# fritzsedlazeck/Sniffles

Hardware: NVIDIA H100
Metric: aligned long-read Gbp/s through lead->cluster->consensus (higher is better)
Workload: dtype int32

## Files before the change

### include/snfb.h

```cpp
#ifndef SNFB_H
#define SNFB_H

#include <stddef.h>
#include <stdint.h>

#ifdef __cplusplus
extern "C" {
#endif

#define SNFB_ABI_VERSION 3

enum { SNFB_INS = 0, SNFB_DEL = 1, SNFB_DUP = 2, SNFB_INV = 3, SNFB_BND = 4,
       SNFB_SINGLE_LEFT = 5, SNFB_SINGLE_RIGHT = 6, SNFB_NTYPES = 7 };
enum { SNFB_SRC_INLINE = 0, SNFB_SRC_SPLIT_PRIM = 1, SNFB_SRC_SPLIT_SUP = 2, SNFB_SRC_BND_SA = 3 };

#define SNFB_MEM_HOST 0u
#define SNFB_MEM_DEVICE 1u
#define SNFB_MEM_HOST_SEQ_ON_DEMAND 2u

#define SNFB_CIGAR_BAM32 0u
#define SNFB_CIGAR_16 1u
#define SNFB_CIGAR16_EVT_MIN 11u

#define SNFB_AUX_NM 1u
// ... 154 lines not shown
    int32_t  fwd;
    int32_t  rev;
    int32_t  support_long;
    int32_t  support_sa;
    int32_t  cov_upstream, cov_start, cov_center, cov_end, cov_downstream;
    int32_t  hap_counts[6];
    int32_t  sa_count;
    int32_t  sa_total;
    int32_t  bnd_mate_contig;
    int32_t  bnd_mate_pos;
    int32_t  bnd_is_first;
    int32_t  bnd_is_reverse;
    int32_t  n_strands;
    int32_t  support_inline;
    int32_t  lead_off;
    int32_t  lead_n;
    int32_t  long_off;
    int32_t  long_n;
    int32_t  alt_off;
    int32_t  alt_len;
    int32_t  hp_top, hp_support, hp_other;
    int32_t  ps_top, ps_top_null, ps_support, ps_other;
    int32_t  cluster_seed;
    int32_t  resplit_bin;
    double   stdev_pos;
    double   stdev_len;
    double   nm_mean;
} snfb_cand;

typedef struct snfb_cand_view {
    uint64_t n_cand;
    const snfb_cand* cand;
    uint64_t n_cand_leads;
    const snfb_lead* cand_leads;
    const uint64_t*  rnames;
    const uint32_t*  rnames_off;
    const double*    task_coverage_mean;
    uint64_t unverified_breaks;
} snfb_cand_view;

typedef struct snfb_seq_view {
    uint64_t n_alt_bytes;
    const uint8_t* alt;
} snfb_seq_view;

typedef struct snfb_ctx snfb_ctx;

int         snfb_version(void);
size_t      snfb_sizeof(int which);
uint64_t    snfb_hash_name(const char* s, size_t n);
int         snfb_ctx_create(int device, snfb_ctx** out);
void        snfb_ctx_destroy(snfb_ctx* ctx);
const char* snfb_last_error(snfb_ctx* ctx);
int         snfb_set_config(snfb_ctx* ctx, const snfb_config* cfg);
int         snfb_load_records(snfb_ctx* ctx, const snfb_records* block);
int         snfb_extract_leads(snfb_ctx* ctx, snfb_lead_view* out);
int         snfb_cluster_call(snfb_ctx* ctx, snfb_cand_view* out);
int         snfb_consensus(snfb_ctx* ctx, snfb_seq_view* out);
int         snfb_run(snfb_ctx* ctx, snfb_lead_view* leads, snfb_cand_view* cands, snfb_seq_view* seqs);
typedef struct snfb_bam_span {
    uint64_t cbeg, cend;
    uint32_t ubeg, uend;
    uint32_t task;
    uint32_t region;
} snfb_bam_span;
typedef struct snfb_bam_input {
    const uint8_t* bgzf; uint64_t n_bytes;
    const snfb_bam_span* span; uint64_t n_span;
    uint32_t n_task, n_contig, n_tr, n_mask;
    const snfb_task* task; const snfb_contig* contig; const int32_t* tr; const int32_t* mask; const uint32_t* mask_task_off;
} snfb_bam_input;
int         snfb_load_bam(snfb_ctx* ctx, const snfb_bam_input* in);
typedef struct snfb_region { int32_t task, start, end, _pad; } snfb_region;
int         snfb_set_regions(snfb_ctx* ctx, const snfb_region* regions, uint32_t n);
int         snfb_ingest_sizes(snfb_ctx* ctx, uint64_t out[8]);
int         snfb_ingest_fetch(snfb_ctx* ctx, snfb_rec* rec, uint16_t* cigar16, uint8_t* var, uint8_t* seq);
int         snfb_inflate_bgzf(snfb_ctx* ctx, const uint8_t* bgzf, uint64_t n_bytes, uint8_t* out, uint64_t out_cap, uint64_t* out_len);
int         snfb_deflate_bgzf(snfb_ctx* ctx, const uint8_t* in, uint64_t n_in, uint8_t* out, uint64_t out_cap, uint64_t* out_len, uint64_t* coffset);
int         snfb_last_timings(snfb_ctx* ctx, const char** names, float* ms, uint64_t* bytes, int cap);
int         snfb_device_candidates(snfb_ctx* ctx, void** dptr, uint64_t* n_cand);
int         snfb_device_alt(snfb_ctx* ctx, void** dptr, uint64_t* n_bytes);
uint64_t    snfb_launch_count(snfb_ctx* ctx);
uint64_t    snfb_rerun_count(snfb_ctx* ctx);
int         snfb_coverage_bins(snfb_ctx* ctx, uint32_t task, int binsize, const double** out, uint64_t* n_bins);
typedef struct snfb_gt_in {
    uint64_t n;
    const int32_t* task; const int32_t* svtype; const int32_t* pos; const int32_t* svlen; const int32_t* bnd_is_first; const int32_t* mate_contig;
    int32_t combine_match, combine_match_max;
} snfb_gt_in;
typedef struct snfb_gt_out {
    int64_t* match;
    int32_t* cov_start; int32_t* cov_center; int32_t* cov_end; int32_t* bnd_no_prev;
} snfb_gt_out;
int         snfb_genotype_targets(snfb_ctx* ctx, const snfb_gt_in* in, snfb_gt_out* out);

#define SNFB_GATHER_LEADS 1u
#define SNFB_GATHER_DEVICE_ONLY 2u
typedef struct snfb_gather_view {
    uint64_t n_cand;        const snfb_cand* cand;
    uint64_t n_alt_bytes;   const uint8_t*  alt;
    uint64_t n_rnames;      const uint64_t* rnames;     const uint32_t* rnames_off;
    uint64_t n_cand_leads;  const snfb_lead* cand_leads;
    const uint64_t* rank_n_cand;
    const void* dev_buffer; uint64_t dev_bytes_per_rank;
} snfb_gather_view;
int         snfb_nccl_unique_id(void* out128);
int         snfb_comm_init(snfb_ctx* ctx, const void* unique_id128, int rank, int nranks);
int         snfb_allgather_candidates(snfb_ctx* ctx, uint32_t flags, snfb_gather_view* out);
typedef struct snfb_poa_job {
    uint64_t seq_off;
    uint32_t offs_off;
    uint32_t n_seq;
    int32_t  min_cov;
    int32_t  m, n, g, e, q, c;
    int32_t  band;
    uint32_t mode;
    uint32_t out_cap;
    uint64_t out_off;
} snfb_poa_job;
int         snfb_poa(snfb_ctx* ctx, const snfb_poa_job* jobs, uint32_t n_jobs, const uint8_t* seqs, uint64_t n_seq_bytes, const int32_t* offs, uint64_t n_offs,
                     uint8_t* out, uint64_t out_bytes, int32_t* out_len);
typedef struct snfb_combine_chain { uint32_t cand_off, n_cand, chunk_off, n_chunk, is_bnd, pad; } snfb_combine_chain;
typedef struct snfb_combine_chunk { int32_t cand_off, n_cand, curr_bin, size, cov_block, pad; } snfb_combine_chunk;
typedef struct snfb_combine_in {
    uint32_t n_chain, n_chunk, n_cand, n_samples;
    const snfb_combine_chain* chains; const snfb_combine_chunk* chunks;
    const int32_t* pos; const int32_t* svlen; const uint32_t* sample;
    const int32_t* mate_contig; const int32_t* mate_pos;
    uint32_t n_cov_block; int32_t bins_per_block, cov_binsize, pad;
    const int64_t* block_start;
    const int32_t* cov;
    int32_t combine_match, combine_match_max, cluster_merge_bnd, combine_separate_intra, combine_overlap_abs, pad2;
    double  combine_pctseq;
    const uint8_t* alt; const uint64_t* alt_off; const uint32_t* alt_len; uint64_t n_alt_bytes;
} snfb_combine_in;
typedef struct snfb_combine_out {
    uint32_t* cand_group;
    int32_t*  emit_chunk;
    uint32_t* emit_ord;
    int32_t*  cov_non;
} snfb_combine_out;
int         snfb_combine_groups(snfb_ctx* ctx, const snfb_combine_in* in, snfb_combine_out* out);
typedef struct snfb_combine_plan_in {
    uint32_t n_flat, n_task;
    const uint32_t* task; const uint32_t* row; const int32_t* svtype; const int32_t* support;
    int32_t support_threshold, bin_min_size, bin_max_candidates, exhaustive;
    snfb_combine_in group;
} snfb_combine_plan_in;
typedef struct snfb_combine_plan_out {
    uint32_t n_cand, n_chain, n_chunk, pad;
    uint32_t* perm; snfb_combine_chain* chains; snfb_combine_chunk* chunks;
    snfb_combine_out group;
} snfb_combine_plan_out;
int         snfb_combine_plan(snfb_ctx* ctx, const snfb_combine_plan_in* in, snfb_combine_plan_out* out);
typedef struct snfb_pop_table {
    uint32_t n, pad;
    const int32_t* contig; const int32_t* block; const int32_t* svtype; const int32_t* pos; const int32_t* svlen;
    const uint8_t* alt; const uint64_t* alt_off; const uint32_t* alt_len; uint64_t n_alt_bytes;
} snfb_pop_table;
typedef struct snfb_pop_query {
    uint32_t n, pad;
    const int32_t* contig; const int32_t* svtype; const int32_t* pos; const int32_t* svlen;
    const uint8_t* alt; const uint64_t* alt_off; const uint32_t* alt_len; uint64_t n_alt_bytes;
    int32_t combine_match, combine_match_max, block_size, pad2;
    double  combine_pctseq;
} snfb_pop_query;
// ... 41 lines not shown
```

### sniffles_b200/binding.py

```python
import ctypes as C
import os

import numpy as np

from . import abi

_HERE = os.path.dirname(os.path.abspath(__file__))
LIB_PATH = os.path.join(_HERE, "libsnfb200.so")
_LIB = None

EXPORTS = ["snfb_version", "snfb_sizeof", "snfb_hash_name", "snfb_ctx_create", "snfb_ctx_destroy", "snfb_last_error", "snfb_set_config",
           "snfb_load_records", "snfb_extract_leads", "snfb_cluster_call", "snfb_consensus", "snfb_run",
           "snfb_last_timings", "snfb_device_candidates", "snfb_device_alt", "snfb_launch_count",
           "snfb_pin_host", "snfb_unpin_host", "snfb_pack_cigar16", "snfb_rerun_count", "snfb_coverage_bins",
           "snfb_nccl_unique_id", "snfb_comm_init", "snfb_allgather_candidates", "snfb_selftest_sqrt_frac", "snfb_poa", "snfb_combine_groups", "snfb_combine_plan", "snfb_selftest_edit_distance",
           "snfb_load_bam", "snfb_set_regions", "snfb_ingest_sizes", "snfb_ingest_fetch", "snfb_inflate_bgzf", "snfb_deflate_bgzf",
           "snfb_genotype_targets", "snfb_load_reference", "snfb_reference_runs", "snfb_fetch_reference",
           "snfb_population_load", "snfb_population_match", "snfb_read_names"]


def lib():
    global _LIB
    if _LIB is None:
        if not os.path.exists(LIB_PATH):
            raise RuntimeError(f"{LIB_PATH} is missing: build it with `python -c 'import __graft_entry__ as g; g.build()'` "
                               "(the CUDA extension is required; there is no CPU fallback)")
        L = C.CDLL(LIB_PATH)
        L.snfb_version.restype = C.c_int
        L.snfb_sizeof.restype = C.c_size_t
        L.snfb_sizeof.argtypes = [C.c_int]
        L.snfb_hash_name.restype = C.c_uint64
        L.snfb_hash_name.argtypes = [C.c_char_p, C.c_size_t]
        L.snfb_ctx_create.argtypes = [C.c_int, C.POINTER(C.c_void_p)]
        L.snfb_ctx_destroy.argtypes = [C.c_void_p]
        L.snfb_last_error.restype = C.c_char_p
        L.snfb_last_error.argtypes = [C.c_void_p]
        L.snfb_set_config.argtypes = [C.c_void_p, C.POINTER(abi.Config)]
        L.snfb_load_records.argtypes = [C.c_void_p, C.POINTER(abi.Records)]
        L.snfb_load_bam.argtypes = [C.c_void_p, C.POINTER(abi.BamInput)]
        L.snfb_set_regions.argtypes = [C.c_void_p, C.c_void_p, C.c_uint32]
        L.snfb_ingest_sizes.argtypes = [C.c_void_p, C.c_void_p]
        L.snfb_ingest_fetch.argtypes = [C.c_void_p, C.c_void_p, C.c_void_p, C.c_void_p, C.c_void_p]
        L.snfb_inflate_bgzf.argtypes = [C.c_void_p, C.c_void_p, C.c_uint64, C.c_void_p, C.c_uint64, C.POINTER(C.c_uint64)]
        L.snfb_deflate_bgzf.argtypes = [C.c_void_p, C.c_void_p, C.c_uint64, C.c_void_p, C.c_uint64, C.POINTER(C.c_uint64), C.c_void_p]
        L.snfb_extract_leads.argtypes = [C.c_void_p, C.POINTER(abi.LeadView)]
        L.snfb_cluster_call.argtypes = [C.c_void_p, C.POINTER(abi.CandView)]
        L.snfb_consensus.argtypes = [C.c_void_p, C.POINTER(abi.SeqView)]
        L.snfb_run.argtypes = [C.c_void_p, C.POINTER(abi.LeadView), C.POINTER(abi.CandView), C.POINTER(abi.SeqView)]
        L.snfb_last_timings.argtypes = [C.c_void_p, C.POINTER(C.c_char_p), C.POINTER(C.c_float), C.POINTER(C.c_uint64), C.c_int]
        L.snfb_device_candidates.argtypes = [C.c_void_p, C.POINTER(C.c_void_p), C.POINTER(C.c_uint64)]
        L.snfb_device_alt.argtypes = [C.c_void_p, C.POINTER(C.c_void_p), C.POINTER(C.c_uint64)]
        L.snfb_launch_count.restype = C.c_uint64
        L.snfb_launch_count.argtypes = [C.c_void_p]
        L.snfb_pin_host.argtypes = [C.c_void_p, C.c_size_t]
        L.snfb_unpin_host.argtypes = [C.c_void_p]
        L.snfb_rerun_count.restype = C.c_uint64
        L.snfb_rerun_count.argtypes = [C.c_void_p]
        L.snfb_coverage_bins.argtypes = [C.c_void_p, C.c_uint32, C.c_int, C.POINTER(C.c_void_p), C.POINTER(C.c_uint64)]
        L.snfb_nccl_unique_id.argtypes = [C.c_void_p]
        L.snfb_comm_init.argtypes = [C.c_void_p, C.c_void_p, C.c_int, C.c_int]
        L.snfb_allgather_candidates.argtypes = [C.c_void_p, C.c_uint32, C.POINTER(abi.GatherView)]
        L.snfb_poa.argtypes = [C.c_void_p, C.c_void_p, C.c_uint32, C.c_void_p, C.c_uint64, C.c_void_p, C.c_uint64, C.c_void_p, C.c_uint64, C.c_void_p]
        L.snfb_genotype_targets.argtypes = [C.c_void_p, C.POINTER(abi.GtIn), C.POINTER(abi.GtOut)]
        L.snfb_read_names.argtypes = [C.c_void_p, C.POINTER(abi.RnamesView)]
        L.snfb_load_reference.argtypes = [C.c_void_p, C.POINTER(abi.RefInput)]
        L.snfb_reference_runs.argtypes = [C.c_void_p, C.POINTER(C.c_void_p), C.POINTER(C.c_void_p), C.POINTER(C.c_uint64)]
        L.snfb_fetch_reference.argtypes = [C.c_void_p, C.c_void_p, C.c_uint64, C.c_void_p, C.c_uint64]
        L.snfb_combine_groups.argtypes = [C.c_void_p, C.POINTER(abi.CombineIn), C.POINTER(abi.CombineOut)]
        L.snfb_combine_plan.argtypes = [C.c_void_p, C.POINTER(abi.CombinePlanIn), C.POINTER(abi.CombinePlanOut)]
        L.snfb_population_load.argtypes = [C.c_void_p, C.POINTER(abi.PopTable)]
        L.snfb_population_match.argtypes = [C.c_void_p, C.POINTER(abi.PopQuery), C.c_void_p]
        L.snfb_selftest_edit_distance.argtypes = [C.c_void_p, C.c_void_p, C.c_uint64, C.c_void_p, C.c_void_p, C.c_void_p, C.c_void_p, C.c_uint32, C.c_void_p]
        L.snfb_selftest_sqrt_frac.restype = C.c_double
        L.snfb_selftest_sqrt_frac.argtypes = [C.c_uint64, C.c_uint64, C.c_uint64, C.c_int]
        L.snfb_pack_cigar16.restype = C.c_uint64
        L.snfb_pack_cigar16.argtypes = [C.c_void_p, C.c_uint64, C.c_void_p, C.c_void_p, C.c_void_p, C.c_uint64, C.c_uint32]
        _LIB = L
    return _LIB


class SnfbError(RuntimeError):
    pass


def pack_cigar16(rec: np.ndarray, cigar32: np.ndarray, evt_min: int = 0):
    L = lib()
    rec = np.ascontiguousarray(rec)
    cigar32 = np.ascontiguousarray(cigar32, dtype="<u4")
    need = L.snfb_pack_cigar16(rec.ctypes.data, len(rec), cigar32.ctypes.data, None, None, 0, int(evt_min))
    if need == 0xFFFFFFFFFFFFFFFF:
        raise SnfbError("snfb_pack_cigar16: a CIGAR holds an operation the path does not know")
    rec16 = np.empty(len(rec), abi.REC_DTYPE)
    cigar16 = np.empty(int(need), "<u2")
    got = L.snfb_pack_cigar16(rec.ctypes.data, len(rec), cigar32.ctypes.data, rec16.ctypes.data, cigar16.ctypes.data, int(need), int(evt_min))
    if got != need:
        raise SnfbError("snfb_pack_cigar16 failed")
    return rec16, cigar16


class Result:

    def __init__(self):
        self.leads = None
        self.task_read_count = None
        self.task_mean_nm = None
        self.rec_nm = None
        self.n_pass = 0
        self.soft_errors = 0
        self.cand = np.zeros(0, abi.CAND_DTYPE)
        self.cand_leads = np.zeros(0, abi.LEAD_DTYPE)
        self.rnames = np.zeros(0, "<u8")
        self.rn_off = np.zeros(1, "<u4")
        self.task_cov_mean = None
        self.alt = np.zeros(0, "u1")

    def alt_of(self, i):
        c = self.cand[i]
        if c["alt_off"] < 0:
            return None
        return self.alt[int(c["alt_off"]):int(c["alt_off"]) + int(c["alt_len"])].tobytes().decode()


class GatheredResult(Result):
    n_cand = n_alt_bytes = n_rnames = n_cand_leads = dev_bytes_per_rank = 0

    def in_emission_order(self):
        return np.argsort(self.cand["task"], kind="stable")


def nccl_unique_id() -> bytes:
    buf = C.create_string_buffer(128)
    if lib().snfb_nccl_unique_id(buf) != 0:
        raise SnfbError("snfb_nccl_unique_id: NCCL is not available")
    return buf.raw


class Context:

    def __init__(self, device: int = 0):
        self._lib = lib()
# ... 56 lines not shown
        z = self.ingest_sizes()
        rec, cig = np.zeros(z["n_rec"], abi.REC_DTYPE), np.zeros(z["n_cigar"], "<u2")
        var, seq = np.zeros(z["n_var"], "u1"), np.zeros(z["n_seq"], "u1")
        self._check(self._lib.snfb_ingest_fetch(self._h, rec.ctypes.data, cig.ctypes.data, var.ctypes.data, seq.ctypes.data), "snfb_ingest_fetch")
        return rec, cig, var, seq

    def inflate_bgzf(self, bgzf: np.ndarray) -> bytes:
        bgzf = np.ascontiguousarray(bgzf, dtype="u1")
        n = C.c_uint64()
        self._check(self._lib.snfb_inflate_bgzf(self._h, bgzf.ctypes.data, len(bgzf), None, 0, C.byref(n)), "snfb_inflate_bgzf")
        out = np.zeros(max(int(n.value), 1), "u1")
        self._check(self._lib.snfb_inflate_bgzf(self._h, bgzf.ctypes.data, len(bgzf), out.ctypes.data, len(out), C.byref(n)), "snfb_inflate_bgzf")
        return out[:int(n.value)].tobytes()

    def deflate_bgzf(self, data) -> tuple:
        src = np.frombuffer(bytes(data), "u1")
        nb = (len(src) + 0xff00 - 1) // 0xff00
        out = np.empty(max(nb * 65536, 1), "u1")
        coff = np.zeros(max(nb, 1), "<u8")
        n = C.c_uint64()
        self._check(self._lib.snfb_deflate_bgzf(self._h, src.ctypes.data, len(src), out.ctypes.data, len(out), C.byref(n), coff.ctypes.data), "snfb_deflate_bgzf")
        return out[:int(n.value)].tobytes(), [int(x) for x in coff[:nb]]

    def run(self, want_leads=True, want_cands=True, want_seqs=True, copy=True) -> Result:
        lv, cv, sv = abi.LeadView(), abi.CandView(), abi.SeqView()
        rc = self._lib.snfb_run(self._h, C.byref(lv) if want_leads else None, C.byref(cv) if want_cands else None,
                                C.byref(sv) if want_seqs else None)
        self._check(rc, "snfb_run")
        return self._collect(lv if want_leads else None, cv if want_cands else None, sv if want_seqs else None, copy)

    def extract_leads(self, want=True):
        lv = abi.LeadView()
        self._check(self._lib.snfb_extract_leads(self._h, C.byref(lv) if want else None), "snfb_extract_leads")
        return self._collect(lv if want else None, None, None, True)

    def cluster_call(self, want=True):
        cv = abi.CandView()
        self._check(self._lib.snfb_cluster_call(self._h, C.byref(cv) if want else None), "snfb_cluster_call")
        return self._collect(None, cv if want else None, None, True)

    def consensus(self, want=True):
        sv = abi.SeqView()
        self._check(self._lib.snfb_consensus(self._h, C.byref(sv) if want else None), "snfb_consensus")
        return self._collect(None, None, sv if want else None, True)

    def _collect(self, lv, cv, sv, copy) -> Result:
        r = Result()
        cp = (lambda a: a.copy()) if copy else (lambda a: a)
        nt = None
        if lv is not None:
            r.leads = cp(abi.view(lv.leads, abi.LEAD_DTYPE, lv.n_leads))
            nt = self._n_task()
            r.task_read_count = cp(abi.view(lv.task_read_count, "<u4", nt))
            r.task_mean_nm = cp(abi.view(lv.task_mean_nm, "<f8", nt))
            r.n_pass, r.soft_errors = int(lv.n_pass), int(lv.soft_errors)
            r._rec_nm_ptr = lv.rec_nm
        if cv is not None:
            nt = self._n_task()
            r.cand = cp(abi.view(cv.cand, abi.CAND_DTYPE, cv.n_cand))
            r.cand_leads = cp(abi.view(cv.cand_leads, abi.LEAD_DTYPE, cv.n_cand_leads))
            r.rn_off = cp(abi.view(cv.rnames_off, "<u4", cv.n_cand + 1))
            r.rnames = cp(abi.view(cv.rnames, "<u8", int(r.rn_off[-1]) if cv.n_cand else 0))
            r.task_cov_mean = cp(abi.view(cv.task_coverage_mean, "<f8", nt))
        if sv is not None:
            r.alt = cp(abi.view(sv.alt, "u1", sv.n_alt_bytes))
        return r

    def _n_task(self):
        b = self._block
        return int(b.n_task) if isinstance(b, abi.Records) else len(b.task)

    def timings(self):
        names = (C.c_char_p * 64)()
        ms = (C.c_float * 64)()
        by = (C.c_uint64 * 64)()
        n = self._lib.snfb_last_timings(self._h, names, ms, by, 64)
        return [(names[i].decode(), float(ms[i]), int(by[i])) for i in range(n)]

    def launch_count(self):
        return int(self._lib.snfb_launch_count(self._h))

    def rerun_count(self):
        return int(self._lib.snfb_rerun_count(self._h))

    def coverage_bins(self, task: int, binsize: int) -> np.ndarray:
        p = C.c_void_p()
        n = C.c_uint64()
        self._check(self._lib.snfb_coverage_bins(self._h, int(task), int(binsize), C.byref(p), C.byref(n)), "snfb_coverage_bins")
        return abi.view(p.value, "<f8", n.value).copy()

    def genotype_targets(self, task, svtype, pos, svlen, bnd_is_first, mate_contig, combine_match, combine_match_max):
        cols = [np.ascontiguousarray(a, dtype="<i4") for a in (task, svtype, pos, svlen, bnd_is_first, mate_contig)]
        n = len(cols[0])
        if any(len(a) != n for a in cols):
            raise ValueError("genotype_targets: the target arrays differ in length")
        out = (np.full(n, -1, "<i8"),) + tuple(np.zeros(n, "<i4") for _ in range(4))
        I, O = abi.GtIn(), abi.GtOut()
        I.n = n
        I.task, I.svtype, I.pos, I.svlen, I.bnd_is_first, I.mate_contig = (a.ctypes.data for a in cols)
        I.combine_match, I.combine_match_max = int(combine_match), int(combine_match_max)
        O.match, O.cov_start, O.cov_center, O.cov_end, O.bnd_no_prev = (a.ctypes.data for a in out)
        self._check(self._lib.snfb_genotype_targets(self._h, C.byref(I), C.byref(O)), "snfb_genotype_targets")
        return out

    def read_names(self):
        v = abi.RnamesView()
        self._check(self._lib.snfb_read_names(self._h, C.byref(v)), "snfb_read_names")
        return ReadNames(abi.view(v.text, "u1", v.n_text).copy(), abi.view(v.off, "<u4", v.n_names + 1).copy() if v.n_names else np.zeros(1, "<u4"),
                         int(v.collisions))

    def load_reference(self, data, contigs, is_bgzf=False):
        data = np.frombuffer(data, "u1") if isinstance(data, (bytes, bytearray, memoryview)) else np.ascontiguousarray(data, dtype="u1")
        contigs = np.ascontiguousarray(contigs, dtype=abi.REF_CONTIG_DTYPE)
        I = abi.RefInput()
        I.bytes, I.n_bytes, I.is_bgzf, I.n_contig, I.contig = data.ctypes.data, len(data), int(bool(is_bgzf)), len(contigs), contigs.ctypes.data
        self._ref_n_contig = len(contigs)
        self._check(self._lib.snfb_load_reference(self._h, C.byref(I)), "snfb_load_reference")
        return self.reference_runs()

    def reference_runs(self):
        r, o, n = C.c_void_p(), C.c_void_p(), C.c_uint64()
        self._check(self._lib.snfb_reference_runs(self._h, C.byref(r), C.byref(o), C.byref(n)), "snfb_reference_runs")
        return abi.view(r.value, "<i4", 2 * n.value).reshape(-1, 2).copy(), abi.view(o.value, "<u8", 0 if not o.value else self._ref_n_contig + 1).copy()

    def fetch_reference(self, queries) -> np.ndarray:
        queries = np.ascontiguousarray(queries, dtype=abi.REF_QUERY_DTYPE)
        cap = int((queries["out_off"] + queries["length"]).max()) if len(queries) else 0
        out = np.zeros(max(cap, 1), "u1")
        self._check(self._lib.snfb_fetch_reference(self._h, queries.ctypes.data, len(queries), out.ctypes.data, cap), "snfb_fetch_reference")
        return out[:cap]

    def comm_init(self, unique_id: bytes, rank: int, nranks: int):
        buf = C.create_string_buffer(bytes(unique_id), 128)
        self._check(self._lib.snfb_comm_init(self._h, buf, int(rank), int(nranks)), "snfb_comm_init")

    def allgather_candidates(self, with_leads=False, device_only=False, copy=True):
        gv = abi.GatherView()
        flags = (abi.GATHER_LEADS if with_leads else 0) | (abi.GATHER_DEVICE_ONLY if device_only else 0)
        self._check(self._lib.snfb_allgather_candidates(self._h, flags, C.byref(gv)), "snfb_allgather_candidates")
        g = GatheredResult()
        g.n_cand, g.n_alt_bytes, g.n_rnames, g.n_cand_leads = int(gv.n_cand), int(gv.n_alt_bytes), int(gv.n_rnames), int(gv.n_cand_leads)
        g.dev_bytes_per_rank = int(gv.dev_bytes_per_rank)
        if not device_only:
            cp = (lambda a: a.copy()) if copy else (lambda a: a)
            g.cand = cp(abi.view(gv.cand, abi.CAND_DTYPE, gv.n_cand))
            g.alt = cp(abi.view(gv.alt, "u1", gv.n_alt_bytes))
            g.rnames = cp(abi.view(gv.rnames, "<u8", gv.n_rnames))
            g.rn_off = cp(abi.view(gv.rnames_off, "<u4", gv.n_cand + 1))
            g.cand_leads = cp(abi.view(gv.cand_leads, abi.LEAD_DTYPE, gv.n_cand_leads)) if with_leads else np.zeros(0, abi.LEAD_DTYPE)
        return g

    def poa(self, jobs):
        n = len(jobs)
        if n == 0:
            return []
        J = (abi.PoaJob * n)()
        flat, offs, out_off = [], [], 0
        seq_off = 0
        for k, jb in enumerate(jobs):
            seqs = [bytes(x) for x in jb["seqs"]]
            total = sum(len(x) for x in seqs)
            J[k].seq_off, J[k].offs_off, J[k].n_seq = seq_off, len(offs), len(seqs)
            o = 0
            for x in seqs:
                offs.append(o)
                o += len(x)
# ... 150 lines not shown
```

### sniffles_b200/csrc/api.cu

```cuda
#include <algorithm>
#include <climits>
#include <cstdio>
#include <cstdlib>
#include <cstring>
#include <string>
#include <vector>
#include <dlfcn.h>
#include <omp.h>

#include "common.cuh"
#include "prims.cuh"
#include "extract.cuh"
#include "cluster.cuh"
#include "consensus.cuh"
#include "poa.cuh"
#include "combine.cuh"
#include "population.cuh"
#include "ingest.cuh"
#include "bgzf_write.cuh"
#include "genotype.cuh"
#include "rnames.cuh"
#include "reference.cuh"

template <bool Pinned> struct Buf {
    void* p = nullptr; size_t cap = 0;
    Buf() = default;
    Buf(const Buf&) = delete; Buf& operator=(const Buf&) = delete;
    ~Buf() { release(); }
    int ensure(size_t bytes) {
        if (bytes <= cap) return 0;
        release();
        size_t want = bytes + bytes / 8 + 256;
        if ((Pinned ? cudaMallocHost(&p, want) : cudaMalloc(&p, want)) != cudaSuccess) { p = nullptr; cudaGetLastError(); return 1; }
        cap = want; return 0;
    }
    template <class T> T* as() { return reinterpret_cast<T*>(p); }
    void reset() { release(); }
private:
    void release() { if (p) { if (Pinned) cudaFreeHost(p); else cudaFree(p); } p = nullptr; cap = 0; }
};
using DevBuf = Buf<false>;
using HostBuf = Buf<true>;
struct Carver {
    uint8_t* base = nullptr; size_t off = 0;
    template <class T> T* take(size_t n) { const size_t o = off; off += (n * sizeof(T) + 255) & ~(size_t)255; return base ? reinterpret_cast<T*>(base + o) : nullptr; }
};
template <bool Pinned, class Lay> static int carve(Buf<Pinned>& buf, Lay&& lay) {
    Carver m; lay(m);
    if (buf.ensure(m.off + 256)) return 1;
    Carver a; a.base = buf.template as<uint8_t>(); lay(a);
    return 0;
}

constexpr int MAX_TIMINGS = 64;

struct Id128 { char b[128]; };
struct NcclApi {
    void* h = nullptr; bool tried = false;
    int (*GetUniqueId)(void*) = nullptr; int (*CommInitRank)(void**, int, Id128, int) = nullptr;
    int (*CommDestroy)(void*) = nullptr; int (*AllGather)(const void*, void*, size_t, int, void*, cudaStream_t) = nullptr; const char* (*GetErrorString)(int) = nullptr;
};
static NcclApi g_nccl;
static bool nccl_load(std::string* err) {
    if (g_nccl.tried) { if (!g_nccl.AllGather && err) *err = "NCCL is not available in this process"; return g_nccl.AllGather != nullptr; }
    g_nccl.tried = true;
    void* h = dlopen(nullptr, RTLD_NOW | RTLD_GLOBAL);
    if (!h || !dlsym(h, "ncclAllGather")) { h = nullptr; const char* names[] = { "libnccl.so.2", "libnccl.so" }; for (const char* n : names) { h = dlopen(n, RTLD_NOW | RTLD_GLOBAL); if (h) break; } }
    if (!h) { if (err) *err = "libnccl.so.2 not found"; return false; }
    g_nccl.h = h;
    g_nccl.GetUniqueId = (int (*)(void*))dlsym(h, "ncclGetUniqueId");
    g_nccl.CommInitRank = (int (*)(void**, int, Id128, int))dlsym(h, "ncclCommInitRank");
    g_nccl.CommDestroy = (int (*)(void*))dlsym(h, "ncclCommDestroy");
    g_nccl.AllGather = (int (*)(const void*, void*, size_t, int, void*, cudaStream_t))dlsym(h, "ncclAllGather");
    g_nccl.GetErrorString = (const char* (*)(int))dlsym(h, "ncclGetErrorString");
    if (!g_nccl.GetUniqueId || !g_nccl.CommInitRank || !g_nccl.CommDestroy || !g_nccl.AllGather) { g_nccl.AllGather = nullptr; if (err) *err = "NCCL symbols missing"; return false; }
    return true;
}

struct Caps { unsigned long long lead = 0, cand = 0, cand_lead = 0, rn = 0, alt = 0, scr16 = 0, item = 0, tile = 0, req = 0, req16 = 0; };

struct snfb_ctx {
    int device = 0; cudaStream_t st = nullptr, st_copy = nullptr, st_side = nullptr; cudaEvent_t ev_b = nullptr, ev_mid = nullptr, ev_fork = nullptr, ev_join = nullptr; std::string err;
    snfb_config cfg{}; bool have_cfg = false;
    bool loaded = false, on_device = false, seq_on_demand = false; const uint8_t* h_seq = nullptr; uint32_t evt_min = 0;
    uint64_t n_rec = 0, n_cigar = 0, n_var = 0, n_seq = 0; uint32_t n_task = 0, n_contig = 0, n_tr = 0, n_mask = 0;
    const snfb_rec* d_rec = nullptr; const uint16_t* d_cigar = nullptr; const uint8_t* d_var = nullptr; const uint8_t* d_seq = nullptr;
    DevBuf b_rec, b_cigar, b_var, b_seq, b_task, b_contig, b_tr, b_trp, b_mask, b_mask_off, b_mask_task;
    HostBuf h_c16, h_rec16;
    DevBuf b_comp, b_raw, b_ing, b_ing_work; HostBuf h_ing; uint64_t ing_sizes[8] = {0, 0, 0, 0, 0, 0, 0, 0}; bool from_bam = false;
    DevBuf b_zin, b_zslot, b_zout, b_zwork;
    DevBuf b_gt;
    DevBuf b_rn, b_rn_text; HostBuf h_rn_meta, h_rn_text;
    DevBuf b_pop, b_popq; population::P pop{}; bool have_pop = false;
    DevBuf b_ref, b_ref_work; std::vector<refseq::Contig> ref_ctg; bool have_ref = false;
    HostBuf h_ref_runs, h_ref_coff, h_ref_out; uint64_t ref_n_runs = 0;
    std::vector<snfb_task> tasks;
    std::vector<snfb_region> regions, next_regions; DevBuf b_region; uint32_t n_region = 0; bool cov_view = false;
    Caps cap; bool force_no_cuts = false;
    DevBuf b_ctr, arena_r, arena_l, arena_c;
    int32_t* rec_pos; int32_t* rec_end; uint8_t* rec_flags; double* rec_nm; uint32_t* rec_nlead; uint32_t* rec_lead_off; uint32_t* sa_list; extract::RecScan* scanrec; extract::RecClip* clip; int32_t* rec_big;
    uint32_t* task_first; uint32_t* task_last; uint32_t* task_reads; unsigned long long* task_cov; int32_t* task_span; double* task_nm; double* nm_part; unsigned* nm_cnt; extract::Seg* sa_seg; uint32_t* scan_tmp_r;
    int32_t* v_pos; int32_t* v_end; uint8_t* v_flags; uint64_t* v_k0; uint64_t* v_k1; uint32_t* v_v0; uint32_t* v_v1; uint32_t* v_hist; uint32_t* v_scan; unsigned long long* v_n;
    snfb_lead* leads; extract::Event* ev_buf; snfb_lead* sorted_leads; uint32_t* radix_hist;
    cluster::B B{};
    consensus::C Cc{}; consensus::SeqReq* seq_req; uint32_t* arena_off; uint8_t* seq_arena;
    HostBuf h_seq_req, h_seq_arena; uint64_t seq_h2d_bytes = 0;
    bool stage_a_done = false, stage_b_done = false, stage_c_done = false;
    HostBuf h_ctr_buf; DevCounters* h_mid = nullptr; DevCounters* h_fin = nullptr; uint32_t* h_work = nullptr;
    HostBuf h_leads, h_task_reads, h_task_nm, h_rec_nm, h_cand, h_cand_leads, h_rnames, h_rn_off, h_task_cov, h_task_cov_raw, h_alt, h_cov_bins;
    void* comm = nullptr; int rank = 0, nranks = 1; DevBuf b_gsend, b_grecv; HostBuf h_gather, h_gather_out; unsigned long long gather_cap = 0;
    cudaEvent_t ev[MAX_TIMINGS + 1]; const char* ev_name[MAX_TIMINGS + 1]; uint64_t ev_bytes[MAX_TIMINGS + 1]; int n_ev = 0; int n_ev_load = 0; uint64_t launches = 0; uint64_t reruns = 0;
};

static uint32_t evt_need(const snfb_ctx* ctx) {
    if (!ctx->have_cfg) return SNFB_CIGAR16_EVT_MIN;
    int t = ctx->cfg.minsvlen_screen < 1 ? 1 : ctx->cfg.minsvlen_screen;
    if ((ctx->cfg.qc_nm_measure || ctx->cfg.phase) && t > 11) t = 11;
    return (uint32_t)(t < (int)SNFB_CIGAR16_EVT_MIN ? t : (int)SNFB_CIGAR16_EVT_MIN);
}
static void ctx_fail(snfb_ctx* ctx, const char* what, const char* msg) { ctx->err = std::string(what) + ": " + msg; }
static int fail(snfb_ctx* ctx, const std::string& m) { ctx->err = m; return 1; }

static void mark(snfb_ctx* ctx, const char* name, uint64_t bytes = 0) {
    if (ctx->n_ev >= MAX_TIMINGS) return;
    cudaEventRecord(ctx->ev[ctx->n_ev], ctx->st);
    ctx->ev_name[ctx->n_ev] = name; ctx->ev_bytes[ctx->n_ev] = bytes; ++ctx->n_ev;
}
static int grid_for(unsigned long long n, int threads) { unsigned long long g = (n + threads - 1) / threads; if (g < 1) g = 1; if (g > (uint64_t)NUM_SMS * 32) g = (uint64_t)NUM_SMS * 32; return (int)g; }
static int bits_for(uint32_t n) { int b = 0; while ((1ull << b) < n) ++b; return b; }

__global__ void k_gather_leads(const snfb_lead* __restrict__ leads, const uint32_t* __restrict__ sval, snfb_lead* __restrict__ out, const unsigned long long* n_ptr, unsigned long long cap) {
    const unsigned long long n = *n_ptr < cap ? *n_ptr : cap;
    for (unsigned long long i = blockIdx.x * (unsigned long long)blockDim.x + threadIdx.x; i < n; i += (unsigned long long)gridDim.x * blockDim.x) out[i] = leads[sval[i]];
}
__global__ void k_view_keys(const snfb_rec* __restrict__ rec, const int32_t* __restrict__ rec_pos, unsigned long long n, uint64_t* __restrict__ key, uint32_t* __restrict__ val, unsigned long long* n_out) {
    for (unsigned long long i = blockIdx.x * (unsigned long long)blockDim.x + threadIdx.x; i < n; i += (unsigned long long)gridDim.x * blockDim.x) {
        key[i] = ((uint64_t)(uint32_t)__ldg(&rec[i].task) << 32) | (uint64_t)((uint32_t)rec_pos[i] ^ 0x80000000u); val[i] = (uint32_t)i;
    }
    if (blockIdx.x == 0 && threadIdx.x == 0) *n_out = n;
}
__global__ void k_view_gather(const uint32_t* __restrict__ ord, unsigned long long n, const int32_t* __restrict__ pos, const int32_t* __restrict__ end, const uint8_t* __restrict__ flags,
                              int32_t* __restrict__ v_pos, int32_t* __restrict__ v_end, uint8_t* __restrict__ v_flags) {
    for (unsigned long long i = blockIdx.x * (unsigned long long)blockDim.x + threadIdx.x; i < n; i += (unsigned long long)gridDim.x * blockDim.x) {
        const uint32_t j = ord[i]; v_pos[i] = pos[j]; v_end[i] = end[j]; v_flags[i] = flags[j];
    }
}
__global__ void k_cov_bins(const int32_t* __restrict__ rec_pos, const int32_t* __restrict__ rec_end, const uint8_t* __restrict__ rec_flags, uint32_t lo, uint32_t hi,
                           int binsize, long long contig_len, long long nbins, unsigned long long* __restrict__ acc) {
    for (unsigned long long i = lo + blockIdx.x * (unsigned long long)blockDim.x + threadIdx.x; i < hi; i += (unsigned long long)gridDim.x * blockDim.x) {
        if (!(rec_flags[i] & extract::RF_PASS)) continue;
        long long a = rec_pos[i], e = rec_end[i]; if (a < 0) a = 0; if (e > contig_len) e = contig_len;
        if (e <= a) continue;
        for (long long bb = a / binsize; bb <= (e - 1) / binsize && bb < nbins; ++bb) {
            const long long s0 = bb * binsize, s1 = s0 + binsize;
            const long long o0 = a > s0 ? a : s0, o1 = e < s1 ? e : s1;
            if (o1 > o0) atomicAdd(&acc[bb], (unsigned long long)(o1 - o0));
        }
    }
}


struct GatherHdr { unsigned long long n_cand, n_alt, n_rn, n_leads, need_bytes, overflow, pad0, pad1; };
__host__ __device__ inline void gather_offsets(const GatherHdr& h, unsigned long long off[6]) {
    auto al = [](unsigned long long x) { return (x + 15ull) & ~15ull; };
    off[0] = sizeof(GatherHdr); off[1] = al(off[0] + h.n_cand * sizeof(snfb_cand)); off[2] = al(off[1] + h.n_alt); off[3] = al(off[2] + 8 * h.n_rn);
    off[4] = al(off[3] + 4 * h.n_cand); off[5] = al(off[4] + h.n_leads * sizeof(snfb_lead));
}
__device__ inline void copy16(uint8_t* dst, const uint8_t* src, unsigned long long nbytes) {
    const unsigned long long n16 = (nbytes + 15) >> 4;
    for (unsigned long long i = blockIdx.x * (unsigned long long)blockDim.x + threadIdx.x; i < n16; i += (unsigned long long)gridDim.x * blockDim.x)
        reinterpret_cast<uint4*>(dst)[i] = reinterpret_cast<const uint4*>(src)[i];
}
__global__ void k_gather_pack(const DevCounters* ctr, const snfb_cand* cand, const uint8_t* alt, const uint64_t* rnames, const uint32_t* rn_off, const snfb_lead* leads, int with_leads,
                              uint8_t* slot, unsigned long long cap) {
    GatherHdr h; h.n_cand = ctr->n_cand; h.n_alt = ctr->n_alt_bytes; h.n_rn = ctr->n_rnames; h.n_leads = with_leads ? ctr->n_cand_leads : 0ull; h.pad0 = h.pad1 = 0;
    unsigned long long off[6]; gather_offsets(h, off);
    h.need_bytes = off[5]; h.overflow = off[5] > cap ? 1ull : 0ull;
    if (blockIdx.x == 0 && threadIdx.x == 0) *reinterpret_cast<GatherHdr*>(slot) = h;
    if (h.overflow) return;
    copy16(slot + off[0], reinterpret_cast<const uint8_t*>(cand), h.n_cand * sizeof(snfb_cand));
    copy16(slot + off[1], alt, h.n_alt);
    copy16(slot + off[2], reinterpret_cast<const uint8_t*>(rnames), 8 * h.n_rn);
    copy16(slot + off[3], reinterpret_cast<const uint8_t*>(rn_off), 4 * h.n_cand);
    if (with_leads) copy16(slot + off[4], reinterpret_cast<const uint8_t*>(leads), h.n_leads * sizeof(snfb_lead));
}
__global__ void k_gather_merge(const uint8_t* recv, unsigned long long cap, int nranks, int with_leads, uint8_t* out, unsigned long long out_cap, unsigned long long* out_layout ) {
    GatherHdr tot{}; bool ovf = false;
    for (int r = 0; r < nranks; ++r) { const GatherHdr* h = reinterpret_cast<const GatherHdr*>(recv + (size_t)r * cap); tot.n_cand += h->n_cand; tot.n_alt += h->n_alt; tot.n_rn += h->n_rn; tot.n_leads += h->n_leads; ovf = ovf || h->overflow; }
    auto al = [](unsigned long long x) { return (x + 255ull) & ~255ull; };
    const unsigned long long o_hdr = 0, o_cand = al((unsigned long long)nranks * sizeof(GatherHdr)), o_alt = al(o_cand + tot.n_cand * sizeof(snfb_cand)), o_rn = al(o_alt + tot.n_alt), o_ro = al(o_rn + 8 * tot.n_rn),
                             o_leads = al(o_ro + 4 * (tot.n_cand + 1)), o_end = al(o_leads + tot.n_leads * sizeof(snfb_lead));
    const bool fits = !ovf && o_end <= out_cap;
    if (blockIdx.x == 0 && threadIdx.x == 0) { out_layout[0] = o_cand; out_layout[1] = o_alt; out_layout[2] = o_rn; out_layout[3] = o_ro; out_layout[4] = o_leads; out_layout[5] = o_end; out_layout[6] = fits ? 0 : 1; out_layout[7] = tot.n_cand; }
    if (!fits) return;
    const unsigned long long tid = blockIdx.x * (unsigned long long)blockDim.x + threadIdx.x, nthr = (unsigned long long)gridDim.x * blockDim.x;
    unsigned long long b_cand = 0, b_alt = 0, b_rn = 0, b_leads = 0;
    for (int r = 0; r < nranks; ++r) {
        const uint8_t* slot = recv + (size_t)r * cap; const GatherHdr h = *reinterpret_cast<const GatherHdr*>(slot);
        unsigned long long off[6]; gather_offsets(h, off);
        if (tid == 0) reinterpret_cast<GatherHdr*>(out + o_hdr)[r] = h;
        const snfb_cand* sc = reinterpret_cast<const snfb_cand*>(slot + off[0]); snfb_cand* dc = reinterpret_cast<snfb_cand*>(out + o_cand) + b_cand;
        for (unsigned long long i = tid; i < h.n_cand; i += nthr) { snfb_cand c = sc[i]; if (c.alt_off >= 0) c.alt_off += (int)b_alt; if (with_leads) { c.lead_off += (int)b_leads; c.long_off += (int)b_leads; } dc[i] = c; }
        for (unsigned long long i = tid; i < h.n_alt; i += nthr) (out + o_alt + b_alt)[i] = (slot + off[1])[i];
        const uint64_t* sr = reinterpret_cast<const uint64_t*>(slot + off[2]); uint64_t* dr = reinterpret_cast<uint64_t*>(out + o_rn) + b_rn;
        for (unsigned long long i = tid; i < h.n_rn; i += nthr) dr[i] = sr[i];
        const uint32_t* so = reinterpret_cast<const uint32_t*>(slot + off[3]); uint32_t* dof = reinterpret_cast<uint32_t*>(out + o_ro) + b_cand;
        for (unsigned long long i = tid; i < h.n_cand; i += nthr) dof[i] = so[i] + (uint32_t)b_rn;
        if (with_leads) { const uint4* sl = reinterpret_cast<const uint4*>(slot + off[4]); uint4* dl = reinterpret_cast<uint4*>(out + o_leads) + 4 * b_leads; for (unsigned long long i = tid; i < 4 * h.n_leads; i += nthr) dl[i] = sl[i]; }
        b_cand += h.n_cand; b_alt += h.n_alt; b_rn += h.n_rn; b_leads += h.n_leads;
    }
    if (tid == 0) reinterpret_cast<uint32_t*>(out + o_ro)[tot.n_cand] = (uint32_t)tot.n_rn;
}

static void launch_inflate(snfb_ctx* ctx, const ingest::BgzfBlock* d_blk, unsigned nb, ingest::IngestCounters* d_ctr) {
    const size_t smem = ingest::INF_SMEM_BYTES;
    const unsigned per_block = ingest::INF_WARPS * (32 / ingest::INF_LANES);
    const unsigned resident = (unsigned)std::max<size_t>(1, std::min<size_t>(8, (220 * 1024) / (smem + 1024)));
    const unsigned grid = std::min<unsigned>((nb + per_block - 1) / per_block, (unsigned)NUM_SMS * resident);
    launch(ctx->launches, ingest::k_inflate, grid, ingest::INF_WARPS * 32, smem, ctx->st, ctx->b_comp.as<uint8_t>(), d_blk, nb, ctx->b_raw.as<uint8_t>(), d_ctr);
}

extern "C" {

int snfb_version(void) { return SNFB_ABI_VERSION; }
size_t snfb_sizeof(int which) {
    switch (which) { case 0: return sizeof(snfb_rec); case 1: return sizeof(snfb_task); case 2: return sizeof(snfb_contig); case 3: return sizeof(snfb_records);
                     case 4: return sizeof(snfb_config); case 5: return sizeof(snfb_lead); case 6: return sizeof(snfb_cand); case 7: return sizeof(snfb_gather_view);
                     case 8: return sizeof(snfb_gt_in); case 9: return sizeof(snfb_gt_out);
                     case 10: return sizeof(snfb_ref_contig); case 11: return sizeof(snfb_ref_input); case 12: return sizeof(snfb_ref_query); case 13: return sizeof(snfb_region);
                     case 14: return sizeof(snfb_combine_plan_in); case 15: return sizeof(snfb_combine_plan_out);
                     case 16: return sizeof(snfb_pop_table); case 17: return sizeof(snfb_pop_query); case 18: return sizeof(snfb_rnames_view); default: return 0; }
}

uint64_t snfb_hash_name(const char* s, size_t n) {
    uint64_t h = 0xcbf29ce484222325ull; for (size_t i = 0; i < n; ++i) { h ^= (uint8_t)s[i]; h *= 0x100000001b3ull; } return h;
}

int snfb_ctx_create(int device, snfb_ctx** out) {
    if (!out) return 1;
    *out = nullptr;
    int ndev = 0;
    if (cudaGetDeviceCount(&ndev) != cudaSuccess || ndev <= 0 || device < 0 || device >= ndev) return 2;
    if (cudaSetDevice(device) != cudaSuccess) return 3;
    snfb_ctx* ctx = new snfb_ctx();
    ctx->device = device;
    if (cudaStreamCreateWithFlags(&ctx->st, cudaStreamNonBlocking) != cudaSuccess || cudaStreamCreateWithFlags(&ctx->st_copy, cudaStreamNonBlocking) != cudaSuccess
        || cudaStreamCreateWithFlags(&ctx->st_side, cudaStreamNonBlocking) != cudaSuccess) { delete ctx; return 4; }
    cudaEventCreateWithFlags(&ctx->ev_b, cudaEventDisableTiming); cudaEventCreateWithFlags(&ctx->ev_mid, cudaEventDisableTiming);
    cudaEventCreateWithFlags(&ctx->ev_fork, cudaEventDisableTiming); cudaEventCreateWithFlags(&ctx->ev_join, cudaEventDisableTiming);
    for (int i = 0; i <= MAX_TIMINGS; ++i) cudaEventCreate(&ctx->ev[i]);
    if (ctx->h_ctr_buf.ensure(2 * sizeof(DevCounters) + 256) || ctx->b_ctr.ensure(sizeof(DevCounters) + 64)) { delete ctx; return 5; }
    ctx->h_mid = ctx->h_ctr_buf.as<DevCounters>(); ctx->h_fin = ctx->h_mid + 1; ctx->h_work = reinterpret_cast<uint32_t*>(ctx->h_fin + 1);
    memset(ctx->h_ctr_buf.p, 0, 2 * sizeof(DevCounters) + 256);
    cudaFuncSetAttribute(cluster::k_cluster_warp<cluster::SMALL_CAP, cluster::CWS_WARPS, false>, cudaFuncAttributeMaxDynamicSharedMemorySize, (int)cluster::CwCfg<cluster::SMALL_CAP, cluster::CWS_WARPS>::smem);
    cudaFuncSetAttribute(cluster::k_cluster_warp<cluster::WARP_CAP, cluster::CWM_WARPS, true>, cudaFuncAttributeMaxDynamicSharedMemorySize, (int)cluster::CwCfg<cluster::WARP_CAP, cluster::CWM_WARPS>::smem);
    cudaFuncSetAttribute(cluster::k_cluster_block, cudaFuncAttributeMaxDynamicSharedMemorySize, (int)cluster::CB_SMEM);
    cudaFuncSetAttribute(bgzfw::k_deflate, cudaFuncAttributeMaxDynamicSharedMemorySize, (int)bgzfw::DEF_SMEM_BYTES);
    *out = ctx; return 0;
}

void snfb_ctx_destroy(snfb_ctx* ctx) {
    if (!ctx) return;
    cudaSetDevice(ctx->device);
    cudaStreamSynchronize(ctx->st); cudaStreamSynchronize(ctx->st_copy); cudaStreamSynchronize(ctx->st_side);
    if (ctx->comm && g_nccl.CommDestroy) g_nccl.CommDestroy(ctx->comm);
    for (int i = 0; i <= MAX_TIMINGS; ++i) cudaEventDestroy(ctx->ev[i]);
    cudaEventDestroy(ctx->ev_b); cudaEventDestroy(ctx->ev_mid); cudaEventDestroy(ctx->ev_fork); cudaEventDestroy(ctx->ev_join);
    cudaStreamDestroy(ctx->st_side); cudaStreamDestroy(ctx->st_copy); cudaStreamDestroy(ctx->st);
    delete ctx;
}

const char* snfb_last_error(snfb_ctx* ctx) { return ctx ? ctx->err.c_str() : "null context"; }

int snfb_set_config(snfb_ctx* ctx, const snfb_config* cfg) {
    if (!ctx || !cfg) return 1;
    ctx->force_no_cuts = false;
    if (cfg->consensus_kmer_len != 6) return fail(ctx, "consensus_kmer_len must be 6 (the reference fixes it, config.py:550)");
    if (cfg->cluster_binsize <= 0 || cfg->cluster_resplit_binsize <= 0 || cfg->coverage_binsize <= 0) return fail(ctx, "bin sizes must be positive");
    ctx->cfg = *cfg; ctx->have_cfg = true; ctx->stage_a_done = ctx->stage_b_done = ctx->stage_c_done = false; return 0;
}

static bool c16_offsets(const snfb_rec* rec_in, uint64_t n_rec, const uint32_t* cigar32, std::vector<uint64_t>& off) {
    off.assign(n_rec + 1, 0);
    const uint8_t* raw = reinterpret_cast<const uint8_t*>(cigar32);
    bool bad = false;
    #pragma omp parallel for schedule(static) reduction(|| : bad)
    for (long long i = 0; i < (long long)n_rec; ++i) {
        long long ref; int b = 0;
        const uint32_t w = ingest::c16_convert<1>(raw, 4ull * rec_in[i].cigar_off, rec_in[i].n_cigar, nullptr, 0, 0, &ref, &b);
        bad = bad || b; off[i + 1] = (w + 7) & ~7ull;
    }
    if (bad) return false;
    for (uint64_t i = 0; i < n_rec; ++i) off[i + 1] += off[i];
    return true;
}
static void c16_fill(const snfb_rec* rec_in, uint64_t n_rec, const uint32_t* cigar32, const std::vector<uint64_t>& off, snfb_rec* rec_out, uint16_t* out16, uint32_t evt_min) {
    const uint8_t* raw = reinterpret_cast<const uint8_t*>(cigar32);
    #pragma omp parallel for schedule(static)
    for (long long i = 0; i < (long long)n_rec; ++i) {
        uint16_t* dst = out16 + off[i]; const uint64_t span = off[i + 1] - off[i];
        long long ref; int bad = 0;
        const uint64_t k = ingest::c16_convert<1>(raw, 4ull * rec_in[i].cigar_off, rec_in[i].n_cigar, dst, evt_min, 0, &ref, &bad);
        if (k < span) memset(dst + k, 0, 2 * (span - k));
        snfb_rec r = rec_in[i]; r.n_cigar = (uint32_t)k; r.cigar_off = off[i];
        rec_out[i] = r;
    }
    memset(out16 + off[n_rec], 0, 16);
}
uint64_t snfb_pack_cigar16(const snfb_rec* rec_in, uint64_t n_rec, const uint32_t* cigar32, snfb_rec* rec_out, uint16_t* out16, uint64_t out_cap, uint32_t evt_min) {
    if (n_rec && (!rec_in || !cigar32)) return UINT64_MAX;
    if (evt_min == 0) evt_min = SNFB_CIGAR16_EVT_MIN;
    std::vector<uint64_t> off;
    if (!c16_offsets(rec_in, n_rec, cigar32, off)) return UINT64_MAX;
    const uint64_t total = off[n_rec] + 8;
    if (!out16) return total;
    if (!rec_out || out_cap < total) return UINT64_MAX;
    c16_fill(rec_in, n_rec, cigar32, off, rec_out, out16, evt_min);
    return total;
}

static int check_tables(snfb_ctx* ctx, const snfb_records* R) {
    for (uint32_t t = 0; t < R->n_task; ++t) {
        const snfb_task& k = R->task[t];
        if (k.tr_n < 0 || k.tr_off < 0 || (uint64_t)k.tr_off + (uint64_t)k.tr_n > R->n_tr) return fail(ctx, "task table: tandem-repeat range outside tr[]");
        if (R->n_contig && (k.contig < 0 || (uint32_t)k.contig >= R->n_contig)) return fail(ctx, "task table: contig index out of range");
        if (k.contig_len < 0 || k.start > k.end) return fail(ctx, "task table: bad region");
        if ((long long)k.contig_len >= ((long long)1 << 26) * (long long)(ctx->have_cfg ? ctx->cfg.cluster_binsize : 100)) return fail(ctx, "contig too long for the bin field of the sort key (contig_len / cluster_binsize must stay below 2^26)");
    }
    if (ctx->n_region) {
        for (uint32_t g = 0; g < ctx->n_region; ++g) {
            const snfb_region& r = ctx->regions[g];
            const std::string who = "region " + std::to_string(g) + " (task " + std::to_string(r.task) + ")";
            if (r.task < 0 || (uint32_t)r.task >= R->n_task) return fail(ctx, "region table: " + who + ": task index out of range");
            if (g && r.task < ctx->regions[g - 1].task) return fail(ctx, "region table: " + who + ": regions must be grouped by task in task order");
            if (r.start < 0 || r.start > r.end) return fail(ctx, "region table: " + who + ": start < 0 or start > end");
        }
    }
    if (R->n_mask && R->mask && R->mask_task_off) {
        for (uint32_t t = 0; t < R->n_task; ++t) if (R->mask_task_off[t] > R->mask_task_off[t + 1] || R->mask_task_off[t + 1] > R->n_mask) return fail(ctx, "mask_task_off must be non-decreasing and end at n_mask");
        for (uint32_t t = 0; t < R->n_task; ++t)
            for (uint32_t m = R->mask_task_off[t]; m < R->mask_task_off[t + 1]; ++m) {
                const uint32_t k = m - R->mask_task_off[t];
                if (R->mask[2 * m] > R->mask[2 * m + 1]) return fail(ctx, "N mask of task " + std::to_string(t) + ": run " + std::to_string(k) + " has start > end");
                if (k && R->mask[2 * m] < R->mask[2 * m - 1]) return fail(ctx, "N mask of task " + std::to_string(t) + ": run " + std::to_string(k) + " starts before run " + std::to_string(k - 1) + " ends (runs must be sorted and disjoint)");
            }
    }
    return 0;
}
static int upload_tables(snfb_ctx* ctx, const snfb_records* R) {
    ctx->tasks.assign(R->task, R->task + R->n_task);
// ... 267 lines not shown
        mark(ctx, "record_sizes", 0);
        launch(ctx->launches, ingest::k_rec_sizes, warp_grid, 256, 0, st, raw, recs, raw_region, (unsigned)n_raw, ctx->b_task.as<snfb_task>(), dev_regions(ctx), evt, keep, groups, var16, seq16, d_ctr);
        prims::exclusive_scan(ctx->launches, keep, idx, scan_tmp, nullptr, n_raw, &d_ctr->n_keep, st);
        prims::exclusive_scan(ctx->launches, groups, grp_off, scan_tmp, nullptr, n_raw, &d_ctr->n_groups, st);
        prims::exclusive_scan(ctx->launches, var16, var_off, scan_tmp, nullptr, n_raw, &d_ctr->n_var, st);
        prims::exclusive_scan(ctx->launches, seq16, seq_off, scan_tmp, nullptr, n_raw, &d_ctr->n_seq16, st);
        CUDA_TRY(cudaMemcpyAsync(hc, d_ctr, sizeof(*hc), cudaMemcpyDeviceToHost, st));
        CUDA_TRY(cudaStreamSynchronize(st));
        if (hc->malformed || hc->bad_cigar) return fail(ctx, std::to_string(hc->malformed) + " malformed BAM record(s), " + std::to_string(hc->bad_cigar) + " with a CIGAR operation the path does not know");
        n_rec = hc->n_keep; n_groups = hc->n_groups; n_var16 = hc->n_var; n_seq16 = hc->n_seq16;
    }
    const uint64_t n_words = 8 * n_groups + 8;
    if (ctx->b_rec.ensure(sizeof(snfb_rec) * (n_rec + 1)) || ctx->b_cigar.ensure(2 * (n_words + 16)) || ctx->b_var.ensure(16 * n_var16 + 16) || ctx->b_seq.ensure(16 * n_seq16 + 16))
        return fail(ctx, "out of device memory for the record block");
    mark(ctx, "pack_records", sizeof(snfb_rec) * n_rec + 2 * n_words + 16 * n_var16 + 16 * n_seq16);
    CUDA_TRY(cudaMemsetAsync(ctx->b_cigar.as<uint16_t>() + 8 * n_groups, 0, 2 * 24, st));
    if (n_raw) {
        const unsigned warp_grid = (unsigned)std::min<uint64_t>((n_raw + 7) / 8, (uint64_t)NUM_SMS * 16);
        launch(ctx->launches, ingest::k_pack, warp_grid, 256, 0, st, raw, recs, raw_region, (unsigned)n_raw, evt, keep, idx, grp_off, groups, var_off, seq_off, ctx->b_rec.as<snfb_rec>(), ctx->b_cigar.as<uint16_t>(), ctx->b_var.as<uint8_t>(), ctx->b_seq.as<uint8_t>());
    }
    mark(ctx, nullptr);
    ctx->n_ev_load = ctx->n_ev;
    ctx->n_rec = n_rec; ctx->n_cigar = n_words; ctx->n_var = 16 * n_var16; ctx->n_seq = 16 * n_seq16; ctx->n_task = in->n_task; ctx->n_contig = in->n_contig; ctx->n_tr = in->n_tr;
    ctx->on_device = false; ctx->seq_on_demand = false; ctx->h_seq = nullptr; ctx->evt_min = evt;
    ctx->d_rec = ctx->b_rec.as<snfb_rec>(); ctx->d_cigar = ctx->b_cigar.as<uint16_t>(); ctx->d_var = ctx->b_var.as<uint8_t>(); ctx->d_seq = ctx->b_seq.as<uint8_t>();
    ctx->ing_sizes[0] = n_rec; ctx->ing_sizes[1] = n_words; ctx->ing_sizes[2] = 16 * n_var16; ctx->ing_sizes[3] = 16 * n_seq16; ctx->ing_sizes[4] = n_raw; ctx->ing_sizes[5] = nb; ctx->ing_sizes[6] = raw_len; ctx->ing_sizes[7] = in->n_bytes;
    CUDA_TRY(cudaStreamSynchronize(st));
    ctx->loaded = true; ctx->from_bam = true; return 0;
}

int snfb_ingest_sizes(snfb_ctx* ctx, uint64_t out[8]) {
    if (!ctx || !out || !ctx->from_bam) return 1;
    for (int i = 0; i < 8; ++i) out[i] = ctx->ing_sizes[i];
    return 0;
}
int snfb_ingest_fetch(snfb_ctx* ctx, snfb_rec* rec, uint16_t* cigar16, uint8_t* var, uint8_t* seq) {
    if (!ctx || !ctx->from_bam || !ctx->loaded) return ctx ? fail(ctx, "snfb_ingest_fetch: no block built by snfb_load_bam") : 1;
    cudaSetDevice(ctx->device);
    if (rec && ctx->n_rec) CUDA_TRY(cudaMemcpy(rec, ctx->d_rec, sizeof(snfb_rec) * ctx->n_rec, cudaMemcpyDeviceToHost));
    if (cigar16 && ctx->n_cigar) CUDA_TRY(cudaMemcpy(cigar16, ctx->d_cigar, 2 * ctx->n_cigar, cudaMemcpyDeviceToHost));
    if (var && ctx->n_var) CUDA_TRY(cudaMemcpy(var, ctx->d_var, ctx->n_var, cudaMemcpyDeviceToHost));
    if (seq && ctx->n_seq) CUDA_TRY(cudaMemcpy(seq, ctx->d_seq, ctx->n_seq, cudaMemcpyDeviceToHost));
    return 0;
}

}

static void carve_r(snfb_ctx* ctx, Carver& c) {
    const size_t n = ctx->n_rec + 1, nt = ctx->n_task;
    ctx->rec_pos = c.take<int32_t>(n); ctx->rec_end = c.take<int32_t>(n); ctx->rec_flags = c.take<uint8_t>(n); ctx->rec_nm = c.take<double>(n); ctx->rec_nlead = c.take<uint32_t>(n); ctx->rec_lead_off = c.take<uint32_t>(n);
    ctx->sa_list = c.take<uint32_t>(n); ctx->scanrec = c.take<extract::RecScan>(n); ctx->clip = c.take<extract::RecClip>(n); ctx->rec_big = c.take<int32_t>(n);
    ctx->task_first = c.take<uint32_t>(nt); ctx->task_last = c.take<uint32_t>(nt); ctx->task_reads = c.take<uint32_t>(nt); ctx->task_cov = c.take<unsigned long long>(nt); ctx->task_span = c.take<int32_t>(nt); ctx->task_nm = c.take<double>(nt);
    const size_t cpt = (ctx->n_rec + extract::NM_CHUNK - 1) / extract::NM_CHUNK + 1;
    ctx->nm_part = c.take<double>(cpt * nt + 1); ctx->nm_cnt = c.take<unsigned>(cpt * nt + 1);
    ctx->sa_seg = c.take<extract::Seg>((size_t)extract::MAXSEG * extract::SA_THREADS * extract::SA_BLOCKS);
    ctx->scan_tmp_r = c.take<uint32_t>(prims::scan_tmp_elems(n) + 16);
    const size_t nv = ctx->cov_view ? n : 1;
    ctx->v_pos = c.take<int32_t>(nv); ctx->v_end = c.take<int32_t>(nv); ctx->v_flags = c.take<uint8_t>(nv);
    ctx->v_k0 = c.take<uint64_t>(nv); ctx->v_k1 = c.take<uint64_t>(nv); ctx->v_v0 = c.take<uint32_t>(nv); ctx->v_v1 = c.take<uint32_t>(nv);
    ctx->v_hist = c.take<uint32_t>(prims::radix_hist_elems(nv) + 16); ctx->v_scan = c.take<uint32_t>(prims::scan_tmp_elems(std::max<size_t>(nv, prims::radix_hist_elems(nv))) + 16);
    ctx->v_n = c.take<unsigned long long>(1);
}
static void carve_l(snfb_ctx* ctx, Carver& c) {
    const size_t n = (size_t)ctx->cap.lead + 8; cluster::B& b = ctx->B;
    ctx->leads = c.take<snfb_lead>(n); ctx->ev_buf = c.take<extract::Event>(n); ctx->sorted_leads = c.take<snfb_lead>(n);
    b.key0 = c.take<uint64_t>(n); b.val0 = c.take<uint32_t>(n); b.key1 = c.take<uint64_t>(n); b.val1 = c.take<uint32_t>(n); b.flag = c.take<uint32_t>(n); b.scan = c.take<uint32_t>(n);
    b.scan_tmp = c.take<uint32_t>(prims::scan_tmp_elems(std::max<unsigned long long>(n, prims::radix_hist_elems(n))) + 16);
    ctx->radix_hist = c.take<uint32_t>(prims::radix_hist_elems(n) + 16);
    b.bin_start = c.take<uint32_t>(n); b.bin_nl = c.take<uint32_t>(n); b.bin_nlong = c.take<uint32_t>(n); b.bin_kept = c.take<uint32_t>(n); b.bin_hap = c.take<uint32_t>(3 * n);
    b.kl_off = c.take<uint32_t>(n); b.kll_off = c.take<uint32_t>(n); b.kb_idx = c.take<uint32_t>(n); b.kl = c.take<uint32_t>(n); b.kll = c.take<uint32_t>(n); b.kleads = c.take<snfb_lead>(n); b.klleads = c.take<snfb_lead>(n);
    b.kb_bin = c.take<uint32_t>(n); b.kb_lead_off = c.take<uint32_t>(n); b.kb_lead_n = c.take<uint32_t>(n); b.kb_long_off = c.take<uint32_t>(n); b.kb_long_n = c.take<uint32_t>(n); b.kb_seed = c.take<int32_t>(n); b.kb_chain = c.take<uint32_t>(n); b.kb_repeat = c.take<uint8_t>(n);
    b.seg_start = c.take<uint32_t>(n); b.c_next = c.take<uint32_t>(n); b.c_last = c.take<uint32_t>(n); b.c_sd = c.take<double>(n); b.c_mean = c.take<double>(n); b.c_rep = c.take<uint8_t>(n);
    b.seg_sd_last = c.take<double>(n); b.seg_maxsd_first = c.take<double>(n); b.cl_first = c.take<uint32_t>(n); b.cl_last = c.take<uint32_t>(n); b.cl_rep = c.take<uint8_t>(n); b.big_list = c.take<uint32_t>(n); b.mid_list = c.take<uint32_t>(n);
    b.g_khi = c.take<uint64_t>(n); b.g_klo = c.take<uint64_t>(n); b.g_u32 = c.take<uint32_t>((size_t)cluster::coop::NU32 * n);
    b.ord = c.take<uint32_t>(n); b.st_leads = c.take<snfb_lead>(n); b.st_plo = c.take<uint32_t>(n); b.st_pn = c.take<uint32_t>(n); b.st_rn = c.take<uint64_t>(n); b.cand_tmp = c.take<snfb_cand>(n); b.sub_valid = c.take<uint8_t>(n);
    b.cl_nsub = c.take<uint32_t>(n); b.cl_nvalid = c.take<uint32_t>(n); b.cl_nlead = c.take<uint32_t>(n); b.cl_nrn = c.take<uint32_t>(n); b.cl_cand_base = c.take<uint32_t>(n); b.cl_lead_base = c.take<uint32_t>(n); b.cl_rn_base = c.take<uint32_t>(n);
    ctx->arena_off = c.take<uint32_t>(n);
}
static void carve_c(snfb_ctx* ctx, Carver& c) {
    const Caps& k = ctx->cap; cluster::B& b = ctx->B; consensus::C& cc = ctx->Cc;
    b.cand = c.take<snfb_cand>(k.cand + 1); b.cand_leads = c.take<snfb_lead>(k.cand_lead + 1); b.out_plo = c.take<uint32_t>(k.cand_lead + 1); b.out_pn = c.take<uint32_t>(k.cand_lead + 1);
    b.rnames = c.take<uint64_t>(k.rn + 1); b.rn_off_out = c.take<uint32_t>(k.cand + 2);
    cc.plan_best = c.take<uint32_t>(k.cand + 1); cc.plan_nother = c.take<uint32_t>(k.cand + 1); cc.plan_otot = c.take<uint32_t>(k.cand + 1); cc.alt_len = c.take<uint32_t>(k.cand + 1); cc.scr_len = c.take<uint32_t>(k.cand + 1);
    cc.alt_off = c.take<uint32_t>(k.cand + 1); cc.scr_off = c.take<uint32_t>(k.cand + 1); cc.work_big = c.take<uint32_t>(k.cand + 1); cc.work_small = c.take<uint32_t>(k.cand + 1); cc.work_ctr = c.take<uint32_t>(64);
    cc.items_big = c.take<consensus::C::Item>(k.item + 1); cc.items_small = c.take<consensus::C::Item>(k.item + 1); cc.tiles = c.take<uint2>(k.tile + 1);
    cc.alt = c.take<uint8_t>(k.alt + 64); cc.scr = c.take<uint8_t>(k.scr16 * 16 + 64);
    ctx->seq_req = c.take<consensus::SeqReq>(k.req + 1); ctx->seq_arena = c.take<uint8_t>(k.req16 * 16 + 64);
}
static int ensure_arenas(snfb_ctx* ctx) {
    if (carve(ctx->arena_r, [&](Carver& c) { carve_r(ctx, c); })) return fail(ctx, "out of device memory (per-record arrays)");
    if (carve(ctx->arena_l, [&](Carver& c) { carve_l(ctx, c); })) return fail(ctx, "out of device memory (per-lead arrays)");
    if (carve(ctx->arena_c, [&](Carver& c) { carve_c(ctx, c); })) return fail(ctx, "out of device memory (candidate / consensus arrays)");
    return 0;
}

static void bind_inputs(snfb_ctx* ctx) {
    cluster::B& b = ctx->B;
    b.leads = ctx->leads; b.rec = ctx->d_rec; b.task = ctx->b_task.as<snfb_task>(); b.contig = ctx->b_contig.as<snfb_contig>();
    b.tr = ctx->n_tr ? ctx->b_tr.as<int32_t>() : nullptr; b.tr_pmax = ctx->b_trp.as<int32_t>();
    b.rec_pos = ctx->cov_view ? ctx->v_pos : ctx->rec_pos; b.rec_end = ctx->cov_view ? ctx->v_end : ctx->rec_end; b.rec_flags = ctx->cov_view ? ctx->v_flags : ctx->rec_flags; b.rec_nm = ctx->rec_nm; b.rec_nlead = ctx->rec_nlead; b.rec_lead_off = ctx->rec_lead_off;
    b.task_first = ctx->task_first; b.task_last = ctx->task_last; b.task_maxspan = ctx->task_span;
    b.mask = ctx->n_mask ? ctx->b_mask.as<int32_t>() : nullptr; b.mask_task_off = ctx->n_mask ? ctx->b_mask_off.as<uint32_t>() : nullptr;
    b.n_task = ctx->n_task; b.n_bound = ctx->cap.lead; b.ctr = ctx->b_ctr.as<DevCounters>(); b.cfg = ctx->cfg;
    b.cut_gap = ctx->force_no_cuts ? INT_MAX : cluster::break_gap(ctx->cfg);
    b.cand_cap = ctx->cap.cand; b.cand_lead_cap = ctx->cap.cand_lead; b.rn_cap = ctx->cap.rn;
    consensus::C& c = ctx->Cc;
    c.cand = b.cand; c.cand_rw = b.cand; c.cand_leads = b.cand_leads; c.out_plo = b.out_plo; c.out_pn = b.out_pn; c.ord = b.ord; c.kleads = b.kleads; c.rec = ctx->d_rec; c.seq = ctx->d_seq; c.arena_off = nullptr;
    c.cand_cap = ctx->cap.cand; c.ctr = b.ctr; c.cfg = ctx->cfg; c.item_cap = ctx->cap.item; c.tile_cap = ctx->cap.tile; c.alt_cap = ctx->cap.alt; c.scr_cap16 = ctx->cap.scr16;
}

static int enqueue_stage_a(snfb_ctx* ctx) {
    const uint64_t nrec = ctx->n_rec; const uint32_t nt = ctx->n_task; const snfb_config& cf = ctx->cfg; cluster::B& b = ctx->B;
    DevCounters* ctr = b.ctr; cudaStream_t st = ctx->st;
    CUDA_TRY(cudaMemsetAsync(ctr, 0, sizeof(DevCounters), st));
    CUDA_TRY(cudaMemsetAsync(ctx->task_first, 0, 4 * nt, st)); CUDA_TRY(cudaMemsetAsync(ctx->task_last, 0, 4 * nt, st));
    CUDA_TRY(cudaMemsetAsync(ctx->task_reads, 0, 4 * nt, st)); CUDA_TRY(cudaMemsetAsync(ctx->task_cov, 0, 8 * nt, st)); CUDA_TRY(cudaMemsetAsync(ctx->task_span, 0, 4 * nt, st));
    CUDA_TRY(cudaMemsetAsync(ctx->task_nm, 0, 8 * nt, st));
    extract::WalkParams S{};
    S.scan = ctx->scanrec; S.n_rec = (uint32_t)nrec; S.cigar = ctx->d_cigar; S.task = b.task;
    S.rec_end = ctx->rec_end; S.rec_nlead = ctx->rec_nlead; S.rec_big = ctx->rec_big; S.rec = ctx->d_rec; S.region = dev_regions(ctx);
    S.ev = ctx->ev_buf; S.ev_cap = ctx->cap.lead; S.n_ev = &ctr->n_ev; S.ctr = ctr; S.minsv = cf.minsvlen_screen;
    if (evt_need(ctx) < ctx->evt_min) {
        if (ctx->on_device) return fail(ctx, "the device-resident CIGAR16 arena was packed with a larger event length than the configuration needs: repack with snfb_pack_cigar16(evt_min)");
        launch(ctx->launches, extract::k_reflag, NUM_SMS * 8, 256, 0, st, const_cast<uint16_t*>(ctx->d_cigar), ctx->n_cigar, evt_need(ctx));
        ctx->evt_min = evt_need(ctx);
    }
    mark(ctx, "k_rec_index");
    if (nrec) {
        extract::IndexParams I{};
        I.rec = ctx->d_rec; I.cigar = ctx->d_cigar; I.task = b.task; I.n_rec = (uint32_t)nrec; I.n_task = nt; I.rec_pos = ctx->rec_pos; I.task_first = ctx->task_first; I.task_last = ctx->task_last;
        I.scan = ctx->scanrec; I.clip = ctx->clip; I.rec_end = ctx->rec_end; I.rec_flags = ctx->rec_flags; I.rec_nm = ctx->rec_nm; I.rec_nlead = ctx->rec_nlead; I.ctr = ctr;
        I.mapq_min = cf.mapq; I.alen_min = cf.min_alignment_length; I.excl = cf.exclude_flags; I.want_nm = (cf.qc_nm_measure || cf.phase) ? 1 : 0;
        I.n_cigar = ctx->n_cigar; I.n_var = ctx->n_var; I.n_seq = ctx->n_seq; I.check_seq = ctx->seq_on_demand ? 0 : 1;
        I.sa_list = ctx->sa_list; I.n_sa = &ctr->n_sa; I.region = dev_regions(ctx); I.last_region = dev_last_region(ctx); I.n_region = ctx->n_region;
        launch(ctx->launches, extract::k_rec_index, (unsigned)((nrec + 255) / 256), 256, 0, st, I);
        mark(ctx, "k_scan", 2 * ctx->n_cigar);
        if (nrec >= extract::WALK_WIDE_MIN) launch(ctx->launches, extract::k_cigar_walk<32>, extract::WALK_BLOCKS, extract::WALK_THREADS, 0, st, S);
        else launch(ctx->launches, extract::k_cigar_walk<1>, extract::WALK_BLOCKS, extract::WALK_THREADS, 0, st, S);
        mark(ctx, "k_rec_post");
        extract::PostParams Q{};
        Q.scan = I.scan; Q.clip = I.clip; Q.task = b.task; Q.n_rec = (uint32_t)nrec; Q.rec_end = ctx->rec_end; Q.rec_big = ctx->rec_big; Q.rec_nm = ctx->rec_nm;
        Q.task_reads = ctx->task_reads; Q.task_cov_bp = ctx->task_cov; Q.task_maxspan = ctx->task_span;
        launch(ctx->launches, extract::k_rec_post, (unsigned)((nrec + 255) / 256), 256, 0, st, Q);
        mark(ctx, "k_emit");
        extract::EmitParams E{};
        E.rec = ctx->d_rec; E.clip = ctx->clip; E.var = ctx->d_var; E.ev = S.ev; E.n_ev = S.n_ev; E.ev_cap = ctx->cap.lead;
        E.leads = ctx->leads; E.ctr = ctr; E.maxlen = cf.dev_seq_cache_maxlen; E.detect_large_ins = cf.detect_large_ins; E.longinslen = (double)cf.long_ins_length / 2.0;
        launch(ctx->launches, extract::k_emit, NUM_SMS * 16, 128, 0, st, E);
        mark(ctx, "k_sa");
        extract::SaParams A{};
        A.rec = ctx->d_rec; A.clip = ctx->clip; A.var = ctx->d_var; A.task = b.task; A.contig = b.contig; A.n_contig = ctx->n_contig;
        A.sa_list = ctx->sa_list; A.n_sa = &ctr->n_sa; A.rec_end = ctx->rec_end; A.rec_nlead = ctx->rec_nlead; A.leads = E.leads; A.lead_cap = ctx->cap.lead; A.ctr = ctr; A.cfg = cf; A.seg_scratch = ctx->sa_seg; A.region = dev_regions(ctx);
        launch(ctx->launches, extract::k_sa, extract::SA_BLOCKS, extract::SA_THREADS, 0, st, A);
        mark(ctx, "k_task_nm");
        const int cpt = (int)((nrec + extract::NM_CHUNK - 1) / extract::NM_CHUNK);
        launch(ctx->launches, extract::k_nm_partial, dim3(cpt, nt), 256, 0, st, ctx->rec_flags, ctx->rec_nm, ctx->task_first, ctx->task_last, ctx->nm_part, ctx->nm_cnt);
        launch(ctx->launches, extract::k_task_nm, nt, 256, 0, st, ctx->task_first, ctx->task_last, ctx->nm_part, ctx->nm_cnt, cpt, ctx->task_nm);
        if (ctx->cov_view) {
            mark(ctx, "cov_order");
            launch(ctx->launches, k_view_keys, grid_for(nrec, 256), 256, 0, st, ctx->d_rec, ctx->rec_pos, (unsigned long long)nrec, ctx->v_k0, ctx->v_v0, ctx->v_n);
            prims::RadixTemp vt{ ctx->v_hist, ctx->v_scan };
            bool vfirst = true;
            prims::radix_sort(ctx->launches, ctx->v_k0, ctx->v_v0, ctx->v_k1, ctx->v_v1, vt, ctx->v_n, nrec, 32 + bits_for(nt), &vfirst, st);
            launch(ctx->launches, k_view_gather, grid_for(nrec, 256), 256, 0, st, vfirst ? ctx->v_v0 : ctx->v_v1, (unsigned long long)nrec, ctx->rec_pos, ctx->rec_end, ctx->rec_flags, ctx->v_pos, ctx->v_end, ctx->v_flags);
        }
    }
    mark(ctx, "scan_rec_leads");
    prims::exclusive_scan(ctx->launches, ctx->rec_nlead, ctx->rec_lead_off, ctx->scan_tmp_r, nullptr, nrec, &ctr->n_leads, st);
    const unsigned long long nb = b.n_bound; const int g = grid_for(nb, 256);
    mark(ctx, "sort_leads");
    launch(ctx->launches, cluster::k_scatter_keys, g, 256, 0, st, b);
    prims::RadixTemp rt{ ctx->radix_hist, b.scan_tmp };
    bool first = true;
    prims::radix_sort(ctx->launches, b.key0, b.val0, b.key1, b.val1, rt, &ctr->n_leads, nb, cluster::TASK_SHIFT + bits_for(ctx->n_task), &first, st);
    b.skey = first ? b.key0 : b.key1; b.sval = first ? b.val0 : b.val1;
    mark(ctx, "bins");
    launch(ctx->launches, cluster::k_bin_heads, g, 256, 0, st, b);
    prims::exclusive_scan(ctx->launches, b.flag, b.scan, b.scan_tmp, &ctr->n_leads, nb, &ctr->n_bins, st);
    launch(ctx->launches, cluster::k_bin_build, g, 256, 0, st, b);
    launch(ctx->launches, cluster::k_bin_stats, g, 256, 0, st, b);
    mark(ctx, nullptr);
    CUDA_TRY(cudaGetLastError());
    return 0;
}

static int enqueue_stage_b(snfb_ctx* ctx) {
    cluster::B& b = ctx->B; DevCounters* ctr = b.ctr; cudaStream_t st = ctx->st;
    const unsigned long long nb = b.n_bound; const int g = grid_for(nb, 128);
    mark(ctx, "kept_bins");
    prims::exclusive_scan(ctx->launches, b.bin_nl, b.kl_off, b.scan_tmp, &ctr->n_bins, nb, &ctr->n_kl, st);
    prims::exclusive_scan(ctx->launches, b.bin_nlong, b.kll_off, b.scan_tmp, &ctr->n_bins, nb, &ctr->n_kll, st);
    prims::exclusive_scan(ctx->launches, b.bin_kept, b.kb_idx, b.scan_tmp, &ctr->n_bins, nb, &ctr->n_kbins, st);
    launch(ctx->launches, cluster::k_kbin_build, g, 128, 0, st, b);
    launch(ctx->launches, cluster::k_gather_kept, grid_for(nb, 256), 256, 0, st, b);
    mark(ctx, "merge_chains");
    launch(ctx->launches, cluster::k_seg_heads, g, 128, 0, st, b);
    prims::exclusive_scan(ctx->launches, b.flag, b.scan, b.scan_tmp, &ctr->n_kbins, nb, &ctr->n_segs, st);
    launch(ctx->launches, cluster::k_seg_build, g, 128, 0, st, b);
    launch(ctx->launches, cluster::k_merge, g, 128, 0, st, b);
    launch(ctx->launches, cluster::k_verify_cuts, g, 128, 0, st, b);
    prims::exclusive_scan(ctx->launches, b.flag, b.scan, b.scan_tmp, &ctr->n_kbins, nb, &ctr->n_clusters, st);
    launch(ctx->launches, cluster::k_cluster_build, g, 128, 0, st, b);
    mark(ctx, "cluster_call");
    CUDA_TRY(cudaEventRecord(ctx->ev_fork, st)); CUDA_TRY(cudaStreamWaitEvent(ctx->st_side, ctx->ev_fork, 0));
    launch(ctx->launches, cluster::k_cluster_block, NUM_SMS, cluster::CB_THREADS, cluster::CB_SMEM, ctx->st_side, b);
    launch(ctx->launches, cluster::k_cluster_warp<cluster::WARP_CAP, cluster::CWM_WARPS, true>, NUM_SMS * 2, cluster::CWM_WARPS * 32, cluster::CwCfg<cluster::WARP_CAP, cluster::CWM_WARPS>::smem, ctx->st_side, b);
    CUDA_TRY(cudaEventRecord(ctx->ev_join, ctx->st_side));
    launch(ctx->launches, cluster::k_cluster_warp<cluster::SMALL_CAP, cluster::CWS_WARPS, false>, NUM_SMS * 4, cluster::CWS_WARPS * 32, cluster::CwCfg<cluster::SMALL_CAP, cluster::CWS_WARPS>::smem, st, b);
    CUDA_TRY(cudaStreamWaitEvent(st, ctx->ev_join, 0));
    mark(ctx, "emit_cands");
    prims::exclusive_scan(ctx->launches, b.cl_nvalid, b.cl_cand_base, b.scan_tmp, &ctr->n_clusters, nb, &ctr->n_cand, st);
    prims::exclusive_scan(ctx->launches, b.cl_nlead, b.cl_lead_base, b.scan_tmp, &ctr->n_clusters, nb, &ctr->n_cand_leads, st);
    prims::exclusive_scan(ctx->launches, b.cl_nrn, b.cl_rn_base, b.scan_tmp, &ctr->n_clusters, nb, &ctr->n_rnames, st);
    launch(ctx->launches, cluster::k_emit_cands, NUM_SMS * 8, 128, 0, st, b);
    mark(ctx, "coverage");
    if (ctx->n_mask) launch(ctx->launches, cluster::k_mask_bp, grid_for((unsigned long long)ctx->n_mask * 32, 128), 128, 0, st, b, ctx->b_mask_task.as<uint32_t>(), ctx->n_mask, ctx->task_cov);
    launch(ctx->launches, cluster::k_coverage, NUM_SMS * 32, 128, 0, st, b);
    consensus::C& c = ctx->Cc;
    CUDA_TRY(cudaMemsetAsync(c.work_ctr, 0, 64, st));
    mark(ctx, "consensus_plan");
    launch(ctx->launches, consensus::k_plan, grid_for(ctx->cap.cand, 128), 128, 0, st, c);
    prims::exclusive_scan(ctx->launches, c.alt_len, c.alt_off, b.scan_tmp, &ctr->n_cand, ctx->cap.cand, &ctr->n_alt_bytes, st);
    prims::exclusive_scan(ctx->launches, c.scr_len, c.scr_off, b.scan_tmp, &ctr->n_cand, ctx->cap.cand, &ctr->n_seq_bytes, st);
    launch(ctx->launches, consensus::k_plan_finish, grid_for(ctx->cap.cand, 128), 128, 0, st, c);
    mark(ctx, nullptr);
    CUDA_TRY(cudaGetLastError());
    return 0;
}

static int enqueue_stage_c(snfb_ctx* ctx) {
    cluster::B& b = ctx->B; consensus::C& c = ctx->Cc; DevCounters* ctr = b.ctr; cudaStream_t st = ctx->st;
    c.seq = ctx->d_seq; c.arena_off = nullptr; ctx->seq_h2d_bytes = 0;
    if (ctx->seq_on_demand) {
        mark(ctx, "seq_requests");
        launch(ctx->launches, consensus::k_seq_requests, grid_for(ctx->cap.cand, 128), 128, 0, st, c, ctx->seq_req, ctx->cap.req, ctx->arena_off, &ctr->n_req, &ctr->n_req_units);
        mark(ctx, nullptr);
        CUDA_TRY(cudaMemcpyAsync(ctx->h_fin, ctr, sizeof(DevCounters), cudaMemcpyDeviceToHost, st));
        CUDA_TRY(cudaStreamSynchronize(st));
        const unsigned long long nreq = ctx->h_fin->n_req, nunits = ctx->h_fin->n_req_units;
        if (nreq <= ctx->cap.req && nunits <= ctx->cap.req16 && nreq) {
            if (ctx->h_seq_req.ensure(sizeof(consensus::SeqReq) * (nreq + 1)) || ctx->h_seq_arena.ensure(nunits * 16 + 64)) return fail(ctx, "out of pinned memory (seq arena)");
            CUDA_TRY(cudaMemcpyAsync(ctx->h_seq_req.p, ctx->seq_req, sizeof(consensus::SeqReq) * nreq, cudaMemcpyDeviceToHost, st));
            CUDA_TRY(cudaStreamSynchronize(st));
            const consensus::SeqReq* rq = ctx->h_seq_req.as<consensus::SeqReq>(); uint8_t* dst = ctx->h_seq_arena.as<uint8_t>(); const uint8_t* src = ctx->h_seq; const uint64_t nseq = ctx->n_seq;
            #pragma omp parallel for schedule(static, 256)
            for (long long i = 0; i < (long long)nreq; ++i) {
                unsigned long long s0 = rq[i].src; unsigned long long nbytes = rq[i].nbytes; if (s0 > nseq) s0 = nseq; if (s0 + nbytes > nseq) nbytes = nseq - s0;
                memcpy(dst + (size_t)rq[i].dst16 * 16, src + s0, (size_t)nbytes);
            }
            mark(ctx, "h2d_seq_slices", nunits * 16);
            CUDA_TRY(cudaMemcpyAsync(ctx->seq_arena, ctx->h_seq_arena.p, nunits * 16, cudaMemcpyHostToDevice, st));
            mark(ctx, nullptr);
            ctx->seq_h2d_bytes = nunits * 16;
        }
        c.seq = ctx->seq_arena; c.arena_off = ctx->arena_off;
    }
    mark(ctx, "consensus");
    launch(ctx->launches, consensus::k_prep, NUM_SMS * 8, 128, 0, st, c);
    mark(ctx, "consensus_align");
    launch(ctx->launches, consensus::k_align, NUM_SMS * 7, consensus::ALIGN_WARPS * 32, 0, st, c);
    mark(ctx, "consensus_vote");
    launch(ctx->launches, consensus::k_vote, NUM_SMS * 16, consensus::VOTE_THREADS, 0, st, c);
    mark(ctx, nullptr);
    CUDA_TRY(cudaGetLastError());
    return 0;
}

static void initial_caps(snfb_ctx* ctx) {
    Caps& k = ctx->cap;
    const unsigned long long nrec = ctx->n_rec;
    const unsigned long long lead = std::max<unsigned long long>(1ull << 16, nrec) + (unsigned long long)extract::WALK_BLOCKS * (extract::WALK_THREADS / 32) * extract::WALK_SLOTS
                                    + (unsigned long long)extract::SA_BLOCKS * extract::SA_THREADS * extract::SLOT_CHUNK / 4;
    if (k.lead < lead) k.lead = lead;
    if (k.cand < k.lead / 8 + 1024) k.cand = k.lead / 8 + 1024;
    if (k.cand_lead < k.lead / 2 + 1024) k.cand_lead = k.lead / 2 + 1024;
    if (k.rn < k.lead / 2 + 1024) k.rn = k.lead / 2 + 1024;
    if (k.alt < (4ull << 20)) k.alt = 4ull << 20;
    if (k.scr16 < (2ull << 20)) k.scr16 = 2ull << 20;
    if (k.item < k.cand_lead / 2 + 1024) k.item = k.cand_lead / 2 + 1024;
    if (k.tile < k.cand + 4096) k.tile = k.cand + 4096;
    if (ctx->seq_on_demand) { if (k.req < k.cand_lead / 2 + 1024) k.req = k.cand_lead / 2 + 1024; if (k.req16 < (1ull << 20)) k.req16 = 1ull << 20; }
    else { if (k.req < 16) k.req = 16; if (k.req16 < 16) k.req16 = 16; }
}
static unsigned long long grown(unsigned long long need) { return need + need / 4 + 1024; }
static bool caps_fit(snfb_ctx* ctx, const DevCounters& c, const uint32_t* work, int upto) {
    Caps& k = ctx->cap; bool ok = true;
    const unsigned long long need_lead = std::max(c.n_slots, c.n_leads);
    if (need_lead > k.lead || c.lead_overflow) { k.lead = std::max(grown(need_lead), k.lead + k.lead / 2); ok = false; }
    if (upto >= 2) {
        if (c.n_cand > k.cand) { k.cand = grown(c.n_cand); ok = false; }
        if (c.n_cand_leads > k.cand_lead) { k.cand_lead = grown(c.n_cand_leads); ok = false; }
        if (c.n_rnames > k.rn) { k.rn = grown(c.n_rnames); ok = false; }
        if (c.n_alt_bytes > k.alt) { k.alt = grown(c.n_alt_bytes); ok = false; }
        if (c.n_seq_bytes > k.scr16) { k.scr16 = grown(c.n_seq_bytes); ok = false; }
        const unsigned long long items = std::max(work[4], work[5]);
        if (items > k.item) { k.item = grown(items); ok = false; }
        if (work[8] > k.tile) { k.tile = grown(work[8]); ok = false; }
    }
    if (upto >= 3) {
        if (c.n_req > k.req) { k.req = grown(c.n_req); ok = false; }
        if (c.n_req_units > k.req16) { k.req16 = grown(c.n_req_units); ok = false; }
        if (ok && c.scratch_overflow) { ok = false; k.alt = grown(k.alt); k.scr16 = grown(k.scr16); }
    } else if (ok && c.scratch_overflow) { ok = false; k.cand_lead = grown(k.cand_lead); k.rn = grown(k.rn); }
    return ok;
}

static int fill_lead_view(snfb_ctx* ctx, snfb_lead_view* out) {
    const DevCounters& c = *ctx->h_fin; const unsigned long long nl = c.n_leads; const uint32_t nt = ctx->n_task;
    if (ctx->h_leads.ensure(sizeof(snfb_lead) * (nl + 1)) || ctx->h_task_reads.ensure(4 * nt) || ctx->h_task_nm.ensure(8 * nt) || ctx->h_rec_nm.ensure(8 * (ctx->n_rec + 1)))
        return fail(ctx, "out of memory for the lead view");
    if (nl) {
        launch(ctx->launches, k_gather_leads, grid_for(nl, 256), 256, 0, ctx->st, ctx->leads, ctx->B.sval, ctx->sorted_leads, &ctx->B.ctr->n_leads, ctx->cap.lead);
        CUDA_TRY(cudaMemcpyAsync(ctx->h_leads.p, ctx->sorted_leads, sizeof(snfb_lead) * nl, cudaMemcpyDeviceToHost, ctx->st));
    }
    CUDA_TRY(cudaMemcpyAsync(ctx->h_task_reads.p, ctx->task_reads, 4 * nt, cudaMemcpyDeviceToHost, ctx->st));
    CUDA_TRY(cudaMemcpyAsync(ctx->h_task_nm.p, ctx->task_nm, 8 * nt, cudaMemcpyDeviceToHost, ctx->st));
    if (ctx->n_rec) CUDA_TRY(cudaMemcpyAsync(ctx->h_rec_nm.p, ctx->rec_nm, 8 * ctx->n_rec, cudaMemcpyDeviceToHost, ctx->st));
    CUDA_TRY(cudaStreamSynchronize(ctx->st));
    out->n_leads = nl; out->leads = ctx->h_leads.as<snfb_lead>();
    out->task_read_count = ctx->h_task_reads.as<uint32_t>(); out->task_mean_nm = ctx->h_task_nm.as<double>(); out->rec_nm = ctx->h_rec_nm.as<double>();
    uint64_t np = 0; for (uint32_t t = 0; t < nt; ++t) np += out->task_read_count[t];
    out->n_pass = np; out->soft_errors = c.soft_errors;
    return 0;
}
static int enqueue_cand_copies(snfb_ctx* ctx, const DevCounters& c, cudaStream_t stream) {
    cluster::B& b = ctx->B; const uint32_t nt = ctx->n_task;
    if (ctx->h_cand.ensure(sizeof(snfb_cand) * (c.n_cand + 1)) || ctx->h_cand_leads.ensure(sizeof(snfb_lead) * (c.n_cand_leads + 1)) || ctx->h_rnames.ensure(8 * (c.n_rnames + 1)) || ctx->h_rn_off.ensure(4 * (c.n_cand + 2))
        || ctx->h_task_cov.ensure(8 * nt) || ctx->h_task_cov_raw.ensure(8 * nt)) return fail(ctx, "out of pinned memory for the candidate view");
    if (c.n_cand) { CUDA_TRY(cudaMemcpyAsync(ctx->h_cand.p, b.cand, sizeof(snfb_cand) * c.n_cand, cudaMemcpyDeviceToHost, stream)); CUDA_TRY(cudaMemcpyAsync(ctx->h_rn_off.p, b.rn_off_out, 4 * c.n_cand, cudaMemcpyDeviceToHost, stream)); }
    if (c.n_cand_leads) CUDA_TRY(cudaMemcpyAsync(ctx->h_cand_leads.p, b.cand_leads, sizeof(snfb_lead) * c.n_cand_leads, cudaMemcpyDeviceToHost, stream));
    if (c.n_rnames) CUDA_TRY(cudaMemcpyAsync(ctx->h_rnames.p, b.rnames, 8 * c.n_rnames, cudaMemcpyDeviceToHost, stream));
    CUDA_TRY(cudaMemcpyAsync(ctx->h_task_cov_raw.p, ctx->task_cov, 8 * nt, cudaMemcpyDeviceToHost, stream));
    return 0;
}
static void finish_cand_view(snfb_ctx* ctx, const DevCounters& c, snfb_cand_view* out) {
    const uint32_t nt = ctx->n_task;
    ctx->h_rn_off.as<uint32_t>()[c.n_cand] = (uint32_t)c.n_rnames;
    double* cm = ctx->h_task_cov.as<double>(); const unsigned long long* cov = ctx->h_task_cov_raw.as<unsigned long long>();
    for (uint32_t t = 0; t < nt; ++t) cm[t] = ctx->tasks[t].contig_len > 0 ? (double)cov[t] / (double)ctx->tasks[t].contig_len : 0.0;
    out->n_cand = c.n_cand; out->cand = ctx->h_cand.as<snfb_cand>(); out->n_cand_leads = c.n_cand_leads; out->cand_leads = ctx->h_cand_leads.as<snfb_lead>();
    out->rnames = ctx->h_rnames.as<uint64_t>(); out->rnames_off = ctx->h_rn_off.as<uint32_t>(); out->task_coverage_mean = cm; out->unverified_breaks = c.unverified_breaks;
}

static const char* fatal_counter(const DevCounters& c) {
    if (c.bad_records) return "the record block is malformed: a record points outside its task table or arenas";
    if (c.unsorted) return "records are not coordinate sorted inside a task";
    if (c.ordinal_overflow) return "a read carries more than 65535 SV signatures (16-bit lead ordinal)";
    return nullptr;
}
static int run_pipeline(snfb_ctx* ctx, int upto, snfb_lead_view* leads, snfb_cand_view* cands, snfb_seq_view* seqs) {
    if (!ctx->loaded) return fail(ctx, "no records loaded");
    if (!ctx->have_cfg) return fail(ctx, "snfb_set_config was not called");
    cudaSetDevice(ctx->device);
    for (uint32_t t = 0; t < ctx->n_task; ++t) if ((long long)ctx->tasks[t].contig_len / ctx->cfg.cluster_binsize >= (1ll << 26)) return fail(ctx, "contig_len / cluster_binsize must stay below 2^26 (bin field of the sort key)");
    initial_caps(ctx);
    ctx->stage_a_done = ctx->stage_b_done = ctx->stage_c_done = false;
    for (int attempt = 0; ; ++attempt) {
        if (attempt == 6) return fail(ctx, "buffer capacities did not converge");
        if (ensure_arenas(ctx)) return 1;
        bind_inputs(ctx);
        ctx->n_ev = ctx->n_ev_load;
        cudaStream_t st = ctx->st; DevCounters* ctr = ctx->B.ctr;
        if (enqueue_stage_a(ctx)) return 1;
        bool mid = false, copies = false;
        if (upto >= 2) {
            if (enqueue_stage_b(ctx)) return 1;
            CUDA_TRY(cudaEventRecord(ctx->ev_b, st)); CUDA_TRY(cudaStreamWaitEvent(ctx->st_copy, ctx->ev_b, 0));
            CUDA_TRY(cudaMemcpyAsync(ctx->h_mid, ctr, sizeof(DevCounters), cudaMemcpyDeviceToHost, ctx->st_copy));
            CUDA_TRY(cudaMemcpyAsync(ctx->h_work, ctx->Cc.work_ctr, 64, cudaMemcpyDeviceToHost, ctx->st_copy));
            CUDA_TRY(cudaEventRecord(ctx->ev_mid, ctx->st_copy));
            mid = true;
        }
        if (upto >= 3 && !ctx->seq_on_demand) { if (enqueue_stage_c(ctx)) return 1; }
        if (mid) {
            CUDA_TRY(cudaEventSynchronize(ctx->ev_mid));
            if (const char* m = fatal_counter(*ctx->h_mid)) { cudaStreamSynchronize(st); return fail(ctx, m); }
            if (!caps_fit(ctx, *ctx->h_mid, ctx->h_work, 2)) { CUDA_TRY(cudaStreamSynchronize(st)); ++ctx->reruns; continue; }
            if (ctx->h_mid->unverified_breaks && !ctx->force_no_cuts) { CUDA_TRY(cudaStreamSynchronize(st)); ctx->force_no_cuts = true; ++ctx->reruns; continue; }
            if (cands) { if (enqueue_cand_copies(ctx, *ctx->h_mid, ctx->st_copy)) return 1; copies = true; }
            if (upto >= 3 && ctx->seq_on_demand) { if (enqueue_stage_c(ctx)) return 1; }
        }
        if (upto >= 3 && seqs) {
            const unsigned long long na = ctx->h_mid->n_alt_bytes;
            if (ctx->h_alt.ensure(na + 16)) return fail(ctx, "out of pinned memory for the ALT arena");
            if (na) CUDA_TRY(cudaMemcpyAsync(ctx->h_alt.p, ctx->Cc.alt, na, cudaMemcpyDeviceToHost, st));
        }
        CUDA_TRY(cudaMemcpyAsync(ctx->h_fin, ctr, sizeof(DevCounters), cudaMemcpyDeviceToHost, st));
        CUDA_TRY(cudaMemcpyAsync(ctx->h_work + 16, ctx->Cc.work_ctr, 64, cudaMemcpyDeviceToHost, st));
        CUDA_TRY(cudaStreamSynchronize(st));
        if (copies) CUDA_TRY(cudaStreamSynchronize(ctx->st_copy));
        CUDA_TRY(cudaGetLastError());
        if (const char* m = fatal_counter(*ctx->h_fin)) return fail(ctx, m);
        if (!caps_fit(ctx, *ctx->h_fin, upto >= 2 ? ctx->h_work + 16 : ctx->h_work, upto)) { ++ctx->reruns; continue; }
        break;
    }
    ctx->stage_a_done = true; ctx->stage_b_done = upto >= 2; ctx->stage_c_done = upto >= 3;
    if (leads) { memset(leads, 0, sizeof *leads); if (fill_lead_view(ctx, leads)) return 1; }
    if (cands) { memset(cands, 0, sizeof *cands); finish_cand_view(ctx, *ctx->h_fin, cands); }
    if (seqs) { memset(seqs, 0, sizeof *seqs); seqs->n_alt_bytes = ctx->h_fin->n_alt_bytes; seqs->alt = ctx->h_alt.as<uint8_t>(); }
    return 0;
}

extern "C" {

int snfb_extract_leads(snfb_ctx* ctx, snfb_lead_view* out) {
    if (!ctx) return 1;
    return run_pipeline(ctx, 1, out, nullptr, nullptr);
}
int snfb_cluster_call(snfb_ctx* ctx, snfb_cand_view* out) {
    if (!ctx) return 1;
    if (!ctx->stage_a_done) return fail(ctx, "snfb_extract_leads must run first");
    return run_pipeline(ctx, 2, nullptr, out, nullptr);
}
int snfb_consensus(snfb_ctx* ctx, snfb_seq_view* out) {
    if (!ctx) return 1;
    if (!ctx->stage_b_done) return fail(ctx, "snfb_cluster_call must run first");
    snfb_seq_view tmp; return run_pipeline(ctx, 3, nullptr, nullptr, out ? out : &tmp);
}
int snfb_run(snfb_ctx* ctx, snfb_lead_view* leads, snfb_cand_view* cands, snfb_seq_view* seqs) {
    if (!ctx) return 1;
    snfb_seq_view tmp; return run_pipeline(ctx, 3, leads, cands, seqs ? seqs : &tmp);
}

int snfb_last_timings(snfb_ctx* ctx, const char** names, float* ms, uint64_t* bytes, int cap) {
    if (!ctx) return 0;
    cudaSetDevice(ctx->device);
    cudaStreamSynchronize(ctx->st);
    int n = 0;
    for (int i = 0; i + 1 < ctx->n_ev && n < cap; ++i) {
        if (!ctx->ev_name[i]) continue;
        float t = 0; if (cudaEventElapsedTime(&t, ctx->ev[i], ctx->ev[i + 1]) != cudaSuccess) t = -1.f;
        names[n] = ctx->ev_name[i]; ms[n] = t; if (bytes) bytes[n] = ctx->ev_bytes[i]; ++n;
    }
    if (ctx->n_ev - ctx->n_ev_load >= 2 && n < cap) {
        float t = 0; if (cudaEventElapsedTime(&t, ctx->ev[ctx->n_ev_load], ctx->ev[ctx->n_ev - 1]) != cudaSuccess) t = -1.f;
        names[n] = "total"; ms[n] = t; if (bytes) bytes[n] = 0; ++n;
    }
    return n;
}

int snfb_device_candidates(snfb_ctx* ctx, void** dptr, uint64_t* n_cand) {
    if (!ctx || !ctx->stage_b_done) return 1;
    if (dptr) *dptr = ctx->B.cand; if (n_cand) *n_cand = ctx->h_fin->n_cand; return 0;
}
int snfb_device_alt(snfb_ctx* ctx, void** dptr, uint64_t* n_bytes) {
    if (!ctx || !ctx->stage_c_done) return 1;
    if (dptr) *dptr = ctx->Cc.alt; if (n_bytes) *n_bytes = ctx->h_fin->n_alt_bytes; return 0;
}
uint64_t snfb_launch_count(snfb_ctx* ctx) { return ctx ? ctx->launches : 0; }
double snfb_selftest_sqrt_frac(uint64_t p_hi, uint64_t p_lo, uint64_t q, int slow) { const u128 P = ((u128)p_hi << 64) | p_lo; return slow ? sqrt_frac_rn_slow(P, q) : sqrt_frac_rn(P, q); }
uint64_t snfb_rerun_count(snfb_ctx* ctx) { return ctx ? ctx->reruns : 0; }
int snfb_pin_host(void* p, size_t bytes) { return cudaHostRegister(p, bytes, cudaHostRegisterDefault) == cudaSuccess ? 0 : 1; }
int snfb_unpin_host(void* p) { return cudaHostUnregister(p) == cudaSuccess ? 0 : 1; }

int snfb_nccl_unique_id(void* out128) {
    std::string e; if (!out128 || !nccl_load(&e)) return 1;
    Id128 id; memset(&id, 0, sizeof id);
    if (g_nccl.GetUniqueId(&id) != 0) return 2;
    memcpy(out128, &id, 128); return 0;
}
int snfb_comm_init(snfb_ctx* ctx, const void* unique_id128, int rank, int nranks) {
    if (!ctx || !unique_id128 || nranks < 1 || rank < 0 || rank >= nranks) return 1;
    std::string e; if (!nccl_load(&e)) return fail(ctx, "NCCL: " + e);
    cudaSetDevice(ctx->device);
    if (ctx->comm) { g_nccl.CommDestroy(ctx->comm); ctx->comm = nullptr; }
    Id128 id; memcpy(&id, unique_id128, 128);
    const int rc = g_nccl.CommInitRank(&ctx->comm, nranks, id, rank);
    if (rc != 0) { ctx->comm = nullptr; return fail(ctx, std::string("ncclCommInitRank: ") + (g_nccl.GetErrorString ? g_nccl.GetErrorString(rc) : "error")); }
    ctx->rank = rank; ctx->nranks = nranks; ctx->gather_cap = 0; return 0;
}
int snfb_allgather_candidates(snfb_ctx* ctx, uint32_t flags, snfb_gather_view* out) {
    if (!ctx || !out) return 1;
    if (!ctx->stage_c_done) return fail(ctx, "snfb_run must run first");
    if (ctx->nranks > 1 && !ctx->comm) return fail(ctx, "snfb_comm_init was not called");
    cudaSetDevice(ctx->device);
    const int nr = ctx->nranks, with_leads = (flags & SNFB_GATHER_LEADS) ? 1 : 0; cudaStream_t st = ctx->st; cluster::B& b = ctx->B;
    memset(out, 0, sizeof *out);
    unsigned long long* h_layout = nullptr; GatherHdr* h_hdr = nullptr; uint64_t* rank_n = nullptr;
    if (carve(ctx->h_gather, [&](Carver& c) { h_layout = c.take<unsigned long long>(8); h_hdr = c.take<GatherHdr>(nr); rank_n = c.take<uint64_t>(nr); })) return fail(ctx, "out of pinned memory (gather)");
    for (int attempt = 0; attempt < 4; ++attempt) {
        if (ctx->gather_cap == 0) {
            const DevCounters& c = *ctx->h_fin; GatherHdr h{}; h.n_cand = c.n_cand; h.n_alt = c.n_alt_bytes; h.n_rn = c.n_rnames; h.n_leads = with_leads ? c.n_cand_leads : 0;
            unsigned long long off[6]; gather_offsets(h, off);
            unsigned long long mx = off[5];
            if (nr > 1) {
                if (ctx->b_gsend.ensure(256) || ctx->b_grecv.ensure(8 * (size_t)nr + 256)) return fail(ctx, "out of device memory (gather)");
                CUDA_TRY(cudaMemcpyAsync(ctx->b_gsend.p, &off[5], 8, cudaMemcpyHostToDevice, st));
                if (g_nccl.AllGather(ctx->b_gsend.p, ctx->b_grecv.p, 8, 0 , ctx->comm, st) != 0) return fail(ctx, "ncclAllGather (sizes) failed");
                std::vector<unsigned long long> all(nr);
                CUDA_TRY(cudaMemcpyAsync(all.data(), ctx->b_grecv.p, 8 * (size_t)nr, cudaMemcpyDeviceToHost, st)); CUDA_TRY(cudaStreamSynchronize(st));
                for (int r = 0; r < nr; ++r) mx = std::max(mx, all[r]);
            }
            ctx->gather_cap = (grown(mx) + 255ull) & ~255ull;
        }
        const unsigned long long cap = ctx->gather_cap, out_cap = (unsigned long long)nr * cap + 4096ull * 8;
        uint8_t* recv = nullptr; uint8_t* merged = nullptr; unsigned long long* d_layout = nullptr;
        if (ctx->b_gsend.ensure(cap + 256) || carve(ctx->b_grecv, [&](Carver& c) { recv = c.take<uint8_t>((size_t)nr * cap); merged = c.take<uint8_t>(out_cap); d_layout = c.take<unsigned long long>(8); }))
            return fail(ctx, "out of device memory (gather)");
        mark(ctx, "allgather");
        launch(ctx->launches, k_gather_pack, NUM_SMS * 4, 256, 0, st, b.ctr, b.cand, ctx->Cc.alt, b.rnames, b.rn_off_out, b.cand_leads, with_leads, nr > 1 ? ctx->b_gsend.as<uint8_t>() : recv, cap);
        if (nr > 1 && g_nccl.AllGather(ctx->b_gsend.p, recv, cap, 0 , ctx->comm, st) != 0) return fail(ctx, "ncclAllGather failed");
        launch(ctx->launches, k_gather_merge, NUM_SMS * 4, 256, 0, st, recv, cap, nr, with_leads, merged, out_cap, d_layout);
        mark(ctx, nullptr);
        CUDA_TRY(cudaMemcpyAsync(h_layout, d_layout, 64, cudaMemcpyDeviceToHost, st));
        CUDA_TRY(cudaMemcpyAsync(h_hdr, recv, sizeof(GatherHdr), cudaMemcpyDeviceToHost, st));
        for (int r = 1; r < nr; ++r) CUDA_TRY(cudaMemcpyAsync(h_hdr + r, recv + (size_t)r * cap, sizeof(GatherHdr), cudaMemcpyDeviceToHost, st));
        CUDA_TRY(cudaStreamSynchronize(st));
        unsigned long long mx = 0; for (int r = 0; r < nr; ++r) mx = std::max(mx, h_hdr[r].need_bytes);
        if (h_layout[6]) { ctx->gather_cap = (grown(mx) + 255ull) & ~255ull; ++ctx->reruns; continue; }
        if (grown(mx) > cap) ctx->gather_cap = (grown(mx) + 255ull) & ~255ull;
        GatherHdr tot{}; for (int r = 0; r < nr; ++r) { tot.n_cand += h_hdr[r].n_cand; tot.n_alt += h_hdr[r].n_alt; tot.n_rn += h_hdr[r].n_rn; tot.n_leads += h_hdr[r].n_leads; }
        for (int r = 0; r < nr; ++r) rank_n[r] = h_hdr[r].n_cand;
        out->n_cand = tot.n_cand; out->n_alt_bytes = tot.n_alt; out->n_rnames = tot.n_rn; out->n_cand_leads = tot.n_leads; out->rank_n_cand = rank_n;
        out->dev_buffer = merged; out->dev_bytes_per_rank = cap;
        if (!(flags & SNFB_GATHER_DEVICE_ONLY)) {
            const unsigned long long total = h_layout[5];
            if (ctx->h_gather_out.ensure(total)) return fail(ctx, "out of pinned memory (gather result)");
            uint8_t* hm = ctx->h_gather_out.as<uint8_t>();
            CUDA_TRY(cudaMemcpyAsync(hm, merged, total, cudaMemcpyDeviceToHost, st)); CUDA_TRY(cudaStreamSynchronize(st));
            out->cand = reinterpret_cast<const snfb_cand*>(hm + h_layout[0]); out->alt = hm + h_layout[1]; out->rnames = reinterpret_cast<const uint64_t*>(hm + h_layout[2]);
            out->rnames_off = reinterpret_cast<const uint32_t*>(hm + h_layout[3]); out->cand_leads = with_leads ? reinterpret_cast<const snfb_lead*>(hm + h_layout[4]) : nullptr;
        }
        return 0;
    }
    return fail(ctx, "gather buffer sizes did not converge");
}

int snfb_poa(snfb_ctx* ctx, const snfb_poa_job* jobs, uint32_t n_jobs, const uint8_t* seqs, uint64_t n_seq_bytes, const int32_t* offs, uint64_t n_offs, uint8_t* out, uint64_t out_bytes, int32_t* out_len) {
    if (!ctx || (n_jobs && (!jobs || !seqs || !offs || !out || !out_len))) return ctx ? fail(ctx, "snfb_poa: null argument") : 1;
    if (n_jobs == 0) return 0;
    cudaSetDevice(ctx->device);
    size_t smax = 0;
    for (uint32_t k = 0; k < n_jobs; ++k) {
        const snfb_poa_job& j = jobs[k];
// ... 558 lines not shown
```

### sniffles_b200/csrc/consensus.cuh

```cuda
#pragma once
#include "common.cuh"

namespace consensus {

constexpr int THREADS = 128;
constexpr int TAB = 2048;
constexpr uint8_t DASH = 0xff;
constexpr int MAXHIT = 512, MAXHIT_LIGHT = 384; constexpr uint32_t HEAVY_L = 3000;

struct C {
    const snfb_cand* cand; snfb_cand* cand_rw; const snfb_lead* cand_leads;
    const uint32_t* out_plo; const uint32_t* out_pn;
    const uint32_t* ord; const snfb_lead* kleads;
    const snfb_rec* rec; const uint8_t* seq;
    const uint32_t* arena_off;
    uint32_t* plan_best; uint32_t* plan_nother; uint32_t* plan_otot; uint32_t* alt_len; uint32_t* scr_len; uint32_t* alt_off; uint32_t* scr_off;
    uint8_t* alt; uint8_t* scr; unsigned long long alt_cap, scr_cap16, cand_cap;
    uint32_t* work_big; uint32_t* work_small; uint32_t* work_ctr;
    struct Item { uint32_t cand; uint32_t k; uint32_t row; uint32_t rd_off; };
    Item* items_big; Item* items_small; uint2* tiles; unsigned long long item_cap, tile_cap;
    DevCounters* ctr; snfb_config cfg;
};

__device__ __forceinline__ uint8_t seq_code(const uint8_t* sq, long long q) { const uint8_t v = sq[q >> 1]; return (q & 1) ? (v & 15) : (v >> 4); }

__global__ void k_plan(C c) {
    const unsigned long long nc = c.ctr->n_cand < c.cand_cap ? c.ctr->n_cand : c.cand_cap;
    for (unsigned long long i = blockIdx.x * (unsigned long long)blockDim.x + threadIdx.x; i < nc; i += (unsigned long long)gridDim.x * blockDim.x) {
        uint32_t al = 0, sl = 0;
        if (c.cand[i].svtype == SNFB_INS && !c.cfg.symbolic) {
            const snfb_cand* cd = &c.cand[i]; long nm = 0, bi = -1; long long bd = 0; long long tot = 0;
            for (int k = 0; k < cd->lead_n; ++k) { const snfb_lead* l = &c.cand_leads[cd->lead_off + k]; if (!(l->flags & SNFB_LF_HAS_SEQ)) continue;
                long long a = (long long)l->seq_len - cd->svlen; if (a < 0) a = -a; long long p = (long long)l->ref_start - cd->pos; if (p < 0) p = -p;
                const long long d = 2 * a + 3 * p; if (nm == 0 || d < bd) { bd = d; bi = k; } ++nm; tot += ((long long)l->seq_len + 7) & ~7ll; }
            if (nm > 0) {
                const uint32_t L = (uint32_t)c.cand_leads[cd->lead_off + bi].seq_len; al = L;
                const bool cons = (nm - 1 >= c.cfg.consensus_min_reads) && !c.cfg.no_consensus;
                c.plan_best[i] = (uint32_t)bi; c.plan_nother[i] = cons ? (uint32_t)(nm - 1) : 0u; c.plan_otot[i] = (uint32_t)(tot - ((L + 7u) & ~7u));
                const unsigned long long bytes = cons ? (unsigned long long)tot + 8 + (unsigned long long)(nm - 1) * ((L + 3u) & ~3u) + (unsigned long long)(nm - 1) * 16 + 64 + 16 + TAB * 8 : (unsigned long long)L + 24;
                sl = (uint32_t)((bytes + 15) / 16);
                c.cand_rw[i].alt_len = (int)L;
                const unsigned long long work = (unsigned long long)L * (unsigned long long)nm;
                if (work > 60000ull) c.work_big[atomicAdd(&c.work_ctr[0], 1u)] = (uint32_t)i; else c.work_small[atomicAdd(&c.work_ctr[1], 1u)] = (uint32_t)i;
                if (cons) {
                    const bool heavy = L > HEAVY_L; C::Item* dst = heavy ? c.items_big : c.items_small;
                    const uint32_t base = atomicAdd(&c.work_ctr[heavy ? 4 : 5], (uint32_t)(nm - 1));
                    uint32_t row = 0, ro = 0;
                    for (int k = 0; k < cd->lead_n; ++k) { const snfb_lead* l = &c.cand_leads[cd->lead_off + k]; if (!(l->flags & SNFB_LF_HAS_SEQ) || k == bi) continue;
                        if ((unsigned long long)base + row < c.item_cap) { C::Item it; it.cand = (uint32_t)i; it.k = (uint32_t)k; it.row = row; it.rd_off = ro; dst[base + row] = it; }
                        ++row; ro += ((uint32_t)l->seq_len + 7u) & ~7u; }
                    const uint32_t nt = (L + 4095u) / 4096u; const uint32_t tb = atomicAdd(&c.work_ctr[8], nt);
                    for (uint32_t t = 0; t < nt; ++t) if ((unsigned long long)tb + t < c.tile_cap) c.tiles[tb + t] = make_uint2((uint32_t)i, t);
                }
            }
        }
        c.alt_len[i] = al; c.scr_len[i] = sl;
    }
}

__global__ void k_plan_finish(C c) {
    const unsigned long long nc = c.ctr->n_cand < c.cand_cap ? c.ctr->n_cand : c.cand_cap;
    for (unsigned long long i = blockIdx.x * (unsigned long long)blockDim.x + threadIdx.x; i < nc; i += (unsigned long long)gridDim.x * blockDim.x)
        if (c.scr_len[i]) c.cand_rw[i].alt_off = (int)c.alt_off[i];
}

__device__ __forceinline__ uint32_t nib_swap(uint32_t w) { return ((w & 0x0f0f0f0fu) << 4) | ((w >> 4) & 0x0f0f0f0fu); }
__device__ __forceinline__ uint32_t spread4(uint32_t x) { const uint32_t t = (x | (x << 8)) & 0x00ff00ffu; return (t | (t << 4)) & 0x0f0f0f0fu; }
__device__ __forceinline__ uint2 unpack8(const uint8_t* __restrict__ sq, long long q, int n) {
    const uintptr_t A = (uintptr_t)(sq + (q >> 1));
    const uint32_t* w = reinterpret_cast<const uint32_t*>(A & ~(uintptr_t)3);
    const int qn = (int)((A & 3) << 1) | (int)(q & 1);
    const uint32_t lo = nib_swap(__ldg(w)), hi = qn + n > 8 ? nib_swap(__ldg(w + 1)) : 0u;
    const uint32_t x = __funnelshift_r(lo, hi, 4 * qn);
    return make_uint2(spread4(x & 0xffffu), spread4(x >> 16));
}
__device__ __forceinline__ void unpack_span(const uint8_t* __restrict__ sq, long long off, int len, uint8_t* __restrict__ dst, int tid, int nthr) {
    const int full = ((uintptr_t)dst & 7) == 0 ? (len & ~7) : 0;
    int jb = tid * 8;
    for (; jb + 7 * nthr * 8 < full; jb += 8 * nthr * 8) {
        uint2 v[8];
        #pragma unroll
        for (int u = 0; u < 8; ++u) v[u] = unpack8(sq, off + jb + u * nthr * 8, 8);
        #pragma unroll
        for (int u = 0; u < 8; ++u) *reinterpret_cast<uint2*>(dst + jb + u * nthr * 8) = v[u];
    }
    for (; jb < full; jb += nthr * 8) *reinterpret_cast<uint2*>(dst + jb) = unpack8(sq, off + jb, 8);
    for (; jb < len; jb += nthr * 8) {
        const int n = min(8, len - jb); const uint2 v = unpack8(sq, off + jb, n);
        for (int t = 0; t < n; ++t) dst[jb + t] = (uint8_t)(((t < 4 ? v.x : v.y) >> (8 * (t & 3))) & 15u);
    }
}
__device__ inline void unpack_lead(const C& c, uint32_t cl_index, uint8_t* dst, int tid, int nthr) {
    const uint32_t plo = c.out_plo[cl_index], pn = c.out_pn[cl_index];
    long long o = 0;
    for (uint32_t p = 0; p < pn; ++p) {
        const uint32_t slot = c.ord[plo + p]; const snfb_lead* l = &c.kleads[slot];
        const uint8_t* sq = c.arena_off ? c.seq + (size_t)c.arena_off[slot] * 16 : c.seq + c.rec[l->rec].seq_off;
        unpack_span(sq, c.arena_off ? (l->seq_off & 1) : l->seq_off, l->seq_len, dst + o, tid, nthr);
        o += l->seq_len;
    }
}

__device__ __forceinline__ uint32_t kmer6(const uint8_t* s) { return (uint32_t)s[0] | ((uint32_t)s[1] << 4) | ((uint32_t)s[2] << 8) | ((uint32_t)s[3] << 12) | ((uint32_t)s[4] << 16) | ((uint32_t)s[5] << 20); }
__device__ __forceinline__ uint32_t kmer6_u(const uint8_t* s) {
    const uintptr_t A = (uintptr_t)s; const uint32_t* w = reinterpret_cast<const uint32_t*>(A & ~(uintptr_t)3); const uint32_t sh = (uint32_t)(A & 3) * 8;
    const uint32_t l0 = w[0], l1 = w[1], l2 = sh > 16 ? w[2] : 0u;
    const uint32_t x0 = __funnelshift_r(l0, l1, sh), x1 = __funnelshift_r(l1, l2, sh);
    uint32_t t = x0 & 0x0f0f0f0fu; t = (t | (t >> 4)) & 0x00ff00ffu; t = (t | (t >> 8)) & 0xffffu;
    return t | ((x1 & 15u) << 16) | (((x1 >> 8) & 15u) << 20);
}
__device__ __forceinline__ uint32_t kslot(uint32_t key) { return (key * 2654435761u) >> 21; }

struct SeqReq { unsigned long long src; uint32_t nbytes; uint32_t dst16; };
__global__ void k_seq_requests(C c, SeqReq* req, unsigned long long req_cap, uint32_t* arena_off_rw, unsigned long long* n_req, unsigned long long* n_units) {
    const unsigned long long nc = c.ctr->n_cand < c.cand_cap ? c.ctr->n_cand : c.cand_cap;
    for (unsigned long long i = blockIdx.x * (unsigned long long)blockDim.x + threadIdx.x; i < nc; i += (unsigned long long)gridDim.x * blockDim.x) {
        if (c.scr_len[i] == 0) continue;
        const snfb_cand* cd = &c.cand[i]; const bool cons = c.plan_nother[i] > 0;
        for (int k = 0; k < cd->lead_n; ++k) {
            const snfb_lead* cl = &c.cand_leads[cd->lead_off + k];
            if (!(cl->flags & SNFB_LF_HAS_SEQ) || (!cons && (uint32_t)k != c.plan_best[i])) continue;
            const uint32_t plo = c.out_plo[cd->lead_off + k], pn = c.out_pn[cd->lead_off + k];
            for (uint32_t p = 0; p < pn; ++p) {
                const uint32_t slot = c.ord[plo + p]; const snfb_lead* l = &c.kleads[slot];
                const unsigned long long b0 = (unsigned long long)l->seq_off >> 1, b1 = ((unsigned long long)l->seq_off + l->seq_len + 1) >> 1;
                const uint32_t nb = (uint32_t)(b1 - b0) + 1;
                const unsigned long long u = atomicAdd(n_units, (unsigned long long)((nb + 15) / 16));
                const unsigned long long r = atomicAdd(n_req, 1ULL);
                arena_off_rw[slot] = (uint32_t)u;
                if (r < req_cap) { req[r].src = c.rec[l->rec].seq_off + b0; req[r].nbytes = nb; req[r].dst16 = (uint32_t)u; }
            }
        }
    }
}



__device__ __forceinline__ int match_count(const uint8_t* a, const uint8_t* b, long n) {
    const uint32_t sa = ((uintptr_t)a & 3) * 8, sb = ((uintptr_t)b & 3) * 8;
    const uint32_t* wa = reinterpret_cast<const uint32_t*>((uintptr_t)a & ~(uintptr_t)3); const uint32_t* wb = reinterpret_cast<const uint32_t*>((uintptr_t)b & ~(uintptr_t)3);
    uint32_t alo = wa[0], blo = wb[0]; int mt = 0;
    long q = 0;
    #pragma unroll 2
    for (; q + 4 <= n; q += 4) {
        const uint32_t ahi = *++wa, bhi = *++wb;
        const uint32_t x = __funnelshift_r(alo, ahi, sa) ^ __funnelshift_r(blo, bhi, sb);
// ... 58 lines not shown
    }
    __device__ __forceinline__ int exclmax(int v, int& tot) const {
        int inc = v;
        #pragma unroll
        for (int o = 1; o < 32; o <<= 1) { const int t = __shfl_up_sync(FULL, inc, o); if (tid >= o) inc = max(inc, t); }
        tot = __shfl_sync(FULL, inc, 31); int e = __shfl_up_sync(FULL, inc, 1); if (tid == 0) e = -1; return e;
    }
    __device__ __forceinline__ long sum(long v) const { return (long)__reduce_add_sync(FULL, (unsigned)v); }
};
template <int WARPS>
struct BlockGrp {
    static constexpr int NTHR = WARPS * 32; int tid; int* red;
    __device__ __forceinline__ void sync() const { __syncthreads(); }
    __device__ __forceinline__ int excl(int v, int& tot) const {
        const int lane = tid & 31, w = tid >> 5; int inc = v;
        #pragma unroll
        for (int o = 1; o < 32; o <<= 1) { const int t = __shfl_up_sync(FULL, inc, o); if (lane >= o) inc += t; }
        if (lane == 31) red[w] = inc;
        __syncthreads();
        int base = 0, all = 0;
        #pragma unroll
        for (int k = 0; k < WARPS; ++k) { const int t = red[k]; if (k < w) base += t; all += t; }
        __syncthreads();
        tot = all; return base + inc - v;
    }
    __device__ __forceinline__ int exclmax(int v, int& tot) const {
        const int lane = tid & 31, w = tid >> 5; int inc = v;
        #pragma unroll
        for (int o = 1; o < 32; o <<= 1) { const int t = __shfl_up_sync(FULL, inc, o); if (lane >= o) inc = max(inc, t); }
        int e = __shfl_up_sync(FULL, inc, 1); if (lane == 0) e = -1;
        if (lane == 31) red[w] = inc;
        __syncthreads();
        int all = -1;
        #pragma unroll
        for (int k = 0; k < WARPS; ++k) { const int t = red[k]; if (k < w) e = max(e, t); all = max(all, t); }
        __syncthreads();
        tot = all; return e;
    }
    __device__ __forceinline__ long sum(long v) const {
        const int lane = tid & 31, w = tid >> 5; const int sv = (int)__reduce_add_sync(FULL, (unsigned)v);
        if (lane == 0) red[w] = sv;
        __syncthreads();
        int all = 0;
        #pragma unroll
        for (int k = 0; k < WARPS; ++k) all += red[k];
        __syncthreads();
        return (long)all;
    }
};

template <int G>
__device__ __forceinline__ long segments_pass(const int* hi, const int* hj, int* hcl, int na, long c0, long j0, long L, const uint8_t* rd, const uint8_t* best, int tid, int nthr) {
    const int PER = nthr / G; const int grp = tid / G, sub = tid % G; long span = 0;
    for (int mb = 1; mb < na; mb += PER) {
        const int m = mb + grp; const bool v = m < na;
        long li = 0, lj = 0, i = 0, j = 0; if (v) { li = hi[m - 1]; lj = hj[m - 1]; i = hi[m]; j = hj[m]; }
        long cs = c0 + lj - j0; if (cs > L) cs = L;
        const long d = j - lj; long fwd_j = d; if (cs + fwd_j > L) fwd_j = L - cs;
        const bool el = v && i - li == fwd_j && fwd_j > 0;
        long nc = 0; if (el) { nc = L - 1 - li; if (nc > d) nc = d; if (nc < 0) nc = 0; }
        const int mt = group_sum<G>(group_match<G>(rd + lj + 1, best + li + 1, nc, sub));
        int st = -1; bool second = false;
        if (el) { if (sub == 0) span += d; if (__ddiv_rn((double)mt, (double)d) >= 0.5) { if (cs == li && fwd_j == d && nc == d) st = mt; else second = true; } }
        const int m2 = group_sum<G>(group_match<G>(rd + lj, best + cs, second ? fwd_j : 0, sub));
        if (second) st = m2;
        if (v && sub == 0) hcl[m] = st;
    }
    return span;
}

struct Layout { uint8_t* best; uint8_t* oth; uint8_t* rows; uint8_t* acc; uint32_t Ls; };
__device__ __forceinline__ Layout cand_layout(const C& c, uint32_t ci, uint32_t L, uint32_t no) {
    Layout y; y.best = c.scr + (size_t)c.scr_off[ci] * 16; y.oth = y.best + ((L + 7u) & ~7u);
    y.rows = reinterpret_cast<uint8_t*>(((uintptr_t)(y.oth + c.plan_otot[ci]) + 3) & ~(uintptr_t)3); y.Ls = (L + 3u) & ~3u; y.acc = y.rows + (size_t)no * y.Ls;
    return y;
}
__device__ __forceinline__ uint8_t* cand_table(const C& c, uint32_t ci, uint32_t** keys, int** pos) {
    uint8_t* scr = c.scr + (size_t)c.scr_off[ci] * 16;
    uint8_t* end = scr + (size_t)c.scr_len[ci] * 16;
    *keys = reinterpret_cast<uint32_t*>(end - TAB * 8); *pos = reinterpret_cast<int*>(end - TAB * 4);
    return scr;
}

__global__ void __launch_bounds__(128) k_prep(C c) {
    __shared__ uint32_t s_cand;
    static const char CODE[17] = "=ACMGRSVTWYHKDBN";
    for (;;) {
        __syncthreads();
        if (threadIdx.x == 0) { const uint32_t q = atomicAdd(&c.work_ctr[2], 1u); const uint32_t nb = c.work_ctr[0], ns = c.work_ctr[1];
            s_cand = q < nb ? c.work_big[q] : (q < nb + ns ? c.work_small[q - nb] : 0xffffffffu); }
        __syncthreads();
        const uint32_t ci = s_cand; if (ci == 0xffffffffu) break;
        const uint32_t L = c.alt_len[ci];
        if ((unsigned long long)c.alt_off[ci] + L > c.alt_cap || (unsigned long long)c.scr_off[ci] + c.scr_len[ci] > c.scr_cap16) { if (threadIdx.x == 0) atomicAdd(&c.ctr->scratch_overflow, 1ULL); continue; }
        const snfb_cand cd = c.cand[ci];
        uint32_t* tk; int* tp; uint8_t* best = cand_table(c, ci, &tk, &tp);
        unpack_lead(c, cd.lead_off + c.plan_best[ci], best, threadIdx.x, blockDim.x);
        const uint32_t no = c.plan_nother[ci];
        if (no == 0 || L == 0) { __syncthreads(); uint8_t* out = c.alt + c.alt_off[ci]; for (uint32_t h = threadIdx.x; h < L; h += blockDim.x) out[h] = (uint8_t)CODE[best[h]]; continue; }
        for (int i = threadIdx.x; i < TAB; i += blockDim.x) { tk[i] = 0xffffffffu; tp[i] = -1; }
        __syncthreads();
        const long skip = c.cfg.consensus_kmer_skip_base + (long)__dmul_rn((double)L, c.cfg.consensus_kmer_skip_seqlen_mult);
        for (long i = (long)threadIdx.x * skip; i < (long)L - 6; i += (long)blockDim.x * skip) {
            const uint32_t key = kmer6_u(best + i); uint32_t s = kslot(key);
            for (;;) { const uint32_t old = atomicCAS(&tk[s], 0xffffffffu, key); if (old == 0xffffffffu || old == key) break; s = (s + 1) & (TAB - 1); }
            if (atomicCAS(&tp[s], -1, (int)i) != -1) tp[s] = -2;
        }
    }
}

template <typename G>
__device__ __forceinline__ void align_item(const C& c, const C::Item it, const G g, int* hi, int* hj, int* hcl, int* run_st, int* run_len, int cap) {
    const int tid = g.tid; constexpr int NT = G::NTHR; const int klen = 6;
    const uint32_t ci = it.cand; const uint32_t L = c.alt_len[ci];
    if ((unsigned long long)c.scr_off[ci] + c.scr_len[ci] > c.scr_cap16) return;
    const snfb_cand* cd = &c.cand[ci];
    uint32_t* t_key; int* t_pos; cand_table(c, ci, &t_key, &t_pos);
    const uint32_t no = c.plan_nother[ci];
    const Layout y = cand_layout(c, ci, L, no);
    uint8_t* best = y.best; uint8_t* acc = y.acc;
    const snfb_lead* l = &c.cand_leads[cd->lead_off + it.k];
    const long Lo = l->seq_len; uint8_t* rd = y.oth + it.rd_off; uint8_t* row = y.rows + (size_t)it.row * y.Ls;
    const long skip = c.cfg.consensus_kmer_skip_base + (long)__dmul_rn((double)L, c.cfg.consensus_kmer_skip_seqlen_mult);
    unpack_lead(c, cd->lead_off + it.k, rd, tid, NT);
    g.sync();
    int nh = 0;
    const long nk = Lo - klen > 0 ? (Lo - klen + skip - 1) / skip : 0;
    for (long kb = 0; kb < nk; kb += 4 * NT) {
        uint32_t key[4], sl[4], tk[4]; int ai[4];
        #pragma unroll
        for (int u = 0; u < 4; ++u) { const long kk = kb + u * NT + tid; key[u] = kk < nk ? kmer6_u(rd + kk * skip) : 0u; sl[u] = kslot(key[u]); }
        #pragma unroll
        for (int u = 0; u < 4; ++u) tk[u] = kb + u * NT + tid < nk ? t_key[sl[u]] : 0xffffffffu;
        #pragma unroll
        for (int u = 0; u < 4; ++u) while (tk[u] != 0xffffffffu && tk[u] != key[u]) { sl[u] = (sl[u] + 1) & (TAB - 1); tk[u] = t_key[sl[u]]; }
        #pragma unroll
        for (int u = 0; u < 4; ++u) ai[u] = tk[u] != 0xffffffffu ? t_pos[sl[u]] : -1;
        #pragma unroll
        for (int u = 0; u < 4; ++u) {
            if (kb + (long)u * NT >= nk) break;
            const long j = (kb + u * NT + tid) * skip;
            if (ai[u] >= 0) { long d = ai[u] - j; if (d < 0) d = -d; if (d > klen) ai[u] = -1; }
            int tot; const int off = g.excl(ai[u] >= 0 ? 1 : 0, tot);
            if (ai[u] >= 0) { const int p = nh + off; if (p < cap) { hi[p] = ai[u]; hj[p] = (int)j; } }
            nh += tot;
        }
    }
    if (nh > cap) nh = cap;
    g.sync();
    int na = 0, pm = -1;
    for (int hb = 0; hb < nh; hb += NT) {
        const int h = hb + tid; const int vi = h < nh ? hi[h] : -1, vj = h < nh ? hj[h] : 0;
        int tmax; const int exc = max(g.exclmax(vi, tmax), pm);
        const bool accp = h < nh && vi > exc;
        int tot; const int off = g.excl(accp ? 1 : 0, tot);
        g.sync();
        if (accp) { hi[na + off] = vi; hj[na + off] = vj; }
        na += tot; pm = max(pm, tmax);
        g.sync();
    }
    const long j0 = na ? hj[0] : 0, c0 = (na && j0 > 0) ? hi[0] : 0;
    long span = skip > 12 ? segments_pass<8>(hi, hj, hcl, na, c0, j0, (long)L, rd, best, tid, NT) : segments_pass<1>(hi, hj, hcl, na, c0, j0, (long)L, rd, best, tid, NT);
    span = g.sum(span);
    g.sync();
    {
        int* hr = hi;
        for (int m = tid; m < na; m += NT) { run_st[m] = 0; run_len[m] = 0; }
        g.sync();
        int run_base = 0;
        for (int mb = 1; mb < na; mb += NT) {
            const int m = mb + tid; int st = -1; long len = 0;
            if (m < na) { const long lj = hj[m - 1]; long cs = c0 + lj - j0; if (cs > (long)L) cs = (long)L; len = hj[m] - lj; if (cs + len > (long)L) len = (long)L - cs; st = hcl[m]; }
            int tot; const int rid = run_base + g.excl((m < na && st < 0 && len > 0) ? 1 : 0, tot);
            g.sync();
            if (m < na) { hr[m] = rid; if (st >= 0) { atomicAdd(&run_st[rid], st); atomicAdd(&run_len[rid], (int)len); } }
            run_base += tot;
        }
        g.sync();
        for (int m = 1 + tid; m < na; m += NT) {
            if (hcl[m] < 0) continue;
            const int r = hr[m], ident = run_st[r];
            if (!(__ddiv_rn((double)ident, (double)run_len[r]) > 0.5 && ident > 5)) hcl[m] = -1;
        }
        g.sync();
    }
    {
        long cl = 0; if (na) { cl = c0 + hj[na - 1] - j0; if (cl > (long)L) cl = (long)L; }
        const uint8_t* src0 = rd + (j0 - c0);
        #pragma unroll 4
        for (long X = 4L * tid; X < (long)L; X += 4L * NT) {
            uint32_t v = 0xffffffffu;
            if (X + 4 > c0 && X < cl) {
                v = load_u32_unaligned(src0 + X);
                if (X < c0) v |= (1u << (8 * (c0 - X))) - 1u;
                if (X + 4 > cl) v |= ~((1u << (8 * (cl - X))) - 1u);
            }
            *reinterpret_cast<uint32_t*>(row + X) = v;
        }
        g.sync();
        for (int m = 1 + tid; m < na; m += NT) {
            if (hcl[m] >= 0) continue;
            const long lj = hj[m - 1]; long cs = c0 + lj - j0; if (cs > (long)L) cs = (long)L;
            long len = hj[m] - lj; if (cs + len > (long)L) len = (long)L - cs;
            if (len > 0) fill_dash(row + cs, len);
        }
    }
    if (tid == 0) acc[it.row] = __ddiv_rn((double)span, (double)L) > 0.2;
    g.sync();
}

constexpr int ALIGN_WARPS = 4;
__global__ void __launch_bounds__(ALIGN_WARPS * 32, 7) k_align(C c) {
    __shared__ int sm[5][ALIGN_WARPS * MAXHIT_LIGHT]; __shared__ int s_red[2 * ALIGN_WARPS]; __shared__ uint32_t s_q;
    static_assert(ALIGN_WARPS * MAXHIT_LIGHT >= MAXHIT, "a block item needs MAXHIT entries");
    const int lane = lane_id(), warp = threadIdx.x >> 5;
    const uint32_t nb = (uint32_t)min((unsigned long long)c.work_ctr[4], c.item_cap), ns = (uint32_t)min((unsigned long long)c.work_ctr[5], c.item_cap);
    for (;;) {
        __syncthreads();
        if (threadIdx.x == 0) s_q = atomicAdd(&c.work_ctr[6], 1u);
        __syncthreads();
        const uint32_t q = s_q; if (q >= nb) break;
        BlockGrp<ALIGN_WARPS> g; g.tid = threadIdx.x; g.red = s_red;
        align_item(c, c.items_big[q], g, sm[0], sm[1], sm[2], sm[3], sm[4], ALIGN_WARPS * MAXHIT_LIGHT);
    }
    __syncthreads();
    for (;;) {
        uint32_t q = 0; if (lane == 0) q = atomicAdd(&c.work_ctr[7], 1u);
        q = __shfl_sync(FULL, q, 0);
        if (q >= ns) break;
        WarpGrp g; g.tid = lane; const int o = warp * MAXHIT_LIGHT;
        align_item(c, c.items_small[q], g, sm[0] + o, sm[1] + o, sm[2] + o, sm[3] + o, sm[4] + o, MAXHIT_LIGHT);
    }
}

constexpr int VOTE_LIST = 256;
__device__ __forceinline__ void vote_add(unsigned long long (&cnt)[4], uint32_t code) {
    const unsigned long long inc = 1ull << (16 * (code & 3u)); const uint32_t sel = (code >> 2) & 3u;
    #pragma unroll
    for (int k = 0; k < 4; ++k) cnt[k] += sel == (uint32_t)k ? inc : 0ull;
}
constexpr int VOTE_THREADS = 64;
__global__ void __launch_bounds__(VOTE_THREADS) k_vote(C c) {
    __shared__ uint2 s_tile; __shared__ int s_nacc, s_nlist; __shared__ uint16_t s_rows[VOTE_LIST];
    static const char CODE[17] = "=ACMGRSVTWYHKDBN";
    for (;;) {
        __syncthreads();
        if (threadIdx.x == 0) { const uint32_t q = atomicAdd(&c.work_ctr[9], 1u); s_tile = q < c.work_ctr[8] && q < c.tile_cap ? c.tiles[q] : make_uint2(0xffffffffu, 0); }
        __syncthreads();
        const uint32_t ci = s_tile.x; if (ci == 0xffffffffu) break;
        const uint32_t L = c.alt_len[ci], no = c.plan_nother[ci];
        if ((unsigned long long)c.alt_off[ci] + L > c.alt_cap || (unsigned long long)c.scr_off[ci] + c.scr_len[ci] > c.scr_cap16) continue;
        const Layout y = cand_layout(c, ci, L, no);
        const uint8_t* best = y.best; const uint8_t* rows = y.rows; const uint8_t* acc = y.acc; const uint32_t Ls = y.Ls;
        if (threadIdx.x < 32) {
            int cnt = 0, extra = 0; const uint32_t lim = no < (uint32_t)VOTE_LIST ? no : (uint32_t)VOTE_LIST;
            for (uint32_t r0 = 0; r0 < lim; r0 += 32) { const uint32_t r = r0 + threadIdx.x; const bool a = r < lim && acc[r]; const unsigned bm = __ballot_sync(FULL, a);
                if (a) s_rows[cnt + __popc(bm & lanemask_lt())] = (uint16_t)r; cnt += __popc(bm); }
            for (uint32_t r = lim + threadIdx.x; r < no; r += 32) extra += acc[r] ? 1 : 0;
            extra = (int)__reduce_add_sync(FULL, (unsigned)extra);
            if (threadIdx.x == 0) { s_nlist = cnt; s_nacc = cnt + extra; }
        }
        __syncthreads();
        const double maxal = (double)(1 + s_nacc); const int nlist = s_nlist;
        uint8_t* out = c.alt + c.alt_off[ci];
        const uint32_t h_end = min(L, (s_tile.y + 1u) * 4096u);
        for (uint32_t h = s_tile.y * 4096u + threadIdx.x * 4u; h < h_end; h += blockDim.x * 4u) {
            const uint32_t bw = *reinterpret_cast<const uint32_t*>(best + h);
            if (nlist == s_nacc && nlist < 255) {
                uint32_t cA = 0, cC = 0, cG = 0, cT = 0, cD = 0, multi = 0;
                for (int r0 = 0; r0 < nlist; r0 += 8) {
                    uint32_t cv[8];
                    #pragma unroll
                    for (int u = 0; u < 8; ++u) cv[u] = r0 + u < nlist ? *reinterpret_cast<const uint32_t*>(rows + (size_t)s_rows[r0 + u] * Ls + h) : 0xffffffffu;
                    #pragma unroll
                    for (int u = 0; u < 8; ++u) {
                        const uint32_t hb = cv[u] & 0x80808080u, d1 = hb >> 7, t = cv[u] & ~(hb | (hb - d1));
                        cD += d1; multi |= ((t | 0x10101010u) - 0x01010101u) & t;
                        cA += t & 0x01010101u; cC += (t >> 1) & 0x01010101u; cG += (t >> 2) & 0x01010101u; cT += (t >> 3) & 0x01010101u;
                    }
                }
                const uint32_t padded = (uint32_t)((nlist + 7) & ~7);
                const uint32_t tot = cA + cC + cG + cT + cD;
                const bool best_ok = (((bw | 0x10101010u) - 0x01010101u) & bw) == 0 && ((bw - 0x01010101u) & ~bw & 0x80808080u) == 0;
                if (multi == 0 && best_ok && padded <= 248 && tot == padded * 0x01010101u) {
                    #pragma unroll
                    for (int b2 = 0; b2 < 4; ++b2) {
                        if (h + b2 >= h_end) break;
                        const uint32_t bc = (bw >> (8 * b2)) & 255u; uint32_t res = bc;
                        const int nal = (int)padded - (int)((cD >> (8 * b2)) & 255u);
                        if (!(nal < 2 || __ddiv_rn((double)nal, maxal) < 0.25)) {
                            int v4[4] = { (int)((cA >> (8 * b2)) & 255u), (int)((cC >> (8 * b2)) & 255u), (int)((cG >> (8 * b2)) & 255u), (int)((cT >> (8 * b2)) & 255u) };
                            int t0 = -1, t1 = -1, c0 = 0, nd = 0;
                            #pragma unroll
                            for (int k = 0; k < 4; ++k) { const int v = v4[k] + ((bc >> k) & 1u); if (!v) continue; ++nd; if (v > t0) { t1 = t0; t0 = v; c0 = 1 << k; } else if (v > t1) t1 = v; }
                            if (nd > 1 && t0 - t1 >= 3) res = (uint32_t)c0;
                        }
                        out[h + b2] = (uint8_t)CODE[res];
                    }
                    continue;
                }
            }
            unsigned long long cnt[4][4]; int nal[4];
            #pragma unroll
            for (int b2 = 0; b2 < 4; ++b2) { nal[b2] = 0; cnt[b2][0] = cnt[b2][1] = cnt[b2][2] = cnt[b2][3] = 0; }
            for (int r0 = 0; r0 < nlist; r0 += 8) {
                uint32_t cv[8];
                #pragma unroll
                for (int u = 0; u < 8; ++u) cv[u] = r0 + u < nlist ? *reinterpret_cast<const uint32_t*>(rows + (size_t)s_rows[r0 + u] * Ls + h) : 0xffffffffu;
                #pragma unroll
                for (int u = 0; u < 8; ++u) {
                    #pragma unroll
                    for (int b2 = 0; b2 < 4; ++b2) { const uint32_t cc = (cv[u] >> (8 * b2)) & 255u; if (cc != DASH) { vote_add(cnt[b2], cc); ++nal[b2]; } }
                }
            }
            for (uint32_t r = VOTE_LIST; r < no; ++r) if (acc[r]) {
                const uint32_t v = *reinterpret_cast<const uint32_t*>(rows + (size_t)r * Ls + h);
                #pragma unroll
                for (int b2 = 0; b2 < 4; ++b2) { const uint32_t cc = (v >> (8 * b2)) & 255u; if (cc != DASH) { vote_add(cnt[b2], cc); ++nal[b2]; } }
            }
            #pragma unroll
            for (int b2 = 0; b2 < 4; ++b2) {
                if (h + b2 >= h_end) break;
                const uint32_t bc = (bw >> (8 * b2)) & 255u; uint32_t res = bc;
                if (!(nal[b2] < 2 || __ddiv_rn((double)nal[b2], maxal) < 0.25)) {
                    vote_add(cnt[b2], bc);
                    int t0 = -1, t1 = -1, c0 = 0, nd = 0;
                    #pragma unroll
                    for (int code = 0; code < 16; ++code) { const int v = (int)((cnt[b2][code >> 2] >> (16 * (code & 3))) & 0xffff); if (!v) continue; ++nd; if (v > t0) { t1 = t0; t0 = v; c0 = code; } else if (v > t1) t1 = v; }
                    if (nd > 1 && t0 - t1 >= 3) res = (uint32_t)c0;
                }
// ... 8 lines not shown
```

### sniffles_b200/csrc/prims.cuh

```cuda
#pragma once
#include "common.cuh"

namespace prims {

constexpr int SCAN_THREADS = 256;
constexpr int SCAN_ITEMS = 16;
constexpr int SCAN_TILE = SCAN_THREADS * SCAN_ITEMS;

__device__ __forceinline__ uint32_t warp_incl_scan(uint32_t v) {
    #pragma unroll
    for (int o = 1; o < 32; o <<= 1) { uint32_t t = __shfl_up_sync(FULL, v, o); if (lane_id() >= o) v += t; }
    return v;
}

__device__ inline uint32_t block_excl_scan(uint32_t v, uint32_t* total) {
    __shared__ uint32_t wsum[8];
    __shared__ uint32_t tot;
    uint32_t inc = warp_incl_scan(v);
    int w = threadIdx.x >> 5;
    if (lane_id() == 31) wsum[w] = inc;
    __syncthreads();
    if (threadIdx.x < 32) {
        uint32_t x = threadIdx.x < 8 ? wsum[threadIdx.x] : 0;
        uint32_t xi = warp_incl_scan(x);
        if (threadIdx.x < 8) wsum[threadIdx.x] = xi - x;
        if (threadIdx.x == 7) tot = xi;
    }
    __syncthreads();
    uint32_t r = inc - v + wsum[w];
    *total = tot;
    __syncthreads();
    return r;
}

__global__ void __launch_bounds__(SCAN_THREADS) k_scan_reduce(const uint32_t* __restrict__ in, uint32_t* __restrict__ tile_sum,
                                                              const unsigned long long* __restrict__ n_ptr, unsigned long long n_bound) {
    unsigned long long n = n_ptr ? *n_ptr : n_bound; if (n > n_bound) n = n_bound;
    unsigned long long base = (unsigned long long)blockIdx.x * SCAN_TILE;
    uint32_t s = 0;
    #pragma unroll
    for (int i = 0; i < SCAN_ITEMS; ++i) { unsigned long long j = base + (unsigned long long)i * SCAN_THREADS + threadIdx.x; if (j < n) s += in[j]; }
    uint32_t tot; block_excl_scan(s, &tot);
    if (threadIdx.x == 0) tile_sum[blockIdx.x] = tot;
}
__global__ void __launch_bounds__(SCAN_THREADS) k_scan_tiles(uint32_t* __restrict__ tile_sum, int ntiles, unsigned long long* total_out) {
    uint32_t carry = 0;
    for (int b = 0; b < ntiles; b += SCAN_THREADS) {
        int j = b + threadIdx.x; uint32_t v = j < ntiles ? tile_sum[j] : 0; uint32_t tot;
        uint32_t e = block_excl_scan(v, &tot);
        if (j < ntiles) tile_sum[j] = e + carry;
        carry += tot;
    }
    if (threadIdx.x == 0 && total_out) *total_out = carry;
}
__global__ void __launch_bounds__(SCAN_THREADS) k_scan_down(const uint32_t* __restrict__ in, uint32_t* __restrict__ out, const uint32_t* __restrict__ tile_sum,
                                                            const unsigned long long* __restrict__ n_ptr, unsigned long long n_bound) {
    unsigned long long n = n_ptr ? *n_ptr : n_bound; if (n > n_bound) n = n_bound;
    unsigned long long base = (unsigned long long)blockIdx.x * SCAN_TILE + (unsigned long long)threadIdx.x * SCAN_ITEMS;
    uint32_t v[SCAN_ITEMS]; uint32_t s = 0;
    #pragma unroll
    for (int i = 0; i < SCAN_ITEMS; ++i) { v[i] = base + i < n ? in[base + i] : 0; s += v[i]; }
    uint32_t tot; uint32_t e = block_excl_scan(s, &tot) + tile_sum[blockIdx.x];
    #pragma unroll
    for (int i = 0; i < SCAN_ITEMS; ++i) { if (base + i < n) out[base + i] = e; e += v[i]; }
}

inline void exclusive_scan(uint64_t& launches, const uint32_t* in, uint32_t* out, uint32_t* tmp, const unsigned long long* n_ptr, unsigned long long n_bound,
                           unsigned long long* total_out, cudaStream_t st) {
    if (n_bound == 0) { if (total_out) cudaMemsetAsync(total_out, 0, 8, st); return; }
    int ntiles = (int)((n_bound + SCAN_TILE - 1) / SCAN_TILE);
    launch(launches, k_scan_reduce, ntiles, SCAN_THREADS, 0, st, in, tmp, n_ptr, n_bound);
    launch(launches, k_scan_tiles, 1, SCAN_THREADS, 0, st, tmp, ntiles, total_out);
    launch(launches, k_scan_down, ntiles, SCAN_THREADS, 0, st, in, out, tmp, n_ptr, n_bound);
}
inline size_t scan_tmp_elems(unsigned long long n_bound) { return (size_t)((n_bound + SCAN_TILE - 1) / SCAN_TILE) + 1; }

constexpr int RS_THREADS = 256;
constexpr int RS_ITEMS = 8;
constexpr int RS_TILE = RS_THREADS * RS_ITEMS;

__global__ void __launch_bounds__(RS_THREADS) k_radix_hist(const uint64_t* __restrict__ keys, uint32_t* __restrict__ hist, const unsigned long long* __restrict__ n_ptr,
                                                           unsigned long long n_bound, int shift, int nblk) {
    __shared__ uint32_t h[256];
    unsigned long long n = *n_ptr; if (n > n_bound) n = n_bound;
    unsigned long long base = (unsigned long long)blockIdx.x * RS_TILE;
    h[threadIdx.x] = 0;
    __syncthreads();
    if (base < n) {
        #pragma unroll
        for (int i = 0; i < RS_ITEMS; ++i) { unsigned long long j = base + (unsigned long long)i * RS_THREADS + threadIdx.x; if (j < n) atomicAdd(&h[(keys[j] >> shift) & 255], 1u); }
    }
    __syncthreads();
    hist[(size_t)threadIdx.x * nblk + blockIdx.x] = h[threadIdx.x];
}

__global__ void __launch_bounds__(RS_THREADS) k_radix_scatter(const uint64_t* __restrict__ kin, const uint32_t* __restrict__ vin, uint64_t* __restrict__ kout, uint32_t* __restrict__ vout,
                                                              const uint32_t* __restrict__ offs, const unsigned long long* __restrict__ n_ptr, unsigned long long n_bound, int shift, int nblk) {
    __shared__ uint32_t cnt[8][256];
    unsigned long long n = *n_ptr; if (n > n_bound) n = n_bound;
    unsigned long long tile0 = (unsigned long long)blockIdx.x * RS_TILE;
    if (tile0 >= n) return;
    int w = threadIdx.x >> 5, l = lane_id();
    for (int i = threadIdx.x; i < 8 * 256; i += RS_THREADS) (&cnt[0][0])[i] = 0;
    __syncthreads();
    uint64_t k[RS_ITEMS]; uint32_t v[RS_ITEMS]; uint32_t lr[RS_ITEMS];
    unsigned long long wbase = tile0 + (unsigned long long)w * 32 * RS_ITEMS;
    #pragma unroll
    for (int r = 0; r < RS_ITEMS; ++r) {
        unsigned long long j = wbase + (unsigned long long)r * 32 + l;
        bool valid = j < n;
        k[r] = valid ? kin[j] : 0; v[r] = valid ? vin[j] : 0;
        uint32_t d = (uint32_t)(k[r] >> shift) & 255u;
        uint32_t m = __match_any_sync(FULL, valid ? d : (256u + (uint32_t)l));
        uint32_t rank = __popc(m & lanemask_lt());
        uint32_t base = valid ? cnt[w][d] : 0;
        __syncwarp();
        if (valid && rank == 0) cnt[w][d] = base + __popc(m);
        __syncwarp();
        lr[r] = base + rank;
    }
    __syncthreads();
    {
        uint32_t s = offs[(size_t)threadIdx.x * nblk + blockIdx.x];
        #pragma unroll
        for (int ww = 0; ww < 8; ++ww) { uint32_t t = cnt[ww][threadIdx.x]; cnt[ww][threadIdx.x] = s; s += t; }
    }
    __syncthreads();
    #pragma unroll
    for (int r = 0; r < RS_ITEMS; ++r) {
        unsigned long long j = wbase + (unsigned long long)r * 32 + l;
        if (j < n) { uint32_t d = (uint32_t)(k[r] >> shift) & 255u; uint32_t pos = cnt[w][d] + lr[r]; kout[pos] = k[r]; vout[pos] = v[r]; }
    }
}

struct RadixTemp { uint32_t* hist; uint32_t* scan_tmp; };
inline size_t radix_hist_elems(unsigned long long n_bound) { return (size_t)256 * (size_t)((n_bound + RS_TILE - 1) / RS_TILE) + 256; }

inline void radix_sort(uint64_t& launches, uint64_t* k0, uint32_t* v0, uint64_t* k1, uint32_t* v1, RadixTemp tmp, const unsigned long long* n_ptr, unsigned long long n_bound,
                       int bits, bool* in_first, cudaStream_t st) {
    *in_first = true;
    if (n_bound == 0) return;
    int nblk = (int)((n_bound + RS_TILE - 1) / RS_TILE);
    for (int shift = 0; shift < bits; shift += 8) {
        const uint64_t* ki = *in_first ? k0 : k1; const uint32_t* vi = *in_first ? v0 : v1;
        uint64_t* ko = *in_first ? k1 : k0; uint32_t* vo = *in_first ? v1 : v0;
        launch(launches, k_radix_hist, nblk, RS_THREADS, 0, st, ki, tmp.hist, n_ptr, n_bound, shift, nblk);
        exclusive_scan(launches, tmp.hist, tmp.hist, tmp.scan_tmp, nullptr, (unsigned long long)256 * nblk, nullptr, st);
        launch(launches, k_radix_scatter, nblk, RS_THREADS, 0, st, ki, vi, ko, vo, tmp.hist, n_ptr, n_bound, shift, nblk);
        *in_first = !*in_first;
    }
}

}
```

Baseline: 9550.

## Slice consensus into candidate ranges pipelined across two streams with per-slice ALT copies

Splits the consensus prep/align/vote work into k slices of candidates, cut so each slice holds about the same number of sequence bytes. Slices alternate between the main and side streams, with event chaining so each slice's prep/align can overlap the previous slice's vote. Each slice's ALT bytes are copied device-to-host as soon as that slice finishes, overlapping the transfer with the remaining compute. This requires per-queue column scans, a slice-planning kernel, and more events and launches, which could outweigh the overlap if slices are small.

```diff
diff --git a/include/snfb.h b/include/snfb.h
--- a/include/snfb.h
+++ b/include/snfb.h
@@ -260,6 +260,7 @@
 int         snfb_device_alt(snfb_ctx* ctx, void** dptr, uint64_t* n_bytes);
 uint64_t    snfb_launch_count(snfb_ctx* ctx);
 uint64_t    snfb_rerun_count(snfb_ctx* ctx);
+int         snfb_set_consensus_slices(snfb_ctx* ctx, int k);
 int         snfb_coverage_bins(snfb_ctx* ctx, uint32_t task, int binsize, const double** out, uint64_t* n_bins);
 typedef struct snfb_gt_in {
     uint64_t n;
diff --git a/sniffles_b200/binding.py b/sniffles_b200/binding.py
--- a/sniffles_b200/binding.py
+++ b/sniffles_b200/binding.py
@@ -16,7 +16,7 @@
            "snfb_nccl_unique_id", "snfb_comm_init", "snfb_allgather_candidates", "snfb_selftest_sqrt_frac", "snfb_poa", "snfb_combine_groups", "snfb_combine_plan", "snfb_selftest_edit_distance",
            "snfb_load_bam", "snfb_set_regions", "snfb_ingest_sizes", "snfb_ingest_fetch", "snfb_inflate_bgzf", "snfb_deflate_bgzf",
            "snfb_genotype_targets", "snfb_load_reference", "snfb_reference_runs", "snfb_fetch_reference",
-           "snfb_population_load", "snfb_population_match", "snfb_read_names"]
+           "snfb_population_load", "snfb_population_match", "snfb_read_names", "snfb_set_consensus_slices"]
 
 
 def lib():
@@ -56,6 +56,7 @@
         L.snfb_unpin_host.argtypes = [C.c_void_p]
         L.snfb_rerun_count.restype = C.c_uint64
         L.snfb_rerun_count.argtypes = [C.c_void_p]
+        L.snfb_set_consensus_slices.argtypes = [C.c_void_p, C.c_int]
         L.snfb_coverage_bins.argtypes = [C.c_void_p, C.c_uint32, C.c_int, C.POINTER(C.c_void_p), C.POINTER(C.c_uint64)]
         L.snfb_nccl_unique_id.argtypes = [C.c_void_p]
         L.snfb_comm_init.argtypes = [C.c_void_p, C.c_void_p, C.c_int, C.c_int]
@@ -278,6 +279,9 @@
 
     def rerun_count(self):
         return int(self._lib.snfb_rerun_count(self._h))
+
+    def set_consensus_slices(self, k: int):
+        self._check(self._lib.snfb_set_consensus_slices(self._h, int(k)), "snfb_set_consensus_slices")
 
     def coverage_bins(self, task: int, binsize: int) -> np.ndarray:
         p = C.c_void_p()
diff --git a/sniffles_b200/csrc/api.cu b/sniffles_b200/csrc/api.cu
--- a/sniffles_b200/csrc/api.cu
+++ b/sniffles_b200/csrc/api.cu
@@ -81,6 +81,7 @@
 
 struct snfb_ctx {
     int device = 0; cudaStream_t st = nullptr, st_copy = nullptr, st_side = nullptr; cudaEvent_t ev_b = nullptr, ev_mid = nullptr, ev_fork = nullptr, ev_join = nullptr; std::string err;
+    cudaEvent_t ev_aligned[consensus::MAX_SLICES] = {}, ev_slice[consensus::MAX_SLICES] = {}; int n_slices = consensus::DEFAULT_SLICES;
     snfb_config cfg{}; bool have_cfg = false;
     bool loaded = false, on_device = false, seq_on_demand = false; const uint8_t* h_seq = nullptr; uint32_t evt_min = 0;
     uint64_t n_rec = 0, n_cigar = 0, n_var = 0, n_seq = 0; uint32_t n_task = 0, n_contig = 0, n_tr = 0, n_mask = 0;
@@ -103,10 +104,10 @@
     int32_t* v_pos; int32_t* v_end; uint8_t* v_flags; uint64_t* v_k0; uint64_t* v_k1; uint32_t* v_v0; uint32_t* v_v1; uint32_t* v_hist; uint32_t* v_scan; unsigned long long* v_n;
     snfb_lead* leads; extract::Event* ev_buf; snfb_lead* sorted_leads; uint32_t* radix_hist;
     cluster::B B{};
-    consensus::C Cc{}; consensus::SeqReq* seq_req; uint32_t* arena_off; uint8_t* seq_arena;
+    consensus::C Cc{}; consensus::SeqReq* seq_req; uint32_t* arena_off; uint8_t* seq_arena; uint32_t* q_scan_tmp;
     HostBuf h_seq_req, h_seq_arena; uint64_t seq_h2d_bytes = 0;
     bool stage_a_done = false, stage_b_done = false, stage_c_done = false;
-    HostBuf h_ctr_buf; DevCounters* h_mid = nullptr; DevCounters* h_fin = nullptr; uint32_t* h_work = nullptr;
+    HostBuf h_ctr_buf; DevCounters* h_mid = nullptr; DevCounters* h_fin = nullptr; consensus::Work* h_work = nullptr;
     HostBuf h_leads, h_task_reads, h_task_nm, h_rec_nm, h_cand, h_cand_leads, h_rnames, h_rn_off, h_task_cov, h_task_cov_raw, h_alt, h_cov_bins;
     void* comm = nullptr; int rank = 0, nranks = 1; DevBuf b_gsend, b_grecv; HostBuf h_gather, h_gather_out; unsigned long long gather_cap = 0;
     cudaEvent_t ev[MAX_TIMINGS + 1]; const char* ev_name[MAX_TIMINGS + 1]; uint64_t ev_bytes[MAX_TIMINGS + 1]; int n_ev = 0; int n_ev_load = 0; uint64_t launches = 0; uint64_t reruns = 0;
@@ -248,10 +249,12 @@
         || cudaStreamCreateWithFlags(&ctx->st_side, cudaStreamNonBlocking) != cudaSuccess) { delete ctx; return 4; }
     cudaEventCreateWithFlags(&ctx->ev_b, cudaEventDisableTiming); cudaEventCreateWithFlags(&ctx->ev_mid, cudaEventDisableTiming);
     cudaEventCreateWithFlags(&ctx->ev_fork, cudaEventDisableTiming); cudaEventCreateWithFlags(&ctx->ev_join, cudaEventDisableTiming);
+    for (int i = 0; i < consensus::MAX_SLICES; ++i) { cudaEventCreateWithFlags(&ctx->ev_aligned[i], cudaEventDisableTiming); cudaEventCreateWithFlags(&ctx->ev_slice[i], cudaEventDisableTiming); }
     for (int i = 0; i <= MAX_TIMINGS; ++i) cudaEventCreate(&ctx->ev[i]);
-    if (ctx->h_ctr_buf.ensure(2 * sizeof(DevCounters) + 256) || ctx->b_ctr.ensure(sizeof(DevCounters) + 64)) { delete ctx; return 5; }
-    ctx->h_mid = ctx->h_ctr_buf.as<DevCounters>(); ctx->h_fin = ctx->h_mid + 1; ctx->h_work = reinterpret_cast<uint32_t*>(ctx->h_fin + 1);
-    memset(ctx->h_ctr_buf.p, 0, 2 * sizeof(DevCounters) + 256);
+    const size_t ctr_bytes = 2 * sizeof(DevCounters) + 2 * sizeof(consensus::Work);
+    if (ctx->h_ctr_buf.ensure(ctr_bytes) || ctx->b_ctr.ensure(sizeof(DevCounters) + 64)) { delete ctx; return 5; }
+    ctx->h_mid = ctx->h_ctr_buf.as<DevCounters>(); ctx->h_fin = ctx->h_mid + 1; ctx->h_work = reinterpret_cast<consensus::Work*>(ctx->h_fin + 1);
+    memset(ctx->h_ctr_buf.p, 0, ctr_bytes);
     cudaFuncSetAttribute(cluster::k_cluster_warp<cluster::SMALL_CAP, cluster::CWS_WARPS, false>, cudaFuncAttributeMaxDynamicSharedMemorySize, (int)cluster::CwCfg<cluster::SMALL_CAP, cluster::CWS_WARPS>::smem);
     cudaFuncSetAttribute(cluster::k_cluster_warp<cluster::WARP_CAP, cluster::CWM_WARPS, true>, cudaFuncAttributeMaxDynamicSharedMemorySize, (int)cluster::CwCfg<cluster::WARP_CAP, cluster::CWM_WARPS>::smem);
     cudaFuncSetAttribute(cluster::k_cluster_block, cudaFuncAttributeMaxDynamicSharedMemorySize, (int)cluster::CB_SMEM);
@@ -266,6 +269,7 @@
     if (ctx->comm && g_nccl.CommDestroy) g_nccl.CommDestroy(ctx->comm);
     for (int i = 0; i <= MAX_TIMINGS; ++i) cudaEventDestroy(ctx->ev[i]);
     cudaEventDestroy(ctx->ev_b); cudaEventDestroy(ctx->ev_mid); cudaEventDestroy(ctx->ev_fork); cudaEventDestroy(ctx->ev_join);
+    for (int i = 0; i < consensus::MAX_SLICES; ++i) { cudaEventDestroy(ctx->ev_aligned[i]); cudaEventDestroy(ctx->ev_slice[i]); }
     cudaStreamDestroy(ctx->st_side); cudaStreamDestroy(ctx->st_copy); cudaStreamDestroy(ctx->st);
     delete ctx;
 }
@@ -699,7 +703,8 @@
     b.cand = c.take<snfb_cand>(k.cand + 1); b.cand_leads = c.take<snfb_lead>(k.cand_lead + 1); b.out_plo = c.take<uint32_t>(k.cand_lead + 1); b.out_pn = c.take<uint32_t>(k.cand_lead + 1);
     b.rnames = c.take<uint64_t>(k.rn + 1); b.rn_off_out = c.take<uint32_t>(k.cand + 2);
     cc.plan_best = c.take<uint32_t>(k.cand + 1); cc.plan_nother = c.take<uint32_t>(k.cand + 1); cc.plan_otot = c.take<uint32_t>(k.cand + 1); cc.alt_len = c.take<uint32_t>(k.cand + 1); cc.scr_len = c.take<uint32_t>(k.cand + 1);
-    cc.alt_off = c.take<uint32_t>(k.cand + 1); cc.scr_off = c.take<uint32_t>(k.cand + 1); cc.work_big = c.take<uint32_t>(k.cand + 1); cc.work_small = c.take<uint32_t>(k.cand + 1); cc.work_ctr = c.take<uint32_t>(64);
+    cc.alt_off = c.take<uint32_t>(k.cand + 1); cc.scr_off = c.take<uint32_t>(k.cand + 1); cc.work_big = c.take<uint32_t>(k.cand + 1); cc.work_small = c.take<uint32_t>(k.cand + 1); cc.work = c.take<consensus::Work>(1);
+    cc.q_cnt = c.take<uint32_t>(consensus::NQ * (k.cand + 1)); cc.q_off = c.take<uint32_t>(consensus::NQ * (k.cand + 1)); ctx->q_scan_tmp = c.take<uint32_t>(consensus::NQ * prims::scan_tmp_elems(k.cand));
     cc.items_big = c.take<consensus::C::Item>(k.item + 1); cc.items_small = c.take<consensus::C::Item>(k.item + 1); cc.tiles = c.take<uint2>(k.tile + 1);
     cc.alt = c.take<uint8_t>(k.alt + 64); cc.scr = c.take<uint8_t>(k.scr16 * 16 + 64);
     ctx->seq_req = c.take<consensus::SeqReq>(k.req + 1); ctx->seq_arena = c.take<uint8_t>(k.req16 * 16 + 64);
@@ -834,12 +839,14 @@
     if (ctx->n_mask) launch(ctx->launches, cluster::k_mask_bp, grid_for((unsigned long long)ctx->n_mask * 32, 128), 128, 0, st, b, ctx->b_mask_task.as<uint32_t>(), ctx->n_mask, ctx->task_cov);
     launch(ctx->launches, cluster::k_coverage, NUM_SMS * 32, 128, 0, st, b);
     consensus::C& c = ctx->Cc;
-    CUDA_TRY(cudaMemsetAsync(c.work_ctr, 0, 64, st));
+    CUDA_TRY(cudaMemsetAsync(c.work, 0, sizeof(consensus::Work), st));
     mark(ctx, "consensus_plan");
     launch(ctx->launches, consensus::k_plan, grid_for(ctx->cap.cand, 128), 128, 0, st, c);
     prims::exclusive_scan(ctx->launches, c.alt_len, c.alt_off, b.scan_tmp, &ctr->n_cand, ctx->cap.cand, &ctr->n_alt_bytes, st);
     prims::exclusive_scan(ctx->launches, c.scr_len, c.scr_off, b.scan_tmp, &ctr->n_cand, ctx->cap.cand, &ctr->n_seq_bytes, st);
+    prims::exclusive_scan_cols(ctx->launches, c.q_cnt, c.q_off, ctx->cap.cand + 1, consensus::NQ, ctx->q_scan_tmp, &ctr->n_cand, ctx->cap.cand, c.work->n, st);
     launch(ctx->launches, consensus::k_plan_finish, grid_for(ctx->cap.cand, 128), 128, 0, st, c);
+    launch(ctx->launches, consensus::k_plan_slices, 1, 32, 0, st, c, ctx->n_slices);
     mark(ctx, nullptr);
     CUDA_TRY(cudaGetLastError());
     return 0;
@@ -872,12 +879,20 @@
         }
         c.seq = ctx->seq_arena; c.arena_off = ctx->arena_off;
     }
-    mark(ctx, "consensus");
-    launch(ctx->launches, consensus::k_prep, NUM_SMS * 8, 128, 0, st, c);
-    mark(ctx, "consensus_align");
-    launch(ctx->launches, consensus::k_align, NUM_SMS * 7, consensus::ALIGN_WARPS * 32, 0, st, c);
-    mark(ctx, "consensus_vote");
-    launch(ctx->launches, consensus::k_vote, NUM_SMS * 16, consensus::VOTE_THREADS, 0, st, c);
+    CUDA_TRY(cudaEventRecord(ctx->ev_fork, st)); CUDA_TRY(cudaStreamWaitEvent(ctx->st_side, ctx->ev_fork, 0));
+    for (int s = 0; s < ctx->n_slices; ++s) {
+        cudaStream_t ss = (s & 1) ? ctx->st_side : st; const bool on_main = ss == st;
+        if (s) CUDA_TRY(cudaStreamWaitEvent(ss, ctx->ev_aligned[s - 1], 0));
+        if (on_main) mark(ctx, "consensus");
+        launch(ctx->launches, consensus::k_prep, NUM_SMS * 8, 128, 0, ss, c, s);
+        if (on_main) mark(ctx, "consensus_align");
+        launch(ctx->launches, consensus::k_align, NUM_SMS * 7, consensus::ALIGN_WARPS * 32, 0, ss, c, s);
+        CUDA_TRY(cudaEventRecord(ctx->ev_aligned[s], ss));
+        if (on_main) mark(ctx, "consensus_vote");
+        launch(ctx->launches, consensus::k_vote, NUM_SMS * 16, consensus::VOTE_THREADS, 0, ss, c, s);
+        CUDA_TRY(cudaEventRecord(ctx->ev_slice[s], ss));
+    }
+    CUDA_TRY(cudaEventRecord(ctx->ev_join, ctx->st_side)); CUDA_TRY(cudaStreamWaitEvent(st, ctx->ev_join, 0));
     mark(ctx, nullptr);
     CUDA_TRY(cudaGetLastError());
     return 0;
@@ -900,7 +915,7 @@
     else { if (k.req < 16) k.req = 16; if (k.req16 < 16) k.req16 = 16; }
 }
 static unsigned long long grown(unsigned long long need) { return need + need / 4 + 1024; }
-static bool caps_fit(snfb_ctx* ctx, const DevCounters& c, const uint32_t* work, int upto) {
+static bool caps_fit(snfb_ctx* ctx, const DevCounters& c, const consensus::Work& work, int upto) {
     Caps& k = ctx->cap; bool ok = true;
     const unsigned long long need_lead = std::max(c.n_slots, c.n_leads);
     if (need_lead > k.lead || c.lead_overflow) { k.lead = std::max(grown(need_lead), k.lead + k.lead / 2); ok = false; }
@@ -910,9 +925,9 @@
         if (c.n_rnames > k.rn) { k.rn = grown(c.n_rnames); ok = false; }
         if (c.n_alt_bytes > k.alt) { k.alt = grown(c.n_alt_bytes); ok = false; }
         if (c.n_seq_bytes > k.scr16) { k.scr16 = grown(c.n_seq_bytes); ok = false; }
-        const unsigned long long items = std::max(work[4], work[5]);
+        const unsigned long long items = std::max(work.n[consensus::Q_HEAVY], work.n[consensus::Q_LIGHT]);
         if (items > k.item) { k.item = grown(items); ok = false; }
-        if (work[8] > k.tile) { k.tile = grown(work[8]); ok = false; }
+        if (work.n[consensus::Q_TILE] > k.tile) { k.tile = grown(work.n[consensus::Q_TILE]); ok = false; }
     }
     if (upto >= 3) {
         if (c.n_req > k.req) { k.req = grown(c.n_req); ok = false; }
@@ -965,13 +980,8 @@
     if (c.ordinal_overflow) return "a read carries more than 65535 SV signatures (16-bit lead ordinal)";
     return nullptr;
 }
-static int run_pipeline(snfb_ctx* ctx, int upto, snfb_lead_view* leads, snfb_cand_view* cands, snfb_seq_view* seqs) {
-    if (!ctx->loaded) return fail(ctx, "no records loaded");
-    if (!ctx->have_cfg) return fail(ctx, "snfb_set_config was not called");
-    cudaSetDevice(ctx->device);
-    for (uint32_t t = 0; t < ctx->n_task; ++t) if ((long long)ctx->tasks[t].contig_len / ctx->cfg.cluster_binsize >= (1ll << 26)) return fail(ctx, "contig_len / cluster_binsize must stay below 2^26 (bin field of the sort key)");
-    initial_caps(ctx);
-    ctx->stage_a_done = ctx->stage_b_done = ctx->stage_c_done = false;
+static void drain(snfb_ctx* ctx) { cudaStreamSynchronize(ctx->st); cudaStreamSynchronize(ctx->st_side); cudaStreamSynchronize(ctx->st_copy); }
+static int run_attempts(snfb_ctx* ctx, int upto, snfb_cand_view* cands, snfb_seq_view* seqs) {
     for (int attempt = 0; ; ++attempt) {
         if (attempt == 6) return fail(ctx, "buffer capacities did not converge");
         if (ensure_arenas(ctx)) return 1;
@@ -979,38 +989,52 @@
         ctx->n_ev = ctx->n_ev_load;
         cudaStream_t st = ctx->st; DevCounters* ctr = ctx->B.ctr;
         if (enqueue_stage_a(ctx)) return 1;
-        bool mid = false, copies = false;
+        bool mid = false;
         if (upto >= 2) {
             if (enqueue_stage_b(ctx)) return 1;
             CUDA_TRY(cudaEventRecord(ctx->ev_b, st)); CUDA_TRY(cudaStreamWaitEvent(ctx->st_copy, ctx->ev_b, 0));
             CUDA_TRY(cudaMemcpyAsync(ctx->h_mid, ctr, sizeof(DevCounters), cudaMemcpyDeviceToHost, ctx->st_copy));
-            CUDA_TRY(cudaMemcpyAsync(ctx->h_work, ctx->Cc.work_ctr, 64, cudaMemcpyDeviceToHost, ctx->st_copy));
+            CUDA_TRY(cudaMemcpyAsync(&ctx->h_work[0], ctx->Cc.work, sizeof(consensus::Work), cudaMemcpyDeviceToHost, ctx->st_copy));
             CUDA_TRY(cudaEventRecord(ctx->ev_mid, ctx->st_copy));
             mid = true;
         }
         if (upto >= 3 && !ctx->seq_on_demand) { if (enqueue_stage_c(ctx)) return 1; }
         if (mid) {
             CUDA_TRY(cudaEventSynchronize(ctx->ev_mid));
-            if (const char* m = fatal_counter(*ctx->h_mid)) { cudaStreamSynchronize(st); return fail(ctx, m); }
-            if (!caps_fit(ctx, *ctx->h_mid, ctx->h_work, 2)) { CUDA_TRY(cudaStreamSynchronize(st)); ++ctx->reruns; continue; }
-            if (ctx->h_mid->unverified_breaks && !ctx->force_no_cuts) { CUDA_TRY(cudaStreamSynchronize(st)); ctx->force_no_cuts = true; ++ctx->reruns; continue; }
-            if (cands) { if (enqueue_cand_copies(ctx, *ctx->h_mid, ctx->st_copy)) return 1; copies = true; }
+            if (const char* m = fatal_counter(*ctx->h_mid)) return fail(ctx, m);
+            if (!caps_fit(ctx, *ctx->h_mid, ctx->h_work[0], 2)) { drain(ctx); ++ctx->reruns; continue; }
+            if (ctx->h_mid->unverified_breaks && !ctx->force_no_cuts) { drain(ctx); ctx->force_no_cuts = true; ++ctx->reruns; continue; }
+            if (cands) { if (enqueue_cand_copies(ctx, *ctx->h_mid, ctx->st_copy)) return 1; }
             if (upto >= 3 && ctx->seq_on_demand) { if (enqueue_stage_c(ctx)) return 1; }
         }
         if (upto >= 3 && seqs) {
             const unsigned long long na = ctx->h_mid->n_alt_bytes;
             if (ctx->h_alt.ensure(na + 16)) return fail(ctx, "out of pinned memory for the ALT arena");
-            if (na) CUDA_TRY(cudaMemcpyAsync(ctx->h_alt.p, ctx->Cc.alt, na, cudaMemcpyDeviceToHost, st));
+            for (int s = 0; s < ctx->n_slices; ++s) {
+                const consensus::Slice& sl = ctx->h_work[0].slice[s];
+                if (sl.alt_hi <= sl.alt_lo) continue;
+                CUDA_TRY(cudaStreamWaitEvent(ctx->st_copy, ctx->ev_slice[s], 0));
+                CUDA_TRY(cudaMemcpyAsync(ctx->h_alt.as<uint8_t>() + sl.alt_lo, ctx->Cc.alt + sl.alt_lo, sl.alt_hi - sl.alt_lo, cudaMemcpyDeviceToHost, ctx->st_copy));
+            }
         }
         CUDA_TRY(cudaMemcpyAsync(ctx->h_fin, ctr, sizeof(DevCounters), cudaMemcpyDeviceToHost, st));
-        CUDA_TRY(cudaMemcpyAsync(ctx->h_work + 16, ctx->Cc.work_ctr, 64, cudaMemcpyDeviceToHost, st));
+        CUDA_TRY(cudaMemcpyAsync(&ctx->h_work[1], ctx->Cc.work, sizeof(consensus::Work), cudaMemcpyDeviceToHost, st));
         CUDA_TRY(cudaStreamSynchronize(st));
-        if (copies) CUDA_TRY(cudaStreamSynchronize(ctx->st_copy));
+        CUDA_TRY(cudaStreamSynchronize(ctx->st_copy));
         CUDA_TRY(cudaGetLastError());
         if (const char* m = fatal_counter(*ctx->h_fin)) return fail(ctx, m);
-        if (!caps_fit(ctx, *ctx->h_fin, upto >= 2 ? ctx->h_work + 16 : ctx->h_work, upto)) { ++ctx->reruns; continue; }
-        break;
-    }
+        if (!caps_fit(ctx, *ctx->h_fin, ctx->h_work[upto >= 2 ? 1 : 0], upto)) { ++ctx->reruns; continue; }
+        return 0;
+    }
+}
+static int run_pipeline(snfb_ctx* ctx, int upto, snfb_lead_view* leads, snfb_cand_view* cands, snfb_seq_view* seqs) {
+    if (!ctx->loaded) return fail(ctx, "no records loaded");
+    if (!ctx->have_cfg) return fail(ctx, "snfb_set_config was not called");
+    cudaSetDevice(ctx->device);
+    for (uint32_t t = 0; t < ctx->n_task; ++t) if ((long long)ctx->tasks[t].contig_len / ctx->cfg.cluster_binsize >= (1ll << 26)) return fail(ctx, "contig_len / cluster_binsize must stay below 2^26 (bin field of the sort key)");
+    initial_caps(ctx);
+    ctx->stage_a_done = ctx->stage_b_done = ctx->stage_c_done = false;
+    if (run_attempts(ctx, upto, cands, seqs)) { drain(ctx); return 1; }
     ctx->stage_a_done = true; ctx->stage_b_done = upto >= 2; ctx->stage_c_done = upto >= 3;
     if (leads) { memset(leads, 0, sizeof *leads); if (fill_lead_view(ctx, leads)) return 1; }
     if (cands) { memset(cands, 0, sizeof *cands); finish_cand_view(ctx, *ctx->h_fin, cands); }
@@ -1067,6 +1091,11 @@
 uint64_t snfb_launch_count(snfb_ctx* ctx) { return ctx ? ctx->launches : 0; }
 double snfb_selftest_sqrt_frac(uint64_t p_hi, uint64_t p_lo, uint64_t q, int slow) { const u128 P = ((u128)p_hi << 64) | p_lo; return slow ? sqrt_frac_rn_slow(P, q) : sqrt_frac_rn(P, q); }
 uint64_t snfb_rerun_count(snfb_ctx* ctx) { return ctx ? ctx->reruns : 0; }
+int snfb_set_consensus_slices(snfb_ctx* ctx, int k) {
+    if (!ctx) return 1;
+    if (k < 1 || k > consensus::MAX_SLICES) return fail(ctx, "snfb_set_consensus_slices: k must be 1 to 8");
+    ctx->n_slices = k; return 0;
+}
 int snfb_pin_host(void* p, size_t bytes) { return cudaHostRegister(p, bytes, cudaHostRegisterDefault) == cudaSuccess ? 0 : 1; }
 int snfb_unpin_host(void* p) { return cudaHostUnregister(p) == cudaSuccess ? 0 : 1; }
 
diff --git a/sniffles_b200/csrc/consensus.cuh b/sniffles_b200/csrc/consensus.cuh
--- a/sniffles_b200/csrc/consensus.cuh
+++ b/sniffles_b200/csrc/consensus.cuh
@@ -7,6 +7,15 @@
 constexpr int TAB = 2048;
 constexpr uint8_t DASH = 0xff;
 constexpr int MAXHIT = 512, MAXHIT_LIGHT = 384; constexpr uint32_t HEAVY_L = 3000;
+
+enum { Q_BIG, Q_SMALL, Q_HEAVY, Q_LIGHT, Q_TILE, NQ };
+constexpr int MAX_SLICES = 8, DEFAULT_SLICES = 2;
+struct Slice { uint32_t c_lo, c_hi; uint32_t lo[NQ], hi[NQ]; unsigned long long alt_lo, alt_hi; };
+struct Work {
+    unsigned long long n[NQ];
+    uint32_t pos[MAX_SLICES][4];
+    Slice slice[MAX_SLICES];
+};
 
 struct C {
     const snfb_cand* cand; snfb_cand* cand_rw; const snfb_lead* cand_leads;
@@ -16,7 +25,8 @@
     const uint32_t* arena_off;
     uint32_t* plan_best; uint32_t* plan_nother; uint32_t* plan_otot; uint32_t* alt_len; uint32_t* scr_len; uint32_t* alt_off; uint32_t* scr_off;
     uint8_t* alt; uint8_t* scr; unsigned long long alt_cap, scr_cap16, cand_cap;
-    uint32_t* work_big; uint32_t* work_small; uint32_t* work_ctr;
+    uint32_t* work_big; uint32_t* work_small; Work* work;
+    uint32_t* q_cnt; uint32_t* q_off;
     struct Item { uint32_t cand; uint32_t k; uint32_t row; uint32_t rd_off; };
     Item* items_big; Item* items_small; uint2* tiles; unsigned long long item_cap, tile_cap;
     DevCounters* ctr; snfb_config cfg;
@@ -27,7 +37,7 @@
 __global__ void k_plan(C c) {
     const unsigned long long nc = c.ctr->n_cand < c.cand_cap ? c.ctr->n_cand : c.cand_cap;
     for (unsigned long long i = blockIdx.x * (unsigned long long)blockDim.x + threadIdx.x; i < nc; i += (unsigned long long)gridDim.x * blockDim.x) {
-        uint32_t al = 0, sl = 0;
+        uint32_t al = 0, sl = 0, heavy_n = 0, light_n = 0, tiles = 0; bool big = false;
         if (c.cand[i].svtype == SNFB_INS && !c.cfg.symbolic) {
             const snfb_cand* cd = &c.cand[i]; long nm = 0, bi = -1; long long bd = 0; long long tot = 0;
             for (int k = 0; k < cd->lead_n; ++k) { const snfb_lead* l = &c.cand_leads[cd->lead_off + k]; if (!(l->flags & SNFB_LF_HAS_SEQ)) continue;
@@ -40,28 +50,49 @@
                 const unsigned long long bytes = cons ? (unsigned long long)tot + 8 + (unsigned long long)(nm - 1) * ((L + 3u) & ~3u) + (unsigned long long)(nm - 1) * 16 + 64 + 16 + TAB * 8 : (unsigned long long)L + 24;
                 sl = (uint32_t)((bytes + 15) / 16);
                 c.cand_rw[i].alt_len = (int)L;
-                const unsigned long long work = (unsigned long long)L * (unsigned long long)nm;
-                if (work > 60000ull) c.work_big[atomicAdd(&c.work_ctr[0], 1u)] = (uint32_t)i; else c.work_small[atomicAdd(&c.work_ctr[1], 1u)] = (uint32_t)i;
-                if (cons) {
-                    const bool heavy = L > HEAVY_L; C::Item* dst = heavy ? c.items_big : c.items_small;
-                    const uint32_t base = atomicAdd(&c.work_ctr[heavy ? 4 : 5], (uint32_t)(nm - 1));
-                    uint32_t row = 0, ro = 0;
-                    for (int k = 0; k < cd->lead_n; ++k) { const snfb_lead* l = &c.cand_leads[cd->lead_off + k]; if (!(l->flags & SNFB_LF_HAS_SEQ) || k == bi) continue;
-                        if ((unsigned long long)base + row < c.item_cap) { C::Item it; it.cand = (uint32_t)i; it.k = (uint32_t)k; it.row = row; it.rd_off = ro; dst[base + row] = it; }
-                        ++row; ro += ((uint32_t)l->seq_len + 7u) & ~7u; }
-                    const uint32_t nt = (L + 4095u) / 4096u; const uint32_t tb = atomicAdd(&c.work_ctr[8], nt);
-                    for (uint32_t t = 0; t < nt; ++t) if ((unsigned long long)tb + t < c.tile_cap) c.tiles[tb + t] = make_uint2((uint32_t)i, t);
-                }
+                big = (unsigned long long)L * (unsigned long long)nm > 60000ull;
+                if (cons) { const bool heavy = L > HEAVY_L; heavy_n = heavy ? (uint32_t)(nm - 1) : 0u; light_n = heavy ? 0u : (uint32_t)(nm - 1); tiles = (L + 4095u) / 4096u; }
             }
         }
         c.alt_len[i] = al; c.scr_len[i] = sl;
+        const size_t col = c.cand_cap + 1;
+        c.q_cnt[Q_BIG * col + i] = sl && big; c.q_cnt[Q_SMALL * col + i] = sl && !big; c.q_cnt[Q_HEAVY * col + i] = heavy_n; c.q_cnt[Q_LIGHT * col + i] = light_n; c.q_cnt[Q_TILE * col + i] = tiles;
     }
 }
 
 __global__ void k_plan_finish(C c) {
-    const unsigned long long nc = c.ctr->n_cand < c.cand_cap ? c.ctr->n_cand : c.cand_cap;
-    for (unsigned long long i = blockIdx.x * (unsigned long long)blockDim.x + threadIdx.x; i < nc; i += (unsigned long long)gridDim.x * blockDim.x)
-        if (c.scr_len[i]) c.cand_rw[i].alt_off = (int)c.alt_off[i];
+    const unsigned long long nc = c.ctr->n_cand < c.cand_cap ? c.ctr->n_cand : c.cand_cap; const size_t col = c.cand_cap + 1;
+    for (unsigned long long i = blockIdx.x * (unsigned long long)blockDim.x + threadIdx.x; i < nc; i += (unsigned long long)gridDim.x * blockDim.x) {
+        if (!c.scr_len[i]) continue;
+        c.cand_rw[i].alt_off = (int)c.alt_off[i];
+        if (c.q_cnt[Q_BIG * col + i]) c.work_big[c.q_off[Q_BIG * col + i]] = (uint32_t)i; else c.work_small[c.q_off[Q_SMALL * col + i]] = (uint32_t)i;
+        const uint32_t nh = c.q_cnt[Q_HEAVY * col + i], no = nh + c.q_cnt[Q_LIGHT * col + i];
+        C::Item* dst = nh ? c.items_big : c.items_small; const uint32_t base = c.q_off[(nh ? Q_HEAVY : Q_LIGHT) * col + i];
+        const snfb_cand* cd = &c.cand[i]; const uint32_t bi = c.plan_best[i];
+        uint32_t row = 0, ro = 0;
+        for (int k = 0; no && k < cd->lead_n; ++k) { const snfb_lead* l = &c.cand_leads[cd->lead_off + k]; if (!(l->flags & SNFB_LF_HAS_SEQ) || (uint32_t)k == bi) continue;
+            if ((unsigned long long)base + row < c.item_cap) { C::Item it; it.cand = (uint32_t)i; it.k = (uint32_t)k; it.row = row; it.rd_off = ro; dst[base + row] = it; }
+            ++row; ro += ((uint32_t)l->seq_len + 7u) & ~7u; }
+        const uint32_t nt = c.q_cnt[Q_TILE * col + i], tb = c.q_off[Q_TILE * col + i];
+        for (uint32_t t = 0; t < nt; ++t) if ((unsigned long long)tb + t < c.tile_cap) c.tiles[tb + t] = make_uint2((uint32_t)i, t);
+    }
+}
+
+__global__ void k_plan_slices(C c, int k) {
+    const int s = threadIdx.x; if (s >= k) return;
+    const unsigned long long nc = c.ctr->n_cand < c.cand_cap ? c.ctr->n_cand : c.cand_cap; const size_t col = c.cand_cap + 1;
+    const unsigned long long tot = c.ctr->n_seq_bytes;
+    auto cut = [&](int j) -> uint32_t {
+        if (j <= 0) return 0; if (j >= k) return (uint32_t)nc;
+        const unsigned long long want = (tot * (unsigned long long)j + k - 1) / (unsigned long long)k;
+        uint32_t lo = 0, hi = (uint32_t)nc;
+        while (lo < hi) { const uint32_t m = (lo + hi) / 2; if (c.scr_off[m] < want) lo = m + 1; else hi = m; }
+        return lo;
+    };
+    Slice sl; sl.c_lo = cut(s); sl.c_hi = cut(s + 1);
+    for (int q = 0; q < NQ; ++q) { sl.lo[q] = sl.c_lo < nc ? c.q_off[q * col + sl.c_lo] : (uint32_t)c.work->n[q]; sl.hi[q] = sl.c_hi < nc ? c.q_off[q * col + sl.c_hi] : (uint32_t)c.work->n[q]; }
+    sl.alt_lo = sl.c_lo < nc ? c.alt_off[sl.c_lo] : c.ctr->n_alt_bytes; sl.alt_hi = sl.c_hi < nc ? c.alt_off[sl.c_hi] : c.ctr->n_alt_bytes;
+    c.work->slice[s] = sl;
 }
 
 __device__ __forceinline__ uint32_t nib_swap(uint32_t w) { return ((w & 0x0f0f0f0fu) << 4) | ((w >> 4) & 0x0f0f0f0fu); }
@@ -286,13 +317,14 @@
     return scr;
 }
 
-__global__ void __launch_bounds__(128) k_prep(C c) {
+__global__ void __launch_bounds__(128) k_prep(C c, int s) {
     __shared__ uint32_t s_cand;
     static const char CODE[17] = "=ACMGRSVTWYHKDBN";
+    const Slice& sl = c.work->slice[s];
     for (;;) {
         __syncthreads();
-        if (threadIdx.x == 0) { const uint32_t q = atomicAdd(&c.work_ctr[2], 1u); const uint32_t nb = c.work_ctr[0], ns = c.work_ctr[1];
-            s_cand = q < nb ? c.work_big[q] : (q < nb + ns ? c.work_small[q - nb] : 0xffffffffu); }
+        if (threadIdx.x == 0) { const uint32_t q = atomicAdd(&c.work->pos[s][0], 1u); const uint32_t nb = sl.hi[Q_BIG] - sl.lo[Q_BIG], ns = sl.hi[Q_SMALL] - sl.lo[Q_SMALL];
+            s_cand = q < nb ? c.work_big[sl.lo[Q_BIG] + q] : (q < nb + ns ? c.work_small[sl.lo[Q_SMALL] + q - nb] : 0xffffffffu); }
         __syncthreads();
         const uint32_t ci = s_cand; if (ci == 0xffffffffu) break;
         const uint32_t L = c.alt_len[ci];
@@ -414,14 +446,15 @@
 }
 
 constexpr int ALIGN_WARPS = 4;
-__global__ void __launch_bounds__(ALIGN_WARPS * 32, 7) k_align(C c) {
+__global__ void __launch_bounds__(ALIGN_WARPS * 32, 7) k_align(C c, int s) {
     __shared__ int sm[5][ALIGN_WARPS * MAXHIT_LIGHT]; __shared__ int s_red[2 * ALIGN_WARPS]; __shared__ uint32_t s_q;
     static_assert(ALIGN_WARPS * MAXHIT_LIGHT >= MAXHIT, "a block item needs MAXHIT entries");
     const int lane = lane_id(), warp = threadIdx.x >> 5;
-    const uint32_t nb = (uint32_t)min((unsigned long long)c.work_ctr[4], c.item_cap), ns = (uint32_t)min((unsigned long long)c.work_ctr[5], c.item_cap);
+    const Slice& sl = c.work->slice[s];
+    const uint32_t b0 = sl.lo[Q_HEAVY], nb = (uint32_t)min((unsigned long long)sl.hi[Q_HEAVY], c.item_cap), s0 = sl.lo[Q_LIGHT], ns = (uint32_t)min((unsigned long long)sl.hi[Q_LIGHT], c.item_cap);
     for (;;) {
         __syncthreads();
-        if (threadIdx.x == 0) s_q = atomicAdd(&c.work_ctr[6], 1u);
+        if (threadIdx.x == 0) s_q = b0 + atomicAdd(&c.work->pos[s][1], 1u);
         __syncthreads();
         const uint32_t q = s_q; if (q >= nb) break;
         BlockGrp<ALIGN_WARPS> g; g.tid = threadIdx.x; g.red = s_red;
@@ -429,7 +462,7 @@
     }
     __syncthreads();
     for (;;) {
-        uint32_t q = 0; if (lane == 0) q = atomicAdd(&c.work_ctr[7], 1u);
+        uint32_t q = 0; if (lane == 0) q = s0 + atomicAdd(&c.work->pos[s][2], 1u);
         q = __shfl_sync(FULL, q, 0);
         if (q >= ns) break;
         WarpGrp g; g.tid = lane; const int o = warp * MAXHIT_LIGHT;
@@ -444,12 +477,13 @@
     for (int k = 0; k < 4; ++k) cnt[k] += sel == (uint32_t)k ? inc : 0ull;
 }
 constexpr int VOTE_THREADS = 64;
-__global__ void __launch_bounds__(VOTE_THREADS) k_vote(C c) {
+__global__ void __launch_bounds__(VOTE_THREADS) k_vote(C c, int s) {
     __shared__ uint2 s_tile; __shared__ int s_nacc, s_nlist; __shared__ uint16_t s_rows[VOTE_LIST];
     static const char CODE[17] = "=ACMGRSVTWYHKDBN";
+    const Slice& sl = c.work->slice[s];
     for (;;) {
         __syncthreads();
-        if (threadIdx.x == 0) { const uint32_t q = atomicAdd(&c.work_ctr[9], 1u); s_tile = q < c.work_ctr[8] && q < c.tile_cap ? c.tiles[q] : make_uint2(0xffffffffu, 0); }
+        if (threadIdx.x == 0) { const uint32_t q = sl.lo[Q_TILE] + atomicAdd(&c.work->pos[s][3], 1u); s_tile = q < sl.hi[Q_TILE] && q < c.tile_cap ? c.tiles[q] : make_uint2(0xffffffffu, 0); }
         __syncthreads();
         const uint32_t ci = s_tile.x; if (ci == 0xffffffffu) break;
         const uint32_t L = c.alt_len[ci], no = c.plan_nother[ci];
diff --git a/sniffles_b200/csrc/prims.cuh b/sniffles_b200/csrc/prims.cuh
--- a/sniffles_b200/csrc/prims.cuh
+++ b/sniffles_b200/csrc/prims.cuh
@@ -34,8 +34,9 @@
 }
 
 __global__ void __launch_bounds__(SCAN_THREADS) k_scan_reduce(const uint32_t* __restrict__ in, uint32_t* __restrict__ tile_sum,
-                                                              const unsigned long long* __restrict__ n_ptr, unsigned long long n_bound) {
+                                                              const unsigned long long* __restrict__ n_ptr, unsigned long long n_bound, size_t stride) {
     unsigned long long n = n_ptr ? *n_ptr : n_bound; if (n > n_bound) n = n_bound;
+    in += blockIdx.y * stride; tile_sum += (size_t)blockIdx.y * gridDim.x;
     unsigned long long base = (unsigned long long)blockIdx.x * SCAN_TILE;
     uint32_t s = 0;
     #pragma unroll
@@ -44,18 +45,19 @@
     if (threadIdx.x == 0) tile_sum[blockIdx.x] = tot;
 }
 __global__ void __launch_bounds__(SCAN_THREADS) k_scan_tiles(uint32_t* __restrict__ tile_sum, int ntiles, unsigned long long* total_out) {
-    uint32_t carry = 0;
+    uint32_t carry = 0; tile_sum += (size_t)blockIdx.x * ntiles;
     for (int b = 0; b < ntiles; b += SCAN_THREADS) {
         int j = b + threadIdx.x; uint32_t v = j < ntiles ? tile_sum[j] : 0; uint32_t tot;
         uint32_t e = block_excl_scan(v, &tot);
         if (j < ntiles) tile_sum[j] = e + carry;
         carry += tot;
     }
-    if (threadIdx.x == 0 && total_out) *total_out = carry;
+    if (threadIdx.x == 0 && total_out) total_out[blockIdx.x] = carry;
 }
 __global__ void __launch_bounds__(SCAN_THREADS) k_scan_down(const uint32_t* __restrict__ in, uint32_t* __restrict__ out, const uint32_t* __restrict__ tile_sum,
-                                                            const unsigned long long* __restrict__ n_ptr, unsigned long long n_bound) {
+                                                            const unsigned long long* __restrict__ n_ptr, unsigned long long n_bound, size_t stride) {
     unsigned long long n = n_ptr ? *n_ptr : n_bound; if (n > n_bound) n = n_bound;
+    in += blockIdx.y * stride; out += blockIdx.y * stride; tile_sum += (size_t)blockIdx.y * gridDim.x;
     unsigned long long base = (unsigned long long)blockIdx.x * SCAN_TILE + (unsigned long long)threadIdx.x * SCAN_ITEMS;
     uint32_t v[SCAN_ITEMS]; uint32_t s = 0;
     #pragma unroll
@@ -65,13 +67,17 @@
     for (int i = 0; i < SCAN_ITEMS; ++i) { if (base + i < n) out[base + i] = e; e += v[i]; }
 }
 
+inline void exclusive_scan_cols(uint64_t& launches, const uint32_t* in, uint32_t* out, size_t stride, int cols, uint32_t* tmp, const unsigned long long* n_ptr,
+                                unsigned long long n_bound, unsigned long long* total_out, cudaStream_t st) {
+    if (n_bound == 0) { if (total_out) cudaMemsetAsync(total_out, 0, 8 * cols, st); return; }
+    int ntiles = (int)((n_bound + SCAN_TILE - 1) / SCAN_TILE);
+    launch(launches, k_scan_reduce, dim3(ntiles, cols), SCAN_THREADS, 0, st, in, tmp, n_ptr, n_bound, stride);
+    launch(launches, k_scan_tiles, cols, SCAN_THREADS, 0, st, tmp, ntiles, total_out);
+    launch(launches, k_scan_down, dim3(ntiles, cols), SCAN_THREADS, 0, st, in, out, tmp, n_ptr, n_bound, stride);
+}
 inline void exclusive_scan(uint64_t& launches, const uint32_t* in, uint32_t* out, uint32_t* tmp, const unsigned long long* n_ptr, unsigned long long n_bound,
                            unsigned long long* total_out, cudaStream_t st) {
-    if (n_bound == 0) { if (total_out) cudaMemsetAsync(total_out, 0, 8, st); return; }
-    int ntiles = (int)((n_bound + SCAN_TILE - 1) / SCAN_TILE);
-    launch(launches, k_scan_reduce, ntiles, SCAN_THREADS, 0, st, in, tmp, n_ptr, n_bound);
-    launch(launches, k_scan_tiles, 1, SCAN_THREADS, 0, st, tmp, ntiles, total_out);
-    launch(launches, k_scan_down, ntiles, SCAN_THREADS, 0, st, in, out, tmp, n_ptr, n_bound);
+    exclusive_scan_cols(launches, in, out, 0, 1, tmp, n_ptr, n_bound, total_out, st);
 }
 inline size_t scan_tmp_elems(unsigned long long n_bound) { return (size_t)((n_bound + SCAN_TILE - 1) / SCAN_TILE) + 1; }
 
```

New measurement: 9933 (median of 6 runs). +4.0%, better.
